# lh3/psmc

Hardware: AMD Instinct MI355X
Metric: genome bins/sec through forward-backward (n=64) (higher is better)
Workload: dtype f64; 1 GPU; configs[2]: whole-genome .psmcfa-like batch, 30000001 bins x 64 states in 90 segments per GPU, -p 4+25*2+4+6, one E-step (EM iteration) per step, parameters of a different EM round every step; mode=fast, bins_per_gpu=30000001, bins_total=30000001, n_states=64, segments=90, longest_segment=2490000, tiles=8127, speculative_overlap_bins=3072, structured_sweeps=True, tile_bins=3712

## Files before the change

include/psmc_hip.h:

```cpp
#ifndef PSMC_HIP_H
#define PSMC_HIP_H
#include <stdint.h>
#ifdef __cplusplus
extern "C" {
#endif

#define PSMC_HIP_MODE_EXACT 0
#define PSMC_HIP_MODE_FAST  1

#define PSMC_HIP_MAX_STATES 1024

#define PSMC_HIP_OK        0
#define PSMC_HIP_EINVAL   -1
#define PSMC_HIP_ENOMEM   -2
#define PSMC_HIP_EDEVICE  -3
#define PSMC_HIP_ENOTSUP  -4
#define PSMC_HIP_ESTATE   -5
#define PSMC_HIP_ECONVERGE -6

typedef struct psmc_hip_ctx psmc_hip_ctx;

int psmc_hip_device_count(void);
int psmc_hip_device_cus(int device);

int psmc_hip_create(psmc_hip_ctx **ctx, int n_states, int device, int mode);
void psmc_hip_destroy(psmc_hip_ctx *ctx);
const char *psmc_hip_strerror(int err);
const char *psmc_hip_last_error(const psmc_hip_ctx *ctx);

int psmc_hip_set_option(psmc_hip_ctx *ctx, const char *key, double value);

int psmc_hip_set_cu_range(psmc_hip_ctx *ctx, int first, int count);

int psmc_hip_load_segments(psmc_hip_ctx *ctx, int n_seg, const uint8_t *const *seq, const int32_t *L);
int psmc_hip_load_segments_device(psmc_hip_ctx *ctx, int n_seg, const void *d_obs, const int64_t *off,
                                  const int32_t *L);
int psmc_hip_select(psmc_hip_ctx *ctx, int n_sel, const int32_t *seg_idx);

int psmc_hip_estep(psmc_hip_ctx *ctx, const double *a, const double *e, const double *a0, double *A, double *E,
                   double *A0, double *LL, double *chk);

int psmc_hip_reserve_tables(psmc_hip_ctx *ctx);

int psmc_hip_reserve_batch_tables(psmc_hip_ctx *ctx, int64_t max_bins);
int psmc_hip_estep_batch(psmc_hip_ctx *ctx, int n_rep, const double *a, const double *e, const double *a0,
                         const int32_t *sel_off, const int32_t *sel_idx, double *A, double *sums, double *E, double *LL);
typedef void (*psmc_hip_batch_done_fn)(void *user, int n_done, const int32_t *replicates);
int psmc_hip_estep_batch_cb(psmc_hip_ctx *ctx, int n_rep, const double *a, const double *e, const double *a0,
                            const int32_t *sel_off, const int32_t *sel_idx, double *A, double *sums, double *E, double *LL,
                            psmc_hip_batch_done_fn done, void *user);
int psmc_hip_batch_info(psmc_hip_ctx *ctx, int out[2]);

int psmc_hip_estep_segments(psmc_hip_ctx *ctx, const double *a, const double *e, const double *a0, double *segA,
                            double *segE, double *segA0, double *segLL, double *chk);

int psmc_hip_estep_device(psmc_hip_ctx *ctx, const double *a, const double *e, const double *a0, void *d_stats,
                          void *stream);
int psmc_hip_fast_diag(psmc_hip_ctx *ctx, double *warm_err_fwd, double *warm_err_bwd, int *n_chunks,
                       int *warmup_used);
int psmc_hip_fast_repairs(psmc_hip_ctx *ctx, int out[6]);
int psmc_hip_fast_plan(psmc_hip_ctx *ctx, double out[8]);

int psmc_hip_estep_factored(psmc_hip_ctx *ctx, const double *a, const double *e, const double *a0, double *sums,
                            double *E, double *LL);

int psmc_hip_fast_info(psmc_hip_ctx *ctx, int out[8]);

int psmc_hip_get_tables(psmc_hip_ctx *ctx, int seg, double *f, double *b, double *s);

int psmc_hip_decode(psmc_hip_ctx *ctx, int seg, int32_t *path, double *maxp);

int psmc_hip_posterior(psmc_hip_ctx *ctx, int seg, double *post, double *recomb);

int psmc_hip_post_counts(psmc_hip_ctx *ctx, int seg, const int32_t *cnt1, int32_t l, int32_t n_cnt, double *cnt);

int psmc_hip_scales(psmc_hip_ctx *ctx, int seg, double *s);


typedef struct psmc_hip_group psmc_hip_group;
int  psmc_hip_group_create(psmc_hip_group **g, int n_states, int n_dev, const int *devices, int mode);
void psmc_hip_group_destroy(psmc_hip_group *g);
const char *psmc_hip_group_last_error(const psmc_hip_group *g);
int  psmc_hip_group_set_option(psmc_hip_group *g, const char *key, double value);
int  psmc_hip_group_load_segments(psmc_hip_group *g, int n_seg, const uint8_t *const *seq, const int32_t *L);
int  psmc_hip_group_estep(psmc_hip_group *g, const double *a, const double *e, const double *a0, double *A, double *E,
                          double *A0, double *LL, double *chk);
int  psmc_hip_group_estep_factored(psmc_hip_group *g, const double *a, const double *e, const double *a0, double *sums,
                                   double *E, double *LL);
int  psmc_hip_group_selfcheck(psmc_hip_group *g, int out[4]);
int  psmc_hip_group_info(psmc_hip_group *g, int *n_shards, int32_t *shard_of_seg, int *last_reduce);
int  psmc_hip_group_route(psmc_hip_group *g, int seg, psmc_hip_ctx **ctx, int *local_seg);
int  psmc_hip_estep_factored_device(psmc_hip_ctx *ctx, const double *a, const double *e, const double *a0, void *d_stats,
                                    void *stream);

#ifdef __cplusplus
}
#endif
#endif
```

psmc_amd/csrc/api.hip:

```cpp
#include "psmc_hip_ctx.h"

static void destroy_kids(psmc_hip_ctx *c);

static int make_streams(psmc_hip_ctx *c)
{
	hipStream_t *st[5] = {&c->stream, &c->stream2, &c->stream3, &c->stream4, &c->stream5};
	for (hipStream_t *s : st) if (*s) { (void)hipStreamSynchronize(*s); (void)hipStreamDestroy(*s); *s = nullptr; }
	if (c->cu_count <= 0) {
		for (hipStream_t *s : st) if (hipStreamCreateWithFlags(s, hipStreamNonBlocking) != hipSuccess) return PSMC_HIP_EDEVICE;
		return 0;
	}
	int cus = 0;
	if (hipDeviceGetAttribute(&cus, hipDeviceAttributeMultiprocessorCount, c->device) != hipSuccess || cus <= 0) return PSMC_HIP_EDEVICE;
	if (c->cu_first < 0 || c->cu_first + c->cu_count > cus) return PSMC_HIP_EINVAL;
	std::vector<uint32_t> mask((size_t)(cus + 31) / 32, 0u);
	for (int i = c->cu_first; i < c->cu_first + c->cu_count; ++i) mask[(size_t)i >> 5] |= 1u << (i & 31);
	for (hipStream_t *s : st) if (hipExtStreamCreateWithCUMask(s, (uint32_t)mask.size(), mask.data()) != hipSuccess) return PSMC_HIP_EDEVICE;
	return 0;
}

extern "C" int psmc_hip_device_cus(int device)
{
	int cus = 0;
	if (hipDeviceGetAttribute(&cus, hipDeviceAttributeMultiprocessorCount, device) != hipSuccess) { (void)hipGetLastError(); return 0; }
// ... 28 lines not shown

extern "C" int psmc_hip_device_count(void)
{
	int n = 0;
	if (hipGetDeviceCount(&n) != hipSuccess) return 0;
	return n;
}

extern "C" const char *psmc_hip_strerror(int err)
{
	switch (err) {
	case PSMC_HIP_OK: return "ok";
	case PSMC_HIP_EINVAL: return "invalid argument";
	case PSMC_HIP_ENOMEM: return "out of memory";
	case PSMC_HIP_EDEVICE: return "HIP runtime error";
	case PSMC_HIP_ENOTSUP: return "not supported in this build";
	case PSMC_HIP_ESTATE: return "call order violated";
	case PSMC_HIP_ECONVERGE: return "fast-mode tile boundaries did not converge";
	default: return "unknown error";
	}
}
extern "C" const char *psmc_hip_last_error(const psmc_hip_ctx *ctx) { return ctx ? ctx->err.c_str() : ""; }

extern "C" int psmc_hip_create(psmc_hip_ctx **out, int n_states, int device, int mode)
{
	if (!out) return PSMC_HIP_EINVAL;
	*out = nullptr;
	if (n_states < 1) return PSMC_HIP_EINVAL;
	if (mode != PSMC_HIP_MODE_EXACT && mode != PSMC_HIP_MODE_FAST) return PSMC_HIP_EINVAL;
	if (n_states > PSMC_HIP_MAX_STATES) return PSMC_HIP_ENOTSUP;
	int nd = psmc_hip_device_count();
	if (nd <= 0 || device < 0 || device >= nd) return PSMC_HIP_EDEVICE;
	if (hipSetDevice(device) != hipSuccess) return PSMC_HIP_EDEVICE;
	psmc_hip_ctx *c = new (std::nothrow) psmc_hip_ctx();
	if (!c) return PSMC_HIP_ENOMEM;
	c->n = n_states; c->ns = n_states > 128 ? (n_states + 63) / 64 * 64 : (n_states > 64 ? 128 : 64); c->device = device; c->mode = mode;
	c->par_len = c->ns > 128 ? 2 * (size_t)c->ns * c->ns + 4 * (size_t)c->ns : psmc_hip_ctx::PAR_LEN;
	if (make_streams(c) != 0) { psmc_hip_destroy(c); return PSMC_HIP_EDEVICE; }
	for (int i = 0; i < 14; ++i)
		if (hipEventCreate(&c->evx[i]) != hipSuccess) { delete c; return PSMC_HIP_EDEVICE; }
	for (int i = 0; i < 10; ++i)
		if (hipEventCreate(&c->ev[i]) != hipSuccess) { delete c; return PSMC_HIP_EDEVICE; }
	if (hipHostMalloc((void **)&c->h_par, c->par_len * sizeof(double), hipHostMallocDefault) != hipSuccess ||
	    hipMalloc((void **)&c->d_par, c->par_len * sizeof(double)) != hipSuccess) {
		psmc_hip_destroy(c);
		return PSMC_HIP_ENOMEM;
	}
	if (const char *env = getenv("PSMC_HIP_OPTIONS")) {
		std::string all(env);
		size_t at = 0;
		while (at < all.size()) {
			size_t end = all.find(',', at);
			if (end == std::string::npos) end = all.size();
			const std::string kv = all.substr(at, end - at);
			const size_t eq = kv.find('=');
			at = end + 1;
			if (kv.empty()) continue;
			char *endp = nullptr;
			const double val = eq == std::string::npos ? 0.0 : strtod(kv.c_str() + eq + 1, &endp);
			const bool parsed = eq != std::string::npos && eq + 1 < kv.size() && endp && *endp == '\0';
			if (parsed && kv.compare(0, eq, "rccl") == 0) continue;
			if (!parsed || psmc_hip_set_option(c, kv.substr(0, eq).c_str(), val) != PSMC_HIP_OK) {
				fprintf(stderr, "[psmc_hip] PSMC_HIP_OPTIONS: bad entry \"%s\" (unknown key, value out of range, or not a number)\n", kv.c_str());
				psmc_hip_destroy(c);
				return PSMC_HIP_EINVAL;
			}
		}
	}
	*out = c;
	return PSMC_HIP_OK;
}

static void destroy_kids(psmc_hip_ctx *c)
{
	if (c->x_twin) { psmc_hip_destroy(c->x_twin); c->x_twin = nullptr; }
	for (psmc_hip_ctx *k : c->kids) psmc_hip_destroy(k);
	c->kids.clear();
	c->share_T = 0;
}

extern "C" void psmc_hip_destroy(psmc_hip_ctx *c)
{
	if (!c) return;
	(void)hipSetDevice(c->device);
	destroy_kids(c);
	if (c->parent) {
		void *mine[] = {c->d_seg_off, c->d_seg_len, c->d_work, c->d_chunks, c->d_entry, c->d_bexit, c->d_Cpart, c->d_Epart, c->d_LLpart,
		                c->d_stage, c->d_stats, c->d_warm, c->d_bentry, c->d_dirty, c->d_cnt, c->d_gate, c->d_queue, c->d_touch, c->d_items, c->d_ftiles, c->d_Kcol,
		                c->d_segA, c->d_segE, c->d_segA0, c->d_chk};
		for (void *p : mine) if (p) (void)hipFree(p);
		if (c->h_cnt) (void)hipHostFree(c->h_cnt);
		if (c->h_ritems) (void)hipHostFree(c->h_ritems);
		if (c->h_mlen) (void)hipHostFree(c->h_mlen);
		if (c->h_chunks) (void)hipHostFree(c->h_chunks);
		if (c->h_mis) (void)hipHostFree(c->h_mis);
		if (c->d_prevx) (void)hipFree(c->d_prevx);
		if (c->d_finv) (void)hipFree(c->d_finv);
		delete c;
		return;
	}
	if (c->stream) (void)hipStreamSynchronize(c->stream);
	free_wide_fast(c);
	if (c->stream2) (void)hipStreamSynchronize(c->stream2);
	if (c->stream3) (void)hipStreamSynchronize(c->stream3);
	if (c->stream4) (void)hipStreamSynchronize(c->stream4);
	if (c->stream5) (void)hipStreamSynchronize(c->stream5);
	if (!c->obs_borrowed && c->d_obs) (void)hipFree(c->d_obs);
	void *ptrs[] = {c->d_seg_off, c->d_seg_len, c->d_work, c->d_par, c->d_f, c->d_b, c->d_s, c->d_segA, c->d_segE,
	                c->d_segA0, c->d_chk, c->d_chunks, c->d_entry, c->d_bexit, c->d_Cpart, c->d_Epart, c->d_LLpart,
	                c->d_stage, c->d_stats, c->d_warm, c->d_bentry, c->d_dirty, c->d_cnt, c->d_gate, c->d_queue, c->d_touch, c->d_sb, c->d_items, c->d_ftiles, c->d_Kcol,
	                c->d_bw_seg, c->d_bw_par, c->d_bw_tab, c->d_bpar, c->d_s_all, c->d_cu_mask, c->d_lkp, c->d_lkoff, c->d_b2};
	for (void *p : ptrs) if (p) (void)hipFree(p);
	if (c->h_par) (void)hipHostFree(c->h_par);
	if (c->h_cnt) (void)hipHostFree(c->h_cnt);
	if (c->h_ritems) (void)hipHostFree(c->h_ritems);
	if (c->h_mlen) (void)hipHostFree(c->h_mlen);
	if (c->h_chunks) (void)hipHostFree(c->h_chunks);
	if (c->h_mis) (void)hipHostFree(c->h_mis);
	if (c->d_prevx) (void)hipFree(c->d_prevx);
	if (c->d_finv) (void)hipFree(c->d_finv);
	for (int i = 0; i < 10; ++i) if (c->ev[i]) (void)hipEventDestroy(c->ev[i]);
	for (int i = 0; i < 14; ++i) if (c->evx[i]) (void)hipEventDestroy(c->evx[i]);
	if (c->stream4) (void)hipStreamDestroy(c->stream4);
	if (c->stream5) (void)hipStreamDestroy(c->stream5);
	if (c->stream2) (void)hipStreamDestroy(c->stream2);
	if (c->stream3) (void)hipStreamDestroy(c->stream3);
	if (c->stream) (void)hipStreamDestroy(c->stream);
	delete c;
}

extern "C" int psmc_hip_set_option(psmc_hip_ctx *c, const char *key, double v)
{
	if (!c || !key) return PSMC_HIP_EINVAL;
	std::string k(key);
	if (k == "batch_first") { if (v < 0 || v > 1e6) return PSMC_HIP_EINVAL; c->batch_first = (int)v; return PSMC_HIP_OK; }
	destroy_kids(c);
	if (k == "chunk") { if (v < 0) return PSMC_HIP_EINVAL; c->chunk = (int)v; c->plan_dirty = true; }
	else if (k == "warmup") { if (v < 0) return PSMC_HIP_EINVAL; c->warmup = (int)v; c->warmup_set = true; c->plan_dirty = true; }
	else if (k == "max_rounds") c->max_rounds = (int)v;
	else if (k == "structured") { c->struct_opt = v != 0 ? 1 : 0; }
	else if (k == "learn") { c->learn = v != 0 ? 1 : 0; }
	else if (k == "merge") { c->merge = v != 0 ? 1 : 0; c->plan_dirty = true; c->chunk_cap = 0; }
	else if (k == "adapt") { c->adapt = v != 0 ? 1 : 0; c->plan_dirty = true; c->chunk_cap = 0; }
	else if (k == "prev_start") { c->prev_start = v != 0 ? 1 : 0; c->prev_ok = false; c->plan_dirty = true; c->chunk_cap = 0; }
	else if (k == "warm_shift") { if (v < 0 || v > 4) return PSMC_HIP_EINVAL; c->warm_shift = (int)v; c->warm_shift_set = true; c->plan_dirty = true; }
	else if (k == "merge1") { if (v < -1 || v > 1) return PSMC_HIP_EINVAL; c->merge1 = (int)v; c->plan_dirty = true; }
	else if (k == "phase1") { if (v < -1 || v > 1) return PSMC_HIP_EINVAL; c->phase1 = (int)v; }
	else if (k == "phase1_waves") { if (v < 1 || v > 4) return PSMC_HIP_EINVAL; c->phase1_waves = (int)v; }
	else if (k == "lanes8") { if (v < -1 || v > 1) return PSMC_HIP_EINVAL; c->lanes8 = (int)v; }
	else if (k == "gap_tiles") { c->gap_tiles = v != 0 ? 1 : 0; c->plan_dirty = true; c->items_dirty = true; }
	else if (k == "coarse") { if (v < -1 || v > 16) return PSMC_HIP_EINVAL; c->coarse = (int)v; c->plan_dirty = true; c->items_dirty = true; }
	else if (k == "kc_sub") { if (v < 1 || v > 16) return PSMC_HIP_EINVAL; c->kc_sub = (int)v; c->kc_sub_set = true; c->plan_dirty = true; c->items_dirty = true; }
	else if (k == "two_phase") { if (v != -1 && v != 0 && v != 2) return PSMC_HIP_EINVAL; c->two_phase = (int)v; c->plan_dirty = true; c->items_dirty = true; }
	else if (k == "kc_min") { if (v < -1) return PSMC_HIP_EINVAL; c->kc_min = (int)v; c->items_dirty = true; }
	else if (k == "ckpt") { c->ckpt = v != 0 ? 1 : 0; }
	else if (k == "fuse") { c->fuse = v != 0 ? 1 : 0; c->plan_dirty = true; }
	else if (k == "fuse128") { if (v != 0 && v != 2) return PSMC_HIP_EINVAL; c->fuse128 = (int)v; c->plan_dirty = true; c->items_dirty = true; }
	else if (k == "group_cap") { if (v < 0) return PSMC_HIP_EINVAL; c->group_cap = (int)v; c->items_dirty = true; }
	else if (k == "share_learn") { c->share_learn = v != 0 ? 1 : 0; }
	else if (k == "exact_refwd") { if (v < -1 || v > 2) return PSMC_HIP_EINVAL; c->exact_refwd = (int)v; c->reserved_refwd = -1; c->reserved_cap = 0; if (c->d_b2) { (void)hipFree(c->d_b2); c->d_b2 = nullptr; c->b2_bins = c->b2_alloc = 0; } }
	else if (k == "batch_sort") { c->batch_sort = v != 0 ? 1 : 0; }
	else if (k == "batch_tailfill") c->batch_tailfill = v != 0;
	else if (k == "batch_major") c->batch_major = v != 0;
	else if (k == "batch_bins") { if (v < 0) return PSMC_HIP_EINVAL; c->batch_bins = (int64_t)v; }
	else if (k == "overlap") c->overlap = v != 0 ? 1 : 0;
	else if (k == "warm_tol") c->warm_tol = v;
	else if (k == "wide_fast") { if (v != 0 && v != 1) return PSMC_HIP_EINVAL; c->wide_fast = (int)v; }
	else if (k == "wide_decode") { if (v != 0 && v != 1) return PSMC_HIP_EINVAL; c->wide_decode = (int)v; }
	else if (k == "rep_impl") c->rep_impl = v < 0 ? -1 : (v != 0 ? 1 : 0);
	else return PSMC_HIP_EINVAL;
	return PSMC_HIP_OK;
}

int set_segments_common(psmc_hip_ctx *c, int n_seg, const int32_t *L)
{
	destroy_kids(c);
	c->reserved_refwd = -1; c->reserved_cap = 0;
	if (c->d_b2) { (void)hipFree(c->d_b2); c->d_b2 = nullptr; c->b2_bins = c->b2_alloc = 0; }
	c->n_seg = n_seg;
	c->L.assign(L, L + n_seg);
	int rc;
	if ((rc = dev_alloc(c, &c->d_seg_off, (size_t)n_seg))) return rc;
	if ((rc = dev_alloc(c, &c->d_seg_len, (size_t)n_seg))) return rc;
	HIPCHK(c, hipMemcpy(c->d_seg_off, c->off.data(), sizeof(int64_t) * n_seg, hipMemcpyHostToDevice));
	HIPCHK(c, hipMemcpy(c->d_seg_len, c->L.data(), sizeof(int32_t) * n_seg, hipMemcpyHostToDevice));
	std::vector<int32_t> all(n_seg);
	for (int i = 0; i < n_seg; ++i) all[i] = i;
	return psmc_hip_select(c, n_seg, all.data());
}

extern "C" int psmc_hip_load_segments(psmc_hip_ctx *c, int n_seg, const uint8_t *const *seq, const int32_t *L)
{
	if (!c || n_seg < 1 || !seq || !L) return fail(c, PSMC_HIP_EINVAL, "load_segments: bad argument");
	HIPCHK(c, hipSetDevice(c->device));
	c->off.resize(n_seg);
	int64_t tot = 0;
	for (int i = 0; i < n_seg; ++i) {
		if (L[i] < 1 || !seq[i]) return fail(c, PSMC_HIP_EINVAL, "load_segments: empty segment");
		c->off[i] = tot;
		tot += ((int64_t)L[i] + 63) & ~(int64_t)63;
	}
	c->total = tot;
	std::vector<uint8_t> host((size_t)tot + 256, 2);
	for (int i = 0; i < n_seg; ++i) {
		for (int32_t j = 0; j < L[i]; ++j)
			if (seq[i][j] > 2) return fail(c, PSMC_HIP_EINVAL, "load_segments: symbol outside {0,1,2}");
		memcpy(host.data() + c->off[i], seq[i], (size_t)L[i]);
	}
	if (!c->obs_borrowed && c->d_obs) { (void)hipFree(c->d_obs); }
	c->d_obs = nullptr; c->obs_borrowed = false;
	int rc;
	if ((rc = dev_alloc(c, &c->d_obs, host.size()))) return rc;
	HIPCHK(c, hipMemcpy(c->d_obs, host.data(), host.size(), hipMemcpyHostToDevice));
	return set_segments_common(c, n_seg, L);
}

extern "C" int psmc_hip_load_segments_device(psmc_hip_ctx *c, int n_seg, const void *d_obs, const int64_t *off,
                                             const int32_t *L)
{
	if (!c || n_seg < 1 || !d_obs || !off || !L) return fail(c, PSMC_HIP_EINVAL, "load_segments_device: bad argument");
	HIPCHK(c, hipSetDevice(c->device));
	int64_t end = 0;
	for (int i = 0; i < n_seg; ++i) {
		if (L[i] < 1 || (off[i] & 63) || off[i] < end) return fail(c, PSMC_HIP_EINVAL, "load_segments_device: bad layout");
		end = off[i] + (((int64_t)L[i] + 63) & ~(int64_t)63);
	}
	if (!c->obs_borrowed && c->d_obs) (void)hipFree(c->d_obs);
	c->d_obs = (uint8_t *)d_obs; c->obs_borrowed = true;
	c->off.assign(off, off + n_seg);
	c->total = end;
	return set_segments_common(c, n_seg, L);
}

extern "C" int psmc_hip_select(psmc_hip_ctx *c, int n_sel, const int32_t *idx)
{
	if (!c || n_sel < 1 || !idx) return fail(c, PSMC_HIP_EINVAL, "select: bad argument");
	if (c->n_seg < 1) return fail(c, PSMC_HIP_ESTATE, "select: no segments loaded");
	std::vector<int32_t> pos(c->n_seg, -1);
	c->sel.assign(idx, idx + n_sel);
	c->work.clear(); c->mult.clear(); c->sel2work.resize(n_sel);
	for (int i = 0; i < n_sel; ++i) {
		if (idx[i] < 0 || idx[i] >= c->n_seg) return fail(c, PSMC_HIP_EINVAL, "select: index out of range");
		if (pos[idx[i]] < 0) { pos[idx[i]] = (int32_t)c->work.size(); c->work.push_back(idx[i]); c->mult.push_back(0); }
		c->sel2work[i] = pos[idx[i]];
		c->mult[pos[idx[i]]]++;
	}
	HIPCHK(c, hipSetDevice(c->device));
	int rc;
	if ((rc = dev_alloc(c, &c->d_work, c->work.size()))) return rc;
	HIPCHK(c, hipMemcpy(c->d_work, c->work.data(), sizeof(int32_t) * c->work.size(), hipMemcpyHostToDevice));
	c->plan_dirty = true;
	++c->sel_serial;
	return PSMC_HIP_OK;
}

bool factor_structure(int n, int S, const double *a , double *sp )
{
	double *P = sp, *R = sp + S, *qa = sp + 2 * S, *cc = sp + 3 * S, *dd = sp + 4 * S;
	memset(sp, 0, 5 * (size_t)S * sizeof(double));
	if (n < 3) return false;
	const double pl = a[(n - 1) * S + 0], pu = a[0 * S + (n - 1)];
	if (!(pl > 1e-280) || !(pu > 1e-280)) return false;
	for (int l = 0; l < n - 1; ++l) qa[l] = a[(n - 1) * S + l] / pl;
	for (int k = 1; k < n; ++k) P[k] = a[k * S + 0];
	for (int l = 1; l < n; ++l) cc[l] = a[0 * S + l] / pu;
	for (int k = 0; k < n - 1; ++k) R[k] = a[k * S + (n - 1)];
	const double tol = 64 * 2.220446049250313e-16;
	for (int k = 0; k < n; ++k) {
		for (int l = 0; l < n; ++l) {
			if (l == k) continue;
			const double v = a[k * S + l], w = l < k ? P[k] * qa[l] : R[k] * cc[l];
			if (!(fabs(v - w) <= tol * fabs(v) + 1e-290)) return false;
		}
		dd[k] = a[k * S + k] - P[k] * qa[k] - R[k] * cc[k];
		if (!(dd[k] >= 0.0)) return false;
	}
	return true;
}

static void fill_kcc(int S, const double *sp, const double *e3 , double *out )
{
	const double *P = sp, *R = sp + S, *qa = sp + 2 * S, *cv = sp + 3 * S, *dd = sp + 4 * S;
	for (int dir = 0; dir < 2; ++dir) {
		double *t = out + (size_t)dir * 11 * S;
		const double *mS = dir == 0 ? P : cv, *wS = dir == 0 ? qa : R, *mP = dir == 0 ? R : qa, *wP = dir == 0 ? cv : P;
		for (int k = 0; k < S; ++k) { t[k] = mS[k]; t[S + k] = mP[k]; }
		for (int sy = 0; sy < 3; ++sy)
			for (int k = 0; k < S; ++k) {
				const double ev = e3[sy * S + k];
				double *u = t + 2 * S + (size_t)sy * 3 * S;
				u[k] = wS[k] * ev; u[S + k] = wP[k] * ev; u[2 * S + k] = dd[k] * ev;
			}
	}
}

bool fill_params(const psmc_hip_ctx *c, const double *a, const double *e, const double *a0, double *dst)
{
	const int n = c->n;
	if (c->ns > 128) {
		const size_t S = (size_t)c->ns;
		double *pa = dst, *pt = pa + S * S, *pe = pt + S * S, *pa0 = pe + 3 * S;
		memset(pa, 0, c->par_len * sizeof(double));
		for (int k = 0; k < n; ++k) {
			for (int l = 0; l < n; ++l) { pa[k * S + l] = a[(size_t)k * n + l]; pt[l * S + k] = a[(size_t)k * n + l]; }
			pe[k] = e[k]; pe[S + k] = e[n + k];
			pa0[k] = a0[k];
// ... 299 lines not shown
```

psmc_amd/csrc/api_batch.hip:

```cpp
#include "psmc_hip_ctx.h"

namespace {
struct RepSel { std::vector<int32_t> work, sel2work; int64_t bins = 0; };
}

static int batch_selections(psmc_hip_ctx *c, int n_rep, const int32_t *sel_off, const int32_t *sel_idx, std::vector<RepSel> &reps)
{
	std::vector<int32_t> pos(c->n_seg);
	reps.assign(n_rep, RepSel());
	for (int r = 0; r < n_rep; ++r) {
		const int n_sel = sel_off[r + 1] - sel_off[r];
		if (n_sel < 1) return fail(c, PSMC_HIP_EINVAL, "estep_batch: empty selection");
		std::fill(pos.begin(), pos.end(), -1);
		RepSel &R = reps[r];
		R.sel2work.resize(n_sel);
		for (int i = 0; i < n_sel; ++i) {
			const int32_t sg = sel_idx[sel_off[r] + i];
			if (sg < 0 || sg >= c->n_seg) return fail(c, PSMC_HIP_EINVAL, "estep_batch: index out of range");
			if (pos[sg] < 0) { pos[sg] = (int32_t)R.work.size(); R.work.push_back(sg); R.bins += ((int64_t)c->L[sg] + 63) & ~(int64_t)63; }
			R.sel2work[i] = pos[sg];
		}
	}
	return 0;
}
// ... 226 lines not shown
		if (c->bpar_cap < (size_t)n_rep) { if ((rc = dev_alloc(c, &c->d_bpar, (size_t)n_rep * PL))) return rc; c->bpar_cap = (size_t)n_rep; }
		if (refwd && !c->d_cu_mask && (rc = dev_alloc(c, &c->d_cu_mask, (size_t)4096))) return rc;
		size_t lk_worst = 0;
		for (int g = 0; g < n_launches; ++g) {
			size_t t = 0;
			for (int i = l_first[g]; i < l_first[g + 1]; ++i) t += wseg[i] >= 0 ? (size_t)(c->L[wseg[i]] / LKP_DIV + LKP_MIN) : 1;
			lk_worst = std::max(lk_worst, t);
		}
		if (c->lkp_cap < lk_worst) { if ((rc = dev_alloc(c, &c->d_lkp, lk_worst))) return rc; c->lkp_cap = lk_worst; }
		if (c->lkoff_cap < worst_entries) { if ((rc = dev_alloc(c, &c->d_lkoff, worst_entries))) return rc; c->lkoff_cap = worst_entries; }
		if (fwd_all && c->s_all_cap < (size_t)all_bins + 128) { if ((rc = dev_alloc(c, &c->d_s_all, (size_t)all_bins + 128))) return rc; c->s_all_cap = (size_t)all_bins + 128; }
	}
	static const bool dbg_t = getenv("PSMC_HIP_DEBUG_TIMES") != nullptr;
	auto now = []() { return dbg_now(); };
	{
		std::vector<double> hp((size_t)n_rep * PL);
		for (int r = 0; r < n_rep; ++r) (void)fill_params(c, a + (size_t)r * n * n, e + (size_t)r * 2 * n, a0 + (size_t)r * n, hp.data() + (size_t)r * PL);
		HIPCHK(c, hipStreamSynchronize(c->stream));
		HIPCHK(c, hipMemcpyAsync(c->d_bw_seg, wseg.data(), sizeof(int32_t) * n_all, hipMemcpyHostToDevice, c->stream));
		HIPCHK(c, hipMemcpyAsync(c->d_bw_par, wpar.data(), sizeof(int32_t) * n_all, hipMemcpyHostToDevice, c->stream));
		HIPCHK(c, hipMemcpyAsync(c->d_bw_tab, wtab.data(), sizeof(int64_t) * n_all, hipMemcpyHostToDevice, c->stream));
		HIPCHK(c, hipMemcpyAsync(c->d_bw_tab + n_all, wtab_s.data(), sizeof(int64_t) * n_all, hipMemcpyHostToDevice, c->stream));
		HIPCHK(c, hipMemcpyAsync(c->d_bpar, hp.data(), sizeof(double) * hp.size(), hipMemcpyHostToDevice, c->stream));
		HIPCHK(c, hipStreamSynchronize(c->stream));
	}
	c->tables_batch = true;
	double fwd_all_s = 0.0;
	if (fwd_all) {
		const double t0 = now();
		EstepLaunch p;
		fill_common(c, p, c->stream, c->d_bpar);
		p.d_work = c->d_bw_seg; p.n_work = n_all; p.d_work_par = c->d_bw_par; p.d_work_tab = c->d_bw_tab + n_all; p.par_stride = (int64_t)PL; p.work_align = align;
		p.exact_refwd = 1; p.exact_only = 1; p.d_s = c->d_s_all;
		if (launch_exact(p) != 0) return fail(c, PSMC_HIP_EDEVICE, "launch_exact (batch, forward pass of all entries)", hipGetLastError());
		if (dbg_t) { (void)hipStreamSynchronize(c->stream); fwd_all_s = now() - t0; }
	}
	if ((double)n_all * (double)(S * S) * 8.0 > 16e9) {
		c->err = "estep_batch: the per-entry statistics of this call (" + std::to_string(n_all) + " entries x " + std::to_string(S) + "^2 doubles) need more than 16 GB of host memory: send fewer replicates per call at this many states";
		return PSMC_HIP_ENOMEM;
	}
	c->h_segA.resize((size_t)n_all * S * S); c->h_segE.resize((size_t)n_all * 3 * S);
	std::vector<double> lk_all((size_t)n_all, 0.0);
	std::vector<int> last_launch(n_rep, 0);
	{
		std::vector<int> launch_of((size_t)n_all, 0);
		for (int g = 0; g < n_launches; ++g) for (int i = l_first[g]; i < l_first[g + 1]; ++i) launch_of[i] = g;
		for (int r = 0; r < n_rep; ++r) for (int w : ent_of[r]) if (w >= 0) last_launch[r] = std::max(last_launch[r], launch_of[w]);
	}
	std::vector<double> sA((size_t)n * n), sE((size_t)2 * n);
	double t_sums = 0.0;
	auto finalize = [&](int r) {
		const RepSel &R = reps[r];
		std::fill(sA.begin(), sA.end(), 0.0); std::fill(sE.begin(), sE.end(), 0.0);
		double ll = 0.0;
		for (size_t i = 0; i < R.sel2work.size(); ++i) {
			const int w = ent_of[r][R.sel2work[i]];
			const double *hA = &c->h_segA[(size_t)w * S * S], *hE = &c->h_segE[(size_t)w * 3 * S];
			ll += lk_all[(size_t)w];
			for (int k = 0; k < n; ++k)
				for (int l = 0; l < n; ++l) sA[(size_t)k * n + l] += hA[k * S + l];
			for (int b = 0; b < 2; ++b)
				for (int l = 0; l < n; ++l) sE[(size_t)b * n + l] += hE[b * S + l];
		}
		if (A) memcpy(A + (size_t)r * n * n, sA.data(), sizeof(double) * n * n);
		if (E) memcpy(E + (size_t)r * 2 * n, sE.data(), sizeof(double) * 2 * n);
		if (LL) LL[r] = ll;
		if (sums) {
			double *q = sums + (size_t)r * 5 * n;
			memset(q, 0, sizeof(double) * 5 * n);
			for (int k = 0; k < n; ++k)
				for (int l = 0; l < n; ++l) {
					const double v = sA[(size_t)k * n + l];
					if (l < k) { q[k] += v; q[3 * n + l] += v; } else if (l > k) { q[n + k] += v; q[4 * n + l] += v; } else q[2 * n + k] = v;
				}
		}
	};
	std::vector<int32_t> finished;
	for (int g = 0; g < n_launches; ++g) {
		const double t_a = now();
		const int e0 = l_first[g], nw = l_first[g + 1] - e0;
		int64_t run = 0; int32_t longest = 0;
		for (int i = e0; i < e0 + nw; ++i) if (wseg[i] >= 0) { run = std::max(run, wtab[i] + padded_len(wseg[i])); longest = std::max(longest, c->L[wseg[i]]); }
		EstepLaunch p;
		fill_common(c, p, c->stream, c->d_bpar);
		p.d_work = c->d_bw_seg + e0; p.n_work = nw; p.d_work_par = c->d_bw_par + e0; p.d_work_tab = c->d_bw_tab + e0; p.par_stride = (int64_t)PL; p.work_align = align;
		p.exact_refwd = refwd ? (c->exact_refwd == 1 ? 1 : 2) : 0;
		p.d_cu_mask = c->d_cu_mask;
		if (fwd_all) { p.exact_only = 2; p.d_work_tab_s = c->d_bw_tab + n_all + e0; p.d_s = c->d_s_all; }
		p.d_segA = c->d_segA; p.d_segE = c->d_segE; p.d_segA0 = c->d_segA0; p.d_chk = c->d_chk;
		const double t_b = now();
		if (launch_exact(p) != 0) return fail(c, PSMC_HIP_EDEVICE, "launch_exact (batch)", hipGetLastError());
		if (dbg_t) (void)hipStreamSynchronize(c->stream);
		const double t_c = now();
		std::vector<int64_t> lkoff((size_t)nw);
		int64_t lk_tot = 0;
		for (int i = 0; i < nw; ++i) { lkoff[i] = lk_tot; lk_tot += wseg[e0 + i] >= 0 ? c->L[wseg[e0 + i]] / LKP_DIV + LKP_MIN : 1; }
		HIPCHK(c, hipMemcpyAsync(c->d_lkoff, lkoff.data(), sizeof(int64_t) * nw, hipMemcpyHostToDevice, c->stream));
		if (launch_lk_products(c->stream, p, fwd_all ? c->d_s_all : c->d_s, c->d_lkoff, c->d_lkp) != 0) return fail(c, PSMC_HIP_EDEVICE, "launch_lk_products", hipGetLastError());
		c->h_lkp.resize((size_t)lk_tot);
		HIPCHK(c, hipMemcpyAsync(c->h_segA.data() + (size_t)e0 * S * S, c->d_segA, sizeof(double) * nw * S * S, hipMemcpyDeviceToHost, c->stream));
		HIPCHK(c, hipMemcpyAsync(c->h_segE.data() + (size_t)e0 * 3 * S, c->d_segE, sizeof(double) * nw * 3 * S, hipMemcpyDeviceToHost, c->stream));
		HIPCHK(c, hipMemcpyAsync(c->h_lkp.data(), c->d_lkp, sizeof(double) * (size_t)lk_tot, hipMemcpyDeviceToHost, c->stream));
		HIPCHK(c, hipStreamSynchronize(c->stream));
		const double t_d = now();
		collect_timing(c);
		int n_over = 0;
		for (int i = 0; i < nw; ++i) {
			if (wseg[e0 + i] < 0) continue;
			const int32_t sg = wseg[e0 + i];
			const double *q = &c->h_lkp[(size_t)lkoff[i]];
			const int cnt = (int)q[0], cap_i = c->L[sg] / LKP_DIV + LKP_MIN;
			if (cnt >= 1 && cnt < cap_i) {
				double sum = 0.0;
				for (int j = 1; j <= cnt; ++j) sum += log(q[j]);
				lk_all[(size_t)e0 + i] = sum;
			} else {
				++n_over;
				c->h_s.resize((size_t)c->L[sg]);
				HIPCHK(c, hipMemcpyAsync(c->h_s.data(), (fwd_all ? c->d_s_all + wtab_s[e0 + i] : c->d_s + wtab[e0 + i]), sizeof(double) * (size_t)c->L[sg], hipMemcpyDeviceToHost, c->stream));
				HIPCHK(c, hipStreamSynchronize(c->stream));
				lk_all[(size_t)e0 + i] = host_lk(c->h_s.data(), c->L[sg]);
			}
		}
		if (dbg_t && n_over) fprintf(stderr, "[psmc_hip] batch launch %d: %d entries logged more products than their buffer holds (host hmm_lk)\n", g, n_over);
		if (dbg_t) fprintf(stderr, "[psmc_hip] batch launch %d: %d entries (longest %d bins), %.1f M table bins | prepare %.3f s, kernels %.3f (fwd %.0f bwd %.0f expect %.0f ms%s), read-back %.3f, hmm_lk %.3f\n",
		                   g, nw, (int)longest, run / 1e6, t_b - t_a, t_c - t_b, c->last_ms[1], c->last_ms[2], c->last_ms[3],
		                   fwd_all ? (g == 0 ? (std::string("; forward pass of all entries ") + std::to_string(fwd_all_s) + " s").c_str() : "; fwd: see launch 0") : "", t_d - t_c, now() - t_d);
		++c->last_batch_groups;
		const double t_f = now();
		finished.clear();
		for (int r = 0; r < n_rep; ++r) if (last_launch[r] == g) { finalize(r); finished.push_back(r); }
		t_sums += now() - t_f;
		if (done && !finished.empty()) done(user, (int)finished.size(), finished.data());
	}
	if (dbg_t) {
		std::string per;
		for (int g = 0; g < n_launches; ++g) per += (g ? " " : "") + std::to_string(std::count(last_launch.begin(), last_launch.end(), g));
		fprintf(stderr, "[psmc_hip] batch: %d replicates, %d entries in %d launches (replicates complete after launch 0..: %s), host sums %.3f s\n", n_rep, n_all, n_launches, per.c_str(), t_sums);
	}
	return PSMC_HIP_OK;
}

static psmc_hip_ctx *batch_child(psmc_hip_ctx *c, int r)
{
	while ((int)c->kids.size() <= r) {
		psmc_hip_ctx *k = new (std::nothrow) psmc_hip_ctx();
		if (!k) return nullptr;
		k->n = c->n; k->ns = c->ns; k->device = c->device; k->mode = c->mode; k->parent = c;
		k->chunk = c->chunk > 0 ? c->chunk : c->share_T;
		k->warmup = c->warmup; k->max_rounds = c->max_rounds; k->rep_impl = c->rep_impl;
		k->n_sub = c->n_sub; k->target_waves = c->target_waves; k->overlap = c->overlap; k->warm_tol = c->warm_tol; k->struct_opt = c->struct_opt;
		k->struct_tiles_set = c->struct_tiles_set; k->struct_tiles = c->struct_tiles;
		k->two_phase = c->two_phase; k->kc_div = c->kc_div; k->kc_min = c->kc_min; k->ckpt = c->ckpt; k->fuse = c->fuse;
		k->learn = c->learn; k->group_cap = c->group_cap; k->warm_shift = c->warm_shift; k->kc_sub = c->kc_sub; k->kcol_prio = c->kcol_prio;
		k->fuse128 = c->fuse128; k->coarse = c->coarse; k->gate = c->gate; k->lanes8 = c->lanes8; k->gap_tiles = c->gap_tiles; k->exact_refwd = c->exact_refwd;
		k->merge = c->merge; k->adapt = c->adapt; k->prev_start = c->prev_start;
		k->merge1 = c->merge1; k->merge_order = c->merge_order; k->runs_late = c->runs_late; k->warm_shift_set = c->warm_shift_set; k->kc_sub_set = c->kc_sub_set;
		k->stream = c->stream; k->stream2 = c->stream2; k->stream3 = c->stream3; k->stream4 = c->stream4; k->stream5 = c->stream5;
		for (int i = 0; i < 14; ++i) k->evx[i] = c->evx[i];
		for (int i = 0; i < 10; ++i) k->ev[i] = c->ev[i];
		k->h_par = c->h_par; k->d_par = c->d_par; k->par_len = c->par_len;
		k->d_obs = c->d_obs; k->obs_borrowed = true; k->off = c->off; k->total = c->total;
		if (set_segments_common(k, c->n_seg, c->L.data()) != 0) { c->err = k->err; psmc_hip_destroy(k); return nullptr; }
		c->kids.push_back(k);
	}
	return c->kids[r];
}

static int batch_exact_once(psmc_hip_ctx *c, int r, const int32_t *idx, int n_sel, const double *a, const double *e, const double *a0,
                            double *A, double *sums, double *E, double *LL, const char *why)
{
	const int n = c->n;
	fprintf(stderr, "[psmc_hip] replicate %d: fast E-step did not converge (%s); repeating this E-step with the exact kernels\n", c->batch_first + r, why);
	int rc = 0;
	if (!c->x_twin) {
		if ((rc = psmc_hip_create(&c->x_twin, n, c->device, PSMC_HIP_MODE_EXACT))) return fail(c, rc, "estep_batch: cannot create the exact twin context");
		if ((rc = psmc_hip_load_segments_device(c->x_twin, c->n_seg, c->d_obs, c->off.data(), c->L.data()))) {
			c->err = "exact twin: " + c->x_twin->err; psmc_hip_destroy(c->x_twin); c->x_twin = nullptr; return rc;
		}
	}
	std::vector<double> Af;
	double *Ao = A;
	if (!Ao) { Af.resize((size_t)n * n); Ao = Af.data(); }
	if ((rc = psmc_hip_select(c->x_twin, n_sel, idx)) || (rc = psmc_hip_estep(c->x_twin, a, e, a0, Ao, E, nullptr, LL, nullptr))) { c->err = "exact twin: " + c->x_twin->err; return rc; }
	if (sums) {
		memset(sums, 0, sizeof(double) * 5 * (size_t)n);
		for (int k = 0; k < n; ++k)
			for (int l = 0; l < n; ++l) {
				const double v = Ao[(size_t)k * n + l];
				if (l < k) { sums[k] += v; sums[3 * n + l] += v; } else if (l > k) { sums[n + k] += v; sums[4 * n + l] += v; } else sums[2 * n + k] = v;
			}
	}
	++c->n_exact_fallbacks;
	return PSMC_HIP_OK;
}

static int batch_fast(psmc_hip_ctx *c, int n_rep, const double *a, const double *e, const double *a0, const int32_t *sel_off,
                      const int32_t *sel_idx, double *A, double *sums, double *E, double *LL, psmc_hip_batch_done_fn done, void *user)
{
	const int n = c->n;
	if (c->share_T == 0 && c->share_learn) {
		int T = c->chunk;
		if (T <= 0) {
			std::vector<RepSel> reps;
			int rc0 = batch_selections(c, n_rep, sel_off, sel_idx, reps);
			if (rc0) return rc0;
			int64_t most = 0; size_t nw = 1;
			for (const RepSel &R : reps) {
				int64_t bins = 0;
				for (int32_t sg : R.work) bins += c->L[sg];
				if (bins > most) { most = bins; nw = R.work.size(); }
			}
			T = auto_tile_len(c, most, nw, true);
		}
		c->share_T = T;
		c->sh_glue_f.assign(c->n_seg, {}); c->sh_glue_b.assign(c->n_seg, {}); c->sh_wf.assign(c->n_seg, {}); c->sh_wb.assign(c->n_seg, {});
		for (int sg = 0; sg < c->n_seg; ++sg) {
			const size_t nt = ((size_t)c->L[sg] + T - 1) / T;
			c->sh_glue_f[sg].assign(nt, 0); c->sh_glue_b[sg].assign(nt, 0); c->sh_wf[sg].assign(nt, c->warmup); c->sh_wb[sg].assign(nt, c->warmup);
		}
	}
	static const bool dbg_t = getenv("PSMC_HIP_DEBUG_TIMES") != nullptr;
	const double t_call = dbg_now();
	double t_est = 0.0;
	for (int r = 0; r < n_rep; ++r) {
		const double t_k = dbg_now();
		psmc_hip_ctx *k = batch_child(c, c->batch_first + r);
		c->dbg_acc[0] += dbg_now() - t_k;
		if (!k) return fail(c, PSMC_HIP_ENOMEM, "estep_batch: cannot create the replicate context");
		const int n_sel = sel_off[r + 1] - sel_off[r];
		if (n_sel < 1) return fail(c, PSMC_HIP_EINVAL, "estep_batch: empty selection");
		const int32_t *idx = sel_idx + sel_off[r];
		int rc = 0;
		{
			const double t_s = dbg_now();
			if ((int)k->sel.size() != n_sel || memcmp(k->sel.data(), idx, sizeof(int32_t) * n_sel) != 0) rc = psmc_hip_select(k, n_sel, idx);
			c->dbg_acc[1] += dbg_now() - t_s;
		}
		const double t_e = dbg_now();
		const double *ar = a + (size_t)r * n * n, *er = e + (size_t)r * 2 * n, *a0r = a0 + (size_t)r * n;
		if (rc == 0) {
			double *Ar = A ? A + (size_t)r * n * n : nullptr, *Sr = sums ? sums + (size_t)r * 5 * n : nullptr, *Er = E ? E + (size_t)r * 2 * n : nullptr, *Lr = LL ? LL + r : nullptr;
			if (A) rc = psmc_hip_estep(k, ar, er, a0r, Ar, Er, nullptr, Lr, nullptr);
			if (rc == 0 && sums) rc = psmc_hip_estep_factored(k, ar, er, a0r, Sr, Er, Lr);
			if (rc == PSMC_HIP_ECONVERGE) rc = batch_exact_once(c, r, idx, n_sel, ar, er, a0r, Ar, Sr, Er, Lr, k->err.c_str());
		}
		t_est += dbg_now() - t_e;
		if (rc) { c->err = "replicate " + std::to_string(r) + ": " + k->err; return rc; }
		if (done) { const int32_t rr = r; done(user, 1, &rr); }
	}
	if (dbg_t) {
		const double *q = c->dbg_acc;
		fprintf(stderr, "[psmc_hip] fast batch on device %d: %d replicates %.3f s | contexts %.3f, select %.3f, E-steps %.3f (plan %.3f, items %.3f, launches %.3f, rest %.3f); "
		                "%.0f repair rounds, %.0f repaired tiles\n", c->device, n_rep, dbg_now() - t_call, q[0], q[1], t_est, q[2], q[3], q[4], t_est - q[2] - q[3] - q[4], q[6], q[7]);
		for (double &v : c->dbg_acc) v = 0.0;
	}
	c->tables_batch = true;
	c->last_batch_groups = n_rep;
	return PSMC_HIP_OK;
}

extern "C" int psmc_hip_estep_batch(psmc_hip_ctx *c, int n_rep, const double *a, const double *e, const double *a0,
                                    const int32_t *sel_off, const int32_t *sel_idx, double *A, double *sums, double *E, double *LL)
{
	return psmc_hip_estep_batch_cb(c, n_rep, a, e, a0, sel_off, sel_idx, A, sums, E, LL, nullptr, nullptr);
}

extern "C" int psmc_hip_estep_batch_cb(psmc_hip_ctx *c, int n_rep, const double *a, const double *e, const double *a0,
                                       const int32_t *sel_off, const int32_t *sel_idx, double *A, double *sums, double *E, double *LL,
                                       psmc_hip_batch_done_fn done, void *user)
{
	if (!c || n_rep < 1 || !a || !e || !a0 || !sel_off || !sel_idx || (!A && !sums)) return fail(c, PSMC_HIP_EINVAL, "estep_batch: bad argument");
	if (c->parent) return fail(c, PSMC_HIP_EINVAL, "estep_batch: not on a replicate context");
	if (c->n_seg < 1) return fail(c, PSMC_HIP_ESTATE, "estep_batch: no segments loaded");
	HIPCHK(c, hipSetDevice(c->device));
	c->wd_kind = WD_NONE;
	if (c->mode == PSMC_HIP_MODE_EXACT || c->ns > 128) return batch_exact(c, n_rep, a, e, a0, sel_off, sel_idx, A, sums, E, LL, done, user);
	return batch_fast(c, n_rep, a, e, a0, sel_off, sel_idx, A, sums, E, LL, done, user);
}

extern "C" int psmc_hip_batch_info(psmc_hip_ctx *c, int out[2])
{
	if (!c || !out) return PSMC_HIP_EINVAL;
	out[0] = c->last_batch_groups; out[1] = (int)c->kids.size();
	return PSMC_HIP_OK;
}
```

psmc_amd/csrc/api_fast.hip:

```cpp
#include "psmc_hip_ctx.h"

int ensure_fast_buffers(psmc_hip_ctx *c)
{
	if (c->d_stage && c->d_stats && c->d_warm && c->d_cnt && c->h_cnt && c->d_gate) return 0;
	int rc;
	const size_t sl = (size_t)c->ns * c->ns + 3 * (size_t)c->ns + 1;
	if ((rc = dev_alloc(c, &c->d_stage, (size_t)RED_ROWS * sl))) return rc;
	if ((rc = dev_alloc(c, &c->d_stats, sl))) return rc;
	if ((rc = dev_alloc(c, &c->d_warm, (size_t)2))) return rc;
	if ((rc = dev_alloc(c, &c->d_cnt, (size_t)4))) return rc;
	if ((rc = dev_alloc(c, &c->d_gate, (size_t)4))) return rc;
	if (!c->h_cnt && (hipHostMalloc((void **)&c->h_cnt, 4 * sizeof(int), hipHostMallocMapped) != hipSuccess ||
	                  hipHostGetDevicePointer((void **)&c->m_cnt, c->h_cnt, 0) != hipSuccess)) {
		c->h_cnt = nullptr;
		return fail(c, PSMC_HIP_ENOMEM, "hipHostMalloc (mapped)");
	}
	return 0;
}

int auto_tile_len(const psmc_hip_ctx *c, int64_t bins, size_t n_work, bool st)
{
	const int64_t ROUND1 = 4096;
	int64_t want = st ? c->struct_tiles : c->target_waves;
	if (st && !c->struct_tiles_set && bins < 2 * ROUND1 * (int64_t)std::max(c->warmup, 1))
// ... 91 lines not shown
		for (int b = 0; b < nc; ++b) {
			if (c->gap[b]) { if (same(b - 1, b)) c->glue_f[b] = 1; if (same(b, b + 1)) c->glue_b[b] = 1; }
			if (b > 0 && c->gap[b - 1] && same(b - 1, b)) c->glue_f[b] = 1;
			if (b + 1 < nc && c->gap[b + 1] && same(b, b + 1)) c->glue_b[b] = 1;
		}
	}
	c->plan_dirty = false; c->chunks_dirty = false; c->prev_ok = false;
	return 0;
}

static int build_items(psmc_hip_ctx *c, bool two_phase_bwd, int coarse)
{
	const int nc = (int)c->chunks.size(), W = c->warmup;
	const int cf = std::max(1, coarse), cb = two_phase_bwd ? 1 : cf;
	std::vector<int> odd(nc, 0), idx(nc, 0);
	for (int b = 1; b < nc; ++b) if (c->chunks[b].off == c->chunks[b - 1].off) { odd[b] = !odd[b - 1]; idx[b] = idx[b - 1] + 1; }
	std::vector<std::pair<long long, std::pair<int, int>>> kf, kb;
	auto key = [](int steps, bool run, bool phase_b) { return (run ? -(1ll << 40) : (phase_b ? (1ll << 40) : 0ll)) - steps; };
	std::vector<char> from_above(nc, 0), in_run(nc, 0), in_run_f(nc, 0), in_run_b(nc, 0);
	std::vector<std::pair<int, int>> gf, gb;
	auto same_seg = [&](int x, int y) { return c->chunks[x].off == c->chunks[y].off; };
	const bool gaps = c->gap_tiles && (int)c->gap.size() == nc;
	std::vector<int64_t> eff(nc + 1, 0);
	for (int b = 0; b < nc; ++b) eff[b + 1] = eff[b] + ((gaps && c->gap[b]) ? 0 : c->chunks[b].hi - c->chunks[b].lo + 1);
	auto span_ok = [&](int b, int e) { return eff[e + 1] - eff[b] <= (int64_t)c->group_cap; };
	for (int b = 0; b < nc;) {
		int e = b + 1;
		while (e < nc && c->glue_f[e] && same_seg(e, b) && span_ok(b, e)) ++e;
		if (e - b > 1) for (int t = b; t < e; ++t) in_run[t] = in_run_f[t] = 1;
		else
			while (e < nc && e - b < cf && same_seg(e, b) && idx[e] % cf != 0 && !c->glue_f[e] && !(e + 1 < nc && c->glue_f[e + 1] && same_seg(e + 1, e))) ++e;
		gf.push_back({b, e - b});
		b = e;
	}
	for (int b = 0; b < nc;) {
		int e = b + 1;
		while (e < nc && c->glue_b[e - 1] && same_seg(e, b) && span_ok(b, e) &&
		       c->chunks[e].lo < c->chunks[e].L)
			++e;
		if (e - b > 1) for (int t = b; t < e; ++t) in_run[t] = in_run_b[t] = 1;
		else
			while (e < nc && e - b < cb && same_seg(e, b) && idx[e] % cb != 0 && !c->glue_b[e - 1] && !(e + 1 < nc && c->glue_b[e] && same_seg(e + 1, e)) &&
			       c->chunks[e].lo < c->chunks[e].L)
				++e;
		gb.push_back({b, e - b});
		b = e;
	}
	int n_run = 0;
	for (int b = 0; b < nc; ++b) n_run += in_run[b];
	const int cap_b = (nc + 7) / 8 * 4;
	c->runs_in_b = two_phase_bwd && c->runs_late && n_run > 0 && n_run <= cap_b / 2;
	int above_budget = c->runs_in_b ? cap_b - n_run : nc;
	for (const auto &gr : gb) {
		const int b = gr.first, e = b + gr.second;
		const Chunk &lo = c->chunks[b], &top = c->chunks[e - 1];
		bool pb = two_phase_bwd && e - b == 1 && odd[b] && b + 1 < nc && c->chunks[b + 1].off == lo.off && c->chunks[b + 1].lo < c->chunks[b + 1].L;
		if (pb && c->runs_in_b && (in_run[b] || in_run[b + 1] || above_budget <= 0)) pb = false;
		if (pb) { from_above[b] = 1; --above_budget; }
		kb.push_back({key(std::min(top.hi + chunk_warm_b(top, W) + 1, top.L) - lo.lo, in_run_b[b] != 0, pb), {b, e - b}});
	}
	std::vector<int> la, lb;
	{
		std::vector<int> freet;
		for (int b = 0; b < nc; ++b) {
			if (from_above[b]) lb.push_back(b | (1 << 30));
			else if (b > 0 && from_above[b - 1]) la.push_back(b);
			else if (c->runs_in_b && in_run[b]) lb.push_back(b);
			else freet.push_back(b);
		}
		const bool single = lb.empty() && nc <= 4096;
		for (int b : freet) { if (single || la.size() <= lb.size()) la.push_back(b); else lb.push_back(b); }
	}
	for (const auto &gr : gf) {
		const int b = gr.first, e = b + gr.second;
		const Chunk &h = c->chunks[b], &l = c->chunks[e - 1];
		kf.push_back({key(l.hi - std::max(1, h.lo - chunk_warm_f(h, W)) + 1, in_run_f[b] != 0, false), {b, e - b}});
	}
	std::sort(kf.begin(), kf.end()); std::sort(kb.begin(), kb.end());
	std::vector<int> h((size_t)4 * nc, 0), mem((size_t)4 * nc, 0);
	c->n_mem_f = c->n_mem_b = 0;
	for (size_t i = 0; i < kf.size(); ++i) {
		h[2 * i] = kf[i].second.first; h[2 * i + 1] = kf[i].second.second;
		if (in_run_f[kf[i].second.first])
			for (int t = 0; t < kf[i].second.second; ++t) { mem[2 * (size_t)c->n_mem_f] = kf[i].second.first + t; mem[2 * (size_t)c->n_mem_f + 1] = 1; ++c->n_mem_f; }
	}
	for (size_t i = 0; i < kb.size(); ++i) {
		h[(size_t)2 * nc + 2 * i] = kb[i].second.first; h[(size_t)2 * nc + 2 * i + 1] = kb[i].second.second;
		if (in_run_b[kb[i].second.first])
			for (int t = 0; t < kb[i].second.second; ++t) {
				mem[(size_t)2 * nc + 2 * (size_t)c->n_mem_b] = kb[i].second.first + t; mem[(size_t)2 * nc + 2 * (size_t)c->n_mem_b + 1] = 1; ++c->n_mem_b;
			}
	}
	c->n_items_f = (int)kf.size(); c->n_items_b = (int)kb.size();
	c->order_f.clear();
	for (const auto &it : kf) if (!in_run_f[it.second.first]) c->order_f.push_back(it.second.first);
	c->n_long_f = c->n_long_b = 0;
	while (c->n_long_f < c->n_items_f && in_run_f[kf[c->n_long_f].second.first]) ++c->n_long_f;
	while (c->n_long_b < c->n_items_b && in_run_b[kb[c->n_long_b].second.first]) ++c->n_long_b;
	c->n_B_b = 0;
	for (int b = 0; b < nc; ++b) c->n_B_b += from_above[b];
	{
		c->n_list_a = (int)la.size(); c->n_list_b = (int)lb.size();
		c->count_group = c->ns == 128 && c->fuse128 == 2 ? 16 : 4;
		while (la.size() % c->count_group) la.push_back(-1);
		while (lb.size() % c->count_group) lb.push_back(-1);
		la.insert(la.end(), lb.begin(), lb.end());
		if (!la.empty()) HIPCHK(c, hipMemcpy(c->d_ftiles, la.data(), sizeof(int) * la.size(), hipMemcpyHostToDevice));
	}
	c->items_two_phase = two_phase_bwd ? 2 : 0; c->items_coarse = coarse;
	HIPCHK(c, hipMemcpy(c->d_items, h.data(), sizeof(int) * h.size(), hipMemcpyHostToDevice));
	{
		std::vector<int> sg;
		for (size_t i = (size_t)c->n_long_b; i < kb.size(); ++i)
			for (int t = kb[i].second.second - 1; t >= 0; --t) { sg.push_back(kb[i].second.first + t); sg.push_back(1); }
		c->n_singles_b = (int)sg.size() / 2;
		if (!sg.empty()) HIPCHK(c, hipMemcpy(c->d_items + (size_t)24 * nc, sg.data(), sizeof(int) * sg.size(), hipMemcpyHostToDevice));
	}
	HIPCHK(c, hipMemcpy(c->d_items + (size_t)8 * nc, mem.data(), sizeof(int) * mem.size(), hipMemcpyHostToDevice));
	{
		std::vector<int> fx;
		for (int b = 0; b < nc; ++b)
			if (!in_run_f[b] && !(b > 0 && in_run_f[b - 1] && same_seg(b - 1, b))) { fx.push_back(b); fx.push_back(1); }
		c->n_fix_f = (int)fx.size() / 2;
		if (!fx.empty()) HIPCHK(c, hipMemcpy(c->d_items + (size_t)30 * nc, fx.data(), sizeof(int) * fx.size(), hipMemcpyHostToDevice));
	}
	{
		const int n4f = c->n_items_f - c->n_long_f, n4b = c->n_items_b - c->n_long_b - c->n_B_b;
		std::vector<std::pair<long long, int>> qk;
		for (int k = 0; 4 * k < n4f; ++k) {
			long long st = 0;
			for (int i = c->n_long_f + 4 * k; i < std::min(c->n_long_f + 4 * k + 4, c->n_items_f); ++i) {
				const Chunk &h = c->chunks[kf[i].second.first], &l = c->chunks[kf[i].second.first + kf[i].second.second - 1];
				st = std::max(st, (long long)(l.hi - std::max(1, h.lo - chunk_warm_f(h, W)) + 1));
			}
			qk.push_back({-st * 504, 2 * k});
		}
		for (int k = 0; 4 * k < n4b; ++k) {
			long long st = 0;
			for (int i = c->n_long_b + 4 * k; i < std::min(c->n_long_b + 4 * k + 4, c->n_long_b + n4b); ++i) {
				const Chunk &lo = c->chunks[kb[i].second.first], &top = c->chunks[kb[i].second.first + kb[i].second.second - 1];
				const int q = std::min(top.hi + chunk_warm_b(top, W) + 1, top.L);
				st = std::max(st, (long long)(q - (coarse > 1 ? std::min(lo.hi, lo.L - 1) : std::min(top.hi, top.L - 1))));
			}
			qk.push_back({-st * 534, 2 * k + 1});
		}
		std::stable_sort(qk.begin(), qk.end(), [](const std::pair<long long, int> &x, const std::pair<long long, int> &y) { return x.first < y.first; });
		std::vector<int> qv(qk.size());
		for (size_t i = 0; i < qk.size(); ++i) qv[i] = qk[i].second;
		if (c->queue_cap < qv.size()) { int rc; if ((rc = dev_alloc(c, &c->d_queue, qv.size()))) return rc; c->queue_cap = qv.size(); }
		c->n_queue = (int)qv.size();
		if (!qv.empty()) HIPCHK(c, hipMemcpy(c->d_queue, qv.data(), sizeof(int) * qv.size(), hipMemcpyHostToDevice));
	}
	std::vector<int> wl((size_t)4 * nc, 0), kc, runs_f, runs_b, kslot, kuniq;
	int gap_slot[2] = {-1, -1};
	auto push_kc = [&](int t, int dir) {
		const int j = (int)kc.size() / 2;
		kc.push_back(t); kc.push_back(dir);
		if (gaps && c->gap[t] && c->chunk_used % 4 == 0) {
			if (gap_slot[dir] < 0) { gap_slot[dir] = (int)kuniq.size(); kuniq.push_back(j); }
			kslot.push_back(gap_slot[dir]);
		} else { kslot.push_back((int)kuniq.size()); kuniq.push_back(j); }
	};
	c->n_wl_f = c->n_wl_b = 0;
	const int kc_min = c->kc_min >= 0 ? c->kc_min : (c->ns == 128 ? (nc > 4096 ? 12 : 8) : (nc > 4096 ? 5 : 4));
	const bool chains = kc_min >= 2;
	const int head_count = c->ns == 64 ? 0 : 1;
	auto add_runs = [&](const std::vector<std::pair<long long, std::pair<int, int>>> &k, int n_long, bool bwd) {
		int &nw = bwd ? c->n_wl_b : c->n_wl_f;
		std::vector<int> &rv = bwd ? runs_b : runs_f;
		int *w = wl.data() + (bwd ? (size_t)2 * nc : 0);
		int budget = std::max(64, nc / c->kc_div);
		for (int i = 0; i < n_long; ++i) {
			int first = k[i].second.first, count = k[i].second.second;
			int cost = 0;
			for (int tt = first; tt < first + count; ++tt) cost += (gaps && c->gap[tt] && c->chunk_used % 4 == 0) ? 0 : 1;
			cost = std::max(cost - 1, 1);
			const bool chain = chains && count >= kc_min && cost <= budget;
			if (chain) budget -= cost;
			if (chain && !bwd && c->chunks[first].lo == 1) {
				w[2 * nw] = first; w[2 * nw + 1] = (head_count == 0 && count - 1 >= 2) ? -1 : 2; ++nw;
				first += 1; count -= 1;
				if (count >= 2) {
					rv.push_back(first); rv.push_back(count); rv.push_back((int)(kc.size() / 2)); rv.push_back(0);
					for (int t = first; t < first + count - 1; ++t) push_kc(t, 0);
				}
			} else if (chain) {
				w[2 * nw] = bwd ? first + count - 1 : first; w[2 * nw + 1] = head_count; ++nw;
				rv.push_back(first); rv.push_back(count); rv.push_back((int)(kc.size() / 2)); rv.push_back(0);
				if (!bwd) for (int t = first; t < first + count - 1; ++t) push_kc(t, 0);
				else for (int t = first + count - 1; t > first; --t) push_kc(t, 1);
			} else { w[2 * nw] = first; w[2 * nw + 1] = (head_count == 0 && !bwd) ? -(count - 1) : count; ++nw; }
		}
	};
	add_runs(kf, c->n_long_f, false);
	add_runs(kb, c->n_long_b, true);
	c->n_chain_f = (int)runs_f.size() / 4; c->n_chain_b = (int)runs_b.size() / 4; c->n_kc = (int)kc.size() / 2; c->n_kuniq = (int)kuniq.size();
	if ((size_t)c->n_kc > (size_t)2 * nc || (size_t)(c->n_chain_f + c->n_chain_b) > (size_t)nc) return fail(c, PSMC_HIP_ESTATE, "build_items: list overflow");
	HIPCHK(c, hipMemcpy(c->d_items + (size_t)12 * nc, wl.data(), sizeof(int) * wl.size(), hipMemcpyHostToDevice));
	if (c->n_kc > 0) {
		std::vector<int> runs(runs_f); runs.insert(runs.end(), runs_b.begin(), runs_b.end());
		HIPCHK(c, hipMemcpy(c->d_items + (size_t)16 * nc, kc.data(), sizeof(int) * kc.size(), hipMemcpyHostToDevice));
		HIPCHK(c, hipMemcpy(c->d_items + (size_t)20 * nc, runs.data(), sizeof(int) * runs.size(), hipMemcpyHostToDevice));
		HIPCHK(c, hipMemcpy(c->d_items + (size_t)26 * nc, kslot.data(), sizeof(int) * kslot.size(), hipMemcpyHostToDevice));
		HIPCHK(c, hipMemcpy(c->d_items + (size_t)28 * nc, kuniq.data(), sizeof(int) * kuniq.size(), hipMemcpyHostToDevice));
		const size_t nsub = kcol2_on(c) ? (size_t)c->kc_sub_used : 1;
		const size_t need = (size_t)c->n_kuniq * nsub * ((size_t)c->ns * c->ns + c->ns);
		if (need > c->kcol_cap) { int rc; if ((rc = dev_alloc(c, &c->d_Kcol, need))) return rc; c->kcol_cap = need; }
	}
	c->items_dirty = false;
	if (getenv("PSMC_HIP_DEBUG"))
		fprintf(stderr, "[psmc_hip] buffers: obs %p (+%lld) chunks %p (%d) items %p entry %p bentry %p bexit %p f %p b %p s %p sb %p Cpart %p Epart %p ftiles %p touch %p par %p Kcol %p\n",
		        (void *)c->d_obs, (long long)c->total + 256, (void *)c->d_chunks, nc, (void *)c->d_items, (void *)c->d_entry, (void *)c->d_bentry, (void *)c->d_bexit,
		        (void *)c->d_f, (void *)c->d_b, (void *)c->d_s, (void *)c->d_sb, (void *)c->d_Cpart, (void *)c->d_Epart, (void *)c->d_ftiles, (void *)c->d_touch, (void *)c->d_par, (void *)c->d_Kcol);
	if (getenv("PSMC_HIP_DEBUG"))
		fprintf(stderr, "[psmc_hip] items: %d tiles of %d bins, fwd %d items (%d runs, %d run tiles, %d walks, %d chains), bwd %d items (%d runs, %d run tiles, %d walks, %d chains, %d from above), %d transfer matrices, fused lists %d + %d\n",
		        nc, c->chunk_used, c->n_items_f, c->n_long_f, c->n_mem_f, c->n_wl_f, c->n_chain_f, c->n_items_b, c->n_long_b, c->n_mem_b, c->n_wl_b, c->n_chain_b, c->n_B_b, c->n_kc, c->n_list_a, c->n_list_b);
	return 0;
}

static void learn_groups(psmc_hip_ctx *c)
{
	const int nc = (int)c->chunks.size(), W = c->warmup;
	const int cap = W << c->warm_shift_used;
	for (int b : c->flagged_f)
		if (b > 0 && b < nc && !c->glue_f[b] && c->chunks[b - 1].off == c->chunks[b].off) {
			Chunk &ch = c->chunks[b];
			if (ch.wf < cap && ch.lo - ch.wf > 1) { ch.wf = std::min(cap, std::max(2 * ch.wf, W)); c->chunks_dirty = true; }
			else c->glue_f[b] = 1;
			c->items_dirty = true;
		}
	for (int b : c->flagged_b)
		if (b >= 0 && b + 1 < nc && !c->glue_b[b] && c->chunks[b + 1].off == c->chunks[b].off) {
			Chunk &ch = c->chunks[b];
			if (ch.wb < cap && (int64_t)ch.hi + ch.wb + 1 < ch.L) { ch.wb = std::min(cap, std::max(2 * ch.wb, W)); c->chunks_dirty = true; }
			else c->glue_b[b] = 1;
			c->items_dirty = true;
		}
	if (c->parent && c->parent->share_T == c->chunk_used && (!c->flagged_f.empty() || !c->flagged_b.empty())) {
		psmc_hip_ctx *P = c->parent;
		auto put = [&](int b) {
			if (b < 0 || b >= nc) return;
			const int sg = c->chunk_seg[b], ix = c->chunk_idx[b];
			if (sg >= (int)P->sh_glue_f.size() || ix >= (int)P->sh_glue_f[sg].size()) return;
			P->sh_glue_f[sg][ix] |= c->glue_f[b]; P->sh_glue_b[sg][ix] |= c->glue_b[b];
			P->sh_wf[sg][ix] = std::max(P->sh_wf[sg][ix], c->chunks[b].wf); P->sh_wb[sg][ix] = std::max(P->sh_wb[sg][ix], c->chunks[b].wb);
		};
		for (int b : c->flagged_f) put(b);
		for (int b : c->flagged_b) put(b);
	}
}

static void adapt_warmups(psmc_hip_ctx *c)
{
	const int nc = (int)c->chunks.size();
	const int cap = c->warmup << c->warm_shift_used, floor_w = std::min(c->warmup, 256);
	const double tol = c->warm_tol;
	bool changed = false;
	for (int b = 0; b < nc; ++b) {
		const double m = c->h_mis[b];
		if (!(m > 0.0)) continue;
		if (c->glue_f[b] || (b + 1 < nc && c->glue_f[b + 1] && c->chunks[b + 1].off == c->chunks[b].off)) continue;
		Chunk &ch = c->chunks[b];
		if (ch.lo - ch.wf <= 1) continue;
		int w = ch.wf;
		if (m > tol) {
			const int ml = c->h_mlen[b];
			w = std::min(std::max(cap, w), w + (ml > 0 ? 16 * ml + 64 : w));
		} else {
			const double slack = log10(tol / std::max(m, 1e-17)), keep = 2.0;
			if (slack > keep) w = std::max(floor_w, w - (((int)std::min((slack - keep) * 160.0, w / 8.0) + 15) & ~15));
		}
		if (w != ch.wf) { ch.wf = w; changed = true; }
	}
	if (changed) {
		c->chunks_dirty = true;
		int64_t total = 0, waste = 0;
		for (size_t i = 0; i + 3 < c->order_f.size(); i += 4) {
			int64_t s4 = 0, mx = 0;
			for (int r = 0; r < 4; ++r) { const Chunk &ch = c->chunks[c->order_f[i + r]]; const int64_t st = (int64_t)ch.hi - std::max(1, ch.lo - ch.wf) + 1; s4 += st; mx = std::max(mx, st); }
			total += 4 * mx; waste += 4 * mx - s4;
		}
		if (total > 0 && waste * 100 > total * 3) c->items_dirty = true;
	}
}

int enqueue_fast(psmc_hip_ctx *c, const double *a, const double *e, const double *a0, double *d_out,
                        hipStream_t st)
{
	HIPCHK(c, hipSetDevice(c->device));
	if (c->n_seg < 1) return fail(c, PSMC_HIP_ESTATE, "estep: no segments loaded");
	int rc;
	c->dec_kind = DEC_NONE;
	const unsigned long long serial0 = dbg_root(c)->tab_serial;
	if ((rc = ensure_tables(c, false))) return rc;
	c->tables_batch = false;
	if ((rc = stage_params(c, a, e, a0, st))) return rc;
	if (!c->want_factored && !(c->use_struct && fused_counts(c)) && (rc = ensure_tables(c, true))) return rc;
	if (c->ns == 128 && !c->use_struct)
		return fail(c, PSMC_HIP_ENOTSUP, "fast mode beyond 64 states needs a transition matrix of the PSMC form (structured sweeps)");
	if (c->want_factored && !c->use_struct)
		return fail(c, PSMC_HIP_ENOTSUP, "factored statistics need a transition matrix of the PSMC form");
	{
		const double t0 = dbg_now();
		if ((c->plan_dirty || c->planned_struct != c->use_struct) && (rc = plan_fast(c))) return rc;
		dbg_root(c)->dbg_acc[2] += dbg_now() - t0;
	}
	EstepLaunch p;
	fill_common(c, p, st);
	p.d_chunks = c->d_chunks; p.n_chunks = (int)c->chunks.size(); p.warmup = c->warmup; p.n_sub = c->n_sub_used;
	const bool two_phase_bwd = c->two_phase_used >= 1 && p.fused == 1;
	p.merge1 = c->merge1_used; p.merge_order = c->merge_order >= 0 ? c->merge_order : (c->chunk_used < c->warmup ? 1 : 0);
	if (c->chunks_dirty) {
		psmc_hip_ctx *R = dbg_root(c);
		if (R->h_chunks_cap < c->chunks.size()) {
			if (R->h_chunks) { (void)hipHostFree(R->h_chunks); R->h_chunks = nullptr; }
			if (hipHostMalloc((void **)&R->h_chunks, sizeof(Chunk) * c->chunks.size(), hipHostMallocDefault) != hipSuccess) return fail(c, PSMC_HIP_ENOMEM, "hipHostMalloc");
			R->h_chunks_cap = c->chunks.size();
		}
		HIPCHK(c, hipStreamSynchronize(st));
		memcpy(R->h_chunks, c->chunks.data(), sizeof(Chunk) * c->chunks.size());
		HIPCHK(c, hipMemcpyAsync(c->d_chunks, R->h_chunks, sizeof(Chunk) * c->chunks.size(), hipMemcpyHostToDevice, st));
		c->chunks_dirty = false;
	}
	const int coarse = (c->use_struct && p.fused != 0) ? c->coarse_used : 1;
	{
		const double t0 = dbg_now();
		if (c->use_struct && (c->items_dirty || c->items_two_phase != (two_phase_bwd ? 2 : 0) || c->items_coarse != coarse) && (rc = build_items(c, two_phase_bwd, coarse))) return rc;
		dbg_root(c)->dbg_acc[3] += dbg_now() - t0;
	}
	p.lanes8 = (c->lanes8 >= 0 ? c->lanes8 != 0 && p.fused != 0 : p.fused == 2 && p.n_chunks > 4096) && c->ns == 64 ? 1 : 0;
	{
		const size_t nc_ = c->chunks.size(), S_ = (size_t)c->ns;
		const size_t need = p.fused == 2 ? nc_ * 7 * S_ + 64 : (p.fused == 1 ? (nc_ / 4 + 8) * S_ * S_ : nc_ * (size_t)c->n_sub_used * S_ * S_);
		if (c->cpart_cap < need) { if ((rc = dev_alloc(c, &c->d_Cpart, need))) return rc; c->cpart_cap = need; }
	}
	{
		c->merge_used = c->merge != 0 && c->h_mlen && c->use_struct && p.fused == 1 && c->ns == 64 && c->chunk_used % 16 == 0;
		p.merge = c->merge_used ? 1 : 0;
		p.d_fmerge = c->d_touch + 2 * (size_t)p.n_chunks; p.d_finv = c->d_finv; p.m_mlen = c->m_mlen; p.h_mlen = c->h_mlen; p.m_mis = c->m_mis;
		p.d_fix_f = c->d_items + 30 * (size_t)p.n_chunks; p.n_fix_f = c->n_fix_f;
		if (c->h_mlen) memset(c->h_mlen, 0, sizeof(int) * p.n_chunks);
		if (c->h_mis) for (int b = 0; b < p.n_chunks; ++b) c->h_mis[b] = -1.0;
		const bool prev = c->prev_start && c->d_prevx && c->prev_ok && c->use_struct && c->prev_serial == serial0 && c->prev_f == c->d_f && c->prev_ckpt == p.ckpt;
		p.d_prevx = prev ? c->d_prevx : nullptr;
		c->prev_ok = false;
	}
	p.d_gate = (c->gate >= 0 ? c->gate != 0 : coarse > 1) ? c->d_gate : nullptr;
	if (c->phase1 != 0 && c->use_struct && p.fused == 1 && c->ns == 64 && !p.lanes8 && !p.merge1 && c->overlap && c->n_queue > 0) {
		int cus = c->cu_count;
		if (cus <= 0 && (hipDeviceGetAttribute(&cus, hipDeviceAttributeMultiprocessorCount, c->device) != hipSuccess || cus <= 0)) return fail(c, PSMC_HIP_EDEVICE, "hipDeviceGetAttribute");
		p.d_queue = c->d_queue; p.n_queue = c->n_queue; p.d_qhead = c->d_gate + 2;
		p.q_grid = std::min(c->n_queue, 4 * cus * c->phase1_waves);
	}
	p.coarse = coarse; p.d_singles_b = c->d_items + 24 * (size_t)p.n_chunks; p.n_singles_b = c->n_singles_b;
	p.n_B_b = c->n_B_b; p.runs_in_b = c->runs_in_b ? 1 : 0; p.n_list_a = c->n_list_a; p.n_list_b = c->n_list_b; p.d_ftiles = c->d_ftiles; p.count_group = c->count_group;
	c->timing_two_launches = p.fused == 1 && p.n_list_b > 0;
	p.d_items_f = c->d_items; p.d_items_b = c->d_items + 2 * p.n_chunks;
	p.d_ritems_f = c->d_items + 4 * p.n_chunks; p.d_ritems_b = c->d_items + 6 * p.n_chunks;
	p.n_items_f = c->n_items_f; p.n_items_b = c->n_items_b; p.tile_len = c->chunk_used; p.h_ritems = c->h_ritems; p.m_ritems = c->m_ritems; p.m_cnt = c->m_cnt;
	c->flagged_f.clear(); c->flagged_b.clear();
	p.flagged_f = &c->flagged_f; p.flagged_b = &c->flagged_b;
	p.d_entry = c->d_entry; p.d_bentry = c->d_bentry; p.d_bexit = c->d_bexit; p.d_Cpart = c->d_Cpart; p.d_Epart = c->d_Epart;
	p.d_dirty = c->d_dirty; p.d_cnt = c->d_cnt; p.h_cnt = c->h_cnt; p.tol = c->warm_tol; p.max_rounds = c->max_rounds;
	p.d_touch_f = c->d_touch; p.d_touch_b = c->d_touch + p.n_chunks; p.d_dirty_b = c->d_dirty + p.n_chunks;
	p.stream2 = c->stream2; p.stream3 = c->stream3; p.stream4 = c->stream4; p.overlap = c->overlap;
	p.n_long_f = c->n_long_f; p.n_long_b = c->n_long_b; p.n_mem_f = c->n_mem_f; p.n_mem_b = c->n_mem_b;
	p.d_members_f = c->d_items + 8 * p.n_chunks; p.d_members_b = c->d_items + 10 * p.n_chunks;
	p.d_wl_f = c->d_items + 12 * (size_t)p.n_chunks; p.d_wl_b = c->d_items + 14 * (size_t)p.n_chunks; p.n_wl_f = c->n_wl_f; p.n_wl_b = c->n_wl_b;
	p.d_kc = c->d_items + 16 * (size_t)p.n_chunks; p.d_kruns = c->d_items + 20 * (size_t)p.n_chunks;
	p.n_kc = c->n_kc; p.n_chain_f = c->n_chain_f; p.n_chain_b = c->n_chain_b;
	p.d_kslot = c->d_items + 26 * (size_t)p.n_chunks; p.d_kuniq = c->d_items + 28 * (size_t)p.n_chunks; p.n_kuniq = c->n_kuniq;
	p.kcol_prio = c->kcol_prio;
	p.d_Kcol = c->d_Kcol; p.kc_sub = kcol2_on(c) ? c->kc_sub_used : 1;
	p.d_Kexp = c->d_Kcol ? c->d_Kcol + (size_t)c->n_kuniq * p.kc_sub * c->ns * c->ns : nullptr; p.stream5 = c->stream5;
	for (int i = 0; i < 14; ++i) p.evx[i] = c->evx[i];
	p.d_LLpart = c->d_LLpart; p.d_stage = c->d_stage; p.d_stats = d_out; p.d_warm = c->d_warm;
	p.tiny_total = (double)c->sel.size() * HMM_TINY_H;
	if (p.d_prevx) launch_gather_prev(p, st, c->n_long_f, c->n_items_f - c->n_long_f, c->d_prevx);
	{
		const double t0 = dbg_now();
		if (launch_fast(p, &c->report) != 0) return fail(c, PSMC_HIP_EDEVICE, "launch_fast", hipGetLastError());
		psmc_hip_ctx *R = dbg_root(c);
		R->dbg_acc[4] += dbg_now() - t0;
		R->dbg_acc[6] += c->report.fwd_rounds + c->report.bwd_rounds; R->dbg_acc[7] += c->report.fwd_tiles + c->report.bwd_tiles;
	}
	if (getenv("PSMC_HIP_DEBUG_FLAGGED")) {
		auto dump = [&](const char *dir, const std::vector<int> &fl, const std::vector<uint8_t> &glue, bool bwd) {
			std::vector<int> u(fl); std::sort(u.begin(), u.end()); u.erase(std::unique(u.begin(), u.end()), u.end());
			fprintf(stderr, "[psmc_hip] flagged %s: %zu tile repairs, %zu distinct tiles, rounds %d:", dir, fl.size(), u.size(), bwd ? c->report.bwd_rounds : c->report.fwd_rounds);
			for (size_t i = 0; i < u.size() && i < 400; ++i) {
				const int b = u[i]; const Chunk &ch = c->chunks[b];
				int seg = 0; while (seg + 1 < c->n_seg && c->off[seg + 1] <= ch.off) ++seg;
				fprintf(stderr, " [t%d seg%d %d..%d w%d g%d x%d m%.1e ml%d]", b, seg, ch.lo, ch.hi, bwd ? ch.wb : ch.wf, (int)glue[b], (int)std::count(fl.begin(), fl.end(), b),
				        c->h_mis ? c->h_mis[(bwd ? c->chunks.size() : 0) + b] : 0.0, (!bwd && c->h_mlen) ? c->h_mlen[b] : 0);
			}
			fprintf(stderr, "\n");
		};
		dump("fwd", c->flagged_f, c->glue_f, false); dump("bwd", c->flagged_b, c->glue_b, true);
	}
	if (!c->report.converged) return fail(c, PSMC_HIP_ECONVERGE, "fast mode: tile boundaries did not converge within max_rounds");
	if (c->merge_used && c->h_mlen)
		for (size_t b = 0; b < c->chunks.size(); ++b) {
			c->report.merged += c->h_mlen[b] > 0;
			if (c->h_mlen[b] < 0 || (c->h_mlen[b] > 0 && !c->adapt)) c->flagged_f.push_back((int)b);
		}
	if (c->use_struct && c->adapt && c->merge_used && c->h_mis) adapt_warmups(c);
	if (c->use_struct && c->learn) learn_groups(c);
	if (c->use_struct) { c->prev_ok = true; c->prev_serial = dbg_root(c)->tab_serial; c->prev_f = c->d_f; c->prev_ckpt = p.ckpt; }
	c->dec_kind = c->merge_used ? DEC_MERGED : (p.fused != 0 ? DEC_NO_BT : DEC_FAST);
	c->dec_serial = dbg_root(c)->tab_serial;
	return 0;
}

int read_warm(psmc_hip_ctx *c, hipStream_t st)
{
	unsigned long long w[2];
	HIPCHK(c, hipMemcpyAsync(w, c->d_warm, sizeof(w), hipMemcpyDeviceToHost, st));
	HIPCHK(c, hipStreamSynchronize(st));
	memcpy(&c->warm_err[0], &w[0], 8); memcpy(&c->warm_err[1], &w[1], 8);
	return 0;
}

extern "C" int psmc_hip_estep_device(psmc_hip_ctx *c, const double *a, const double *e, const double *a0,
                                     void *d_stats, void *stream)
{
	if (!c || !a || !e || !a0 || !d_stats) return fail(c, PSMC_HIP_EINVAL, "estep_device: bad argument");
	if (c->mode != PSMC_HIP_MODE_FAST) return fail(c, PSMC_HIP_ENOTSUP, "estep_device: fast mode only");
	c->timing_valid = false;
	return enqueue_fast(c, a, e, a0, (double *)d_stats, (hipStream_t)stream);
}

extern "C" int psmc_hip_fast_diag(psmc_hip_ctx *c, double *wf, double *wb, int *n_chunks, int *warmup_used)
{
	if (!c) return PSMC_HIP_EINVAL;
	if (c->mode != PSMC_HIP_MODE_FAST || !c->d_warm) return fail(c, PSMC_HIP_ESTATE, "fast_diag: no fast E-step yet");
	HIPCHK(c, hipSetDevice(c->device));
	unsigned long long w[2];
	HIPCHK(c, hipMemcpy(w, c->d_warm, sizeof(w), hipMemcpyDeviceToHost));
	memcpy(&c->warm_err[0], &w[0], 8); memcpy(&c->warm_err[1], &w[1], 8);
	if (wf) *wf = c->warm_err[0];
	if (wb) *wb = c->warm_err[1];
	if (n_chunks) *n_chunks = (int)(c->wf_ran ? c->wf_chunks.size() : c->chunks.size());
	if (warmup_used) *warmup_used = c->wf_ran ? c->wf_W : c->warmup;
	return PSMC_HIP_OK;
}

extern "C" int psmc_hip_fast_repairs(psmc_hip_ctx *c, int out[6])
{
	if (!c || !out) return PSMC_HIP_EINVAL;
	out[0] = c->report.fwd_rounds; out[1] = c->report.bwd_rounds;
	out[2] = c->report.fwd_tiles; out[3] = c->report.bwd_tiles;
	out[4] = c->report.merged; out[5] = c->report.recounted;
	return PSMC_HIP_OK;
}

void unpack_factored(const double *h, int n, double *sums, double *E, double *LL)
{
	if (sums) memcpy(sums, h, sizeof(double) * 5 * n);
	if (E) memcpy(E, h + (size_t)5 * n, sizeof(double) * 2 * n);
	if (LL) *LL = h[(size_t)7 * n];
}

extern "C" int psmc_hip_estep_factored(psmc_hip_ctx *c, const double *a, const double *e, const double *a0, double *sums,
                                       double *E, double *LL)
{
	if (!c || !a || !e || !a0) return fail(c, PSMC_HIP_EINVAL, "estep_factored: bad argument");
	if (c->mode != PSMC_HIP_MODE_FAST) return fail(c, PSMC_HIP_ENOTSUP, "estep_factored: fast mode only");
	HIPCHK(c, hipSetDevice(c->device));
	if (c->ns > 128 && c->wide_fast) return estep_factored_wide(c, a, e, a0, sums, E, LL);
	int rc;
	if ((rc = ensure_fast_buffers(c))) return rc;
	c->want_factored = true;
	rc = enqueue_fast(c, a, e, a0, c->d_stats, c->stream);
	c->want_factored = false;
	if (rc) return rc;
	if ((rc = read_warm(c, c->stream))) return rc;
	collect_timing(c);
	const int n = c->n;
	std::vector<double> h((size_t)7 * n + 1);
	HIPCHK(c, hipMemcpy(h.data(), c->d_stats, sizeof(double) * h.size(), hipMemcpyDeviceToHost));
	unpack_factored(h.data(), n, sums, E, LL);
	return PSMC_HIP_OK;
}

extern "C" int psmc_hip_estep_factored_device(psmc_hip_ctx *c, const double *a, const double *e, const double *a0, void *d_stats, void *stream)
{
	if (!c || !a || !e || !a0 || !d_stats) return fail(c, PSMC_HIP_EINVAL, "estep_factored_device: bad argument");
	if (c->mode != PSMC_HIP_MODE_FAST) return fail(c, PSMC_HIP_ENOTSUP, "estep_factored_device: fast mode only");
	HIPCHK(c, hipSetDevice(c->device));
	c->timing_valid = false;
	if (c->ns > 128 && c->wide_fast) return estep_wide_fast(c, a, e, a0, (double *)d_stats, (hipStream_t)stream);
	c->want_factored = true;
	const int rc = enqueue_fast(c, a, e, a0, (double *)d_stats, (hipStream_t)stream);
	c->want_factored = false;
	return rc;
}

extern "C" int psmc_hip_fast_info(psmc_hip_ctx *c, int out[8])
{
	if (!c || !out) return PSMC_HIP_EINVAL;
	if (c->wf_ran) {
		const int nc = (int)c->wf_chunks.size();
		out[0] = 1; out[1] = c->wf_T; out[2] = nc; out[3] = nc; out[4] = 3; out[5] = 0; out[6] = 1; out[7] = 0;
		return PSMC_HIP_OK;
	}
	out[0] = c->use_struct ? 1 : 0; out[1] = c->chunk_used; out[2] = c->use_struct ? c->n_items_f : (int)c->chunks.size();
	out[3] = c->use_struct ? c->n_items_b : (int)c->chunks.size();
	out[4] = c->last_fused; out[5] = c->last_ckpt; out[6] = c->timing_two_launches ? 2 : 1; out[7] = c->merge1_used;
	return PSMC_HIP_OK;
}

extern "C" int psmc_hip_fast_plan(psmc_hip_ctx *c, double out[8])
{
	if (!c || !out) return PSMC_HIP_EINVAL;
	if (c->plan_dirty || c->chunks.empty()) return fail(c, PSMC_HIP_ESTATE, "fast_plan: no current plan (run a fast E-step first)");
	const int nc = (int)c->chunks.size();
	double sf = 0, sb = 0, mf = 0, mb = 0; int nf = 0, nb = 0, gf = 0, gb = 0;
	for (int b = 0; b < nc; ++b) {
		const Chunk &ch = c->chunks[b];
		if (c->glue_f[b]) ++gf; else if (!(ch.flags & CHUNK_ANCHOR_F)) { sf += ch.wf; mf = std::max(mf, (double)ch.wf); ++nf; }
		if (c->glue_b[b]) ++gb; else if (!(ch.flags & (CHUNK_ANCHOR_B | CHUNK_LAST))) { sb += ch.wb; mb = std::max(mb, (double)ch.wb); ++nb; }
	}
	out[0] = nc; out[1] = c->chunk_used; out[2] = nf ? sf / nf : 0.0; out[3] = nb ? sb / nb : 0.0; out[4] = mf; out[5] = mb; out[6] = gf; out[7] = gb;
	return PSMC_HIP_OK;
}

int estep_fast(psmc_hip_ctx *c, const double *a, const double *e, const double *a0, double *A, double *E,
                      double *A0, double *LL, double *chk)
{
	const int n = c->n;
	int rc = enqueue_fast(c, a, e, a0, c->d_stats, c->stream);
	if (rc) return rc;
	if ((rc = read_warm(c, c->stream))) return rc;
	collect_timing(c);
	std::vector<double> h((size_t)n * n + 2 * n + 1);
	HIPCHK(c, hipMemcpy(h.data(), c->d_stats, sizeof(double) * h.size(), hipMemcpyDeviceToHost));
	if (A) memcpy(A, h.data(), sizeof(double) * n * n);
	if (E) memcpy(E, h.data() + (size_t)n * n, sizeof(double) * 2 * n);
	if (LL) *LL = h[(size_t)n * n + 2 * n];
	if (A0) memset(A0, 0, sizeof(double) * n);
	if (chk) for (size_t i = 0; i < c->sel.size(); ++i) chk[i] = 1.0;
	return PSMC_HIP_OK;
}

extern "C" int psmcdbg_check_bentry(psmc_hip_ctx *c)
{
	if (!c || c->ns != 64 || !c->d_bentry || !c->d_ftiles) return -1;
	(void)hipSetDevice(c->device);
	(void)hipDeviceSynchronize();
	const int nc = (int)c->chunks.size();
	const int ga = (c->n_list_a + 3) / 4, gb = (c->n_list_b + 3) / 4, ng = ga + gb;
	std::vector<int> tl(4 * (size_t)ng), tf(nc), tb(nc);
	const std::vector<Chunk> &ch = c->chunks;
	(void)hipMemcpy(tl.data(), c->d_ftiles, sizeof(int) * tl.size(), hipMemcpyDeviceToHost);
	(void)hipMemcpy(tf.data(), c->d_touch, sizeof(int) * tf.size(), hipMemcpyDeviceToHost);
	(void)hipMemcpy(tb.data(), c->d_touch + nc, sizeof(int) * tb.size(), hipMemcpyDeviceToHost);
	const double *d_e = c->d_par + 4 * 4096;
	{
			std::vector<double> ha(64 * 64), he(3 * 64), hb((size_t)nc * 64), hx((size_t)nc * 64);
			(void)hipMemcpy(ha.data(), c->d_par, sizeof(double) * ha.size(), hipMemcpyDeviceToHost);
			(void)hipMemcpy(he.data(), d_e, sizeof(double) * he.size(), hipMemcpyDeviceToHost);
			(void)hipMemcpy(hb.data(), c->d_bentry, sizeof(double) * hb.size(), hipMemcpyDeviceToHost);
			(void)hipMemcpy(hx.data(), c->d_bexit, sizeof(double) * hx.size(), hipMemcpyDeviceToHost);
			for (int k = 0; k < 64; ++k) he[128 + k] = 1.0;
			std::vector<int> from_above(nc, 0), in_list(nc, 0);
			for (size_t i = 0; i < tl.size(); ++i) if (tl[i] >= 0) { from_above[tl[i] & ~(1 << 30)] = (tl[i] >> 30) & 1; in_list[tl[i] & ~(1 << 30)] = i < 4 * (size_t)ga ? 1 : 2; }
			for (int b0 = 0; b0 < nc;) {
				int b1 = b0; while (b1 + 1 < nc && ch[b1 + 1].off == ch[b0].off) ++b1;
				const int L = ch[b0].L;
				std::vector<uint8_t> o(L);
				(void)hipMemcpy(o.data(), c->d_obs + ch[b0].off, (size_t)L, hipMemcpyDeviceToHost);
				std::vector<double> bt(64), y(64);
				for (int k = 0; k < 64; ++k) bt[k] = he[(o[L - 1] & 3) * 64 + k];
				int b = b1;
				for (int pp = L - 1; pp >= 1; --pp) {
					while (b >= b0 && std::min(ch[b].hi, L - 1) < ch[b].lo) --b;
					if (b >= b0 && pp == std::min(ch[b].hi, L - 1)) {
						double sx = 0, sy = 0, num = 0, den = 0;
						for (int k = 0; k < 64; ++k) { sx += hb[(size_t)b * 64 + k]; sy += bt[k]; }
						for (int k = 0; k < 64; ++k) { num = std::max(num, std::fabs(hb[(size_t)b * 64 + k] / sx - bt[k] / sy)); den = std::max(den, bt[k] / sy); }
						if (!(num / den < 1e-9))
							fprintf(stderr, "[psmc_hip] RECHECK bentry of tile %d (lo %d hi %d L %d list %d from_above %d tf %d tb %d; above: tf %d tb %d list %d) off by %.2e, sum %.3e; rounds %d/%d\n",
							        b, ch[b].lo, ch[b].hi, L, in_list[b], from_above[b], tf[b], tb[b], b + 1 <= b1 ? tf[b + 1] : -1, b + 1 <= b1 ? tb[b + 1] : -1, b + 1 <= b1 ? in_list[b + 1] : -1, num / den, sx,
							        c->report.fwd_rounds, c->report.bwd_rounds);
						--b;
					}
					double tot = 0;
					for (int k = 0; k < 64; ++k) { double acc = 0; for (int l = 0; l < 64; ++l) acc += ha[k * 64 + l] * bt[l]; y[k] = acc; }
					for (int k = 0; k < 64; ++k) { bt[k] = he[(o[pp - 1] & 3) * 64 + k] * y[k]; tot += bt[k]; }
					for (int k = 0; k < 64; ++k) bt[k] /= tot;
				}
				b0 = b1 + 1;
			}
		}
	return 0;
}
```

psmc_amd/csrc/estep_struct.hip:

```cpp
#include <hip/hip_runtime.h>
#include "wave_prims.h"
#include "struct_prims.h"
#include "psmc_hip_internal.h"

namespace psmc {

#ifdef PSMC_TRACE_SWEEP
__device__ unsigned long long g_trace_f[4 * 16384], g_trace_b[4 * 16384], g_trace_w[4 * 16384];
__device__ __forceinline__ void trace_put(unsigned long long *t, int block, int slot, unsigned long long v) {
	if ((threadIdx.x & 63) == 0 && block < 16384) t[4 * block + slot] = v;
}
__device__ __forceinline__ unsigned long long trace_hw() {
	const unsigned hw = __builtin_amdgcn_s_getreg((31 << 11) | (0 << 6) | 4), xcc = __builtin_amdgcn_s_getreg((31 << 11) | (0 << 6) | 20);
	return (unsigned long long)hw | ((unsigned long long)(xcc & 0xf) << 32);
}
#define PSMC_TRACE(t, block, slot, v) trace_put(t, block, slot, v)
#else
#define PSMC_TRACE(t, block, slot, v) ((void)0)
#endif

template <int J> __device__ __forceinline__ int sym_of(unsigned w) { return (int)((w >> (8 * J)) & 3u); }
__device__ __forceinline__ unsigned sym_word(const uint4 sv, int g) { return g == 0 ? sv.x : (g == 1 ? sv.y : (g == 2 ? sv.z : sv.w)); }
__device__ __forceinline__ int64_t readlane_i64(int64_t v, int lane) {
	const unsigned lo = (unsigned)__builtin_amdgcn_readlane((int)(unsigned)v, lane);
// ... 414 lines not shown
			int mode = (base + 1 > cur.lo && base + 16 < cur.top) ? 1 : ((base + 1 > cur.top && base + 16 <= p_first) ? 2 : 0);
			if (walk && mode == 1) mode = 2;
			if (__all(mode == 1)) bwd_block<1, NPL, LPT>(sc, hm, lds_e, k0, m, sv, base, p_first, p_low, T, cur, x, bto, sbo, bentry, bexit);
			else if (__all(mode == 2)) bwd_block<2, NPL, LPT>(sc, hm, lds_e, k0, m, sv, base, p_first, p_low, T, cur, x, bto, sbo, bentry, bexit);
			else bwd_block<0, NPL, LPT>(sc, hm, lds_e, k0, m, sv, base, p_first, p_low, T, cur, x, bto, sbo, bentry, bexit);
		}
	}
#ifdef PSMC_TRACE_SWEEP
	if (trb) { PSMC_TRACE(g_trace_b, block, 2, wall_clock64()); PSMC_TRACE(g_trace_b, block, 1, __builtin_readcyclecounter() - trb_c0); }
#endif
}

template <bool REPAIR, int NPL, int LPT = 16>
__global__ __launch_bounds__(64) void k_bwd_struct(const double *__restrict__ sp, const double *__restrict__ e,
                                                     const uint8_t *__restrict__ obs, const Chunk *__restrict__ chunks,
                                                     const SweepItem *__restrict__ items, int n_items, int W, int T,
                                                     int flags, double *__restrict__ bt, double *__restrict__ sb,
                                                     double *__restrict__ bentry, double *__restrict__ bexit,
                                                     int *__restrict__ touch_b)
{
	bwd_struct_body<REPAIR, NPL, LPT>(blockIdx.x, sp, e, obs, chunks, items, n_items, W, T, flags, bt, sb, bentry, bexit, touch_b);
}

template <bool CK>
__global__ __launch_bounds__(64) void k_phase1_queue(const double *__restrict__ sp, const double *__restrict__ e,
                                                       const double *__restrict__ a0, const uint8_t *__restrict__ obs,
                                                       const Chunk *__restrict__ chunks, const SweepItem *__restrict__ items_f, int n_f,
                                                       const SweepItem *__restrict__ items_b, int n_b, int W, int T, int flags_f,
                                                       int flags_b, double *__restrict__ f, double *__restrict__ invd,
                                                       double *__restrict__ entry, double *__restrict__ bt, double *__restrict__ sb,
                                                       double *__restrict__ bentry, double *__restrict__ bexit, int *__restrict__ touch_f,
                                                       int *__restrict__ touch_b, const int *__restrict__ q, int n_q,
                                                       int *__restrict__ head, int *__restrict__ started, const FwdCtl ctl)
{
	announce_start(started);
	for (;;) {
		int i = 0;
		if (threadIdx.x == 0) i = atomicAdd(head, 1);
		i = __builtin_amdgcn_readfirstlane(i);
		if (i >= n_q) break;
		const int w = q[i];
		__builtin_amdgcn_s_setprio(0);
		if ((w & 1) == 0)
			fwd_struct_body<false, 4, CK>(w >> 1, sp, e, a0, obs, chunks, items_f, n_f, W, T, flags_f, f, invd, entry, touch_f, ctl);
		else
			bwd_struct_body<false, 4>(w >> 1, sp, e, obs, chunks, items_b, n_b, W, T, flags_b, bt, sb, bentry, bexit, touch_b);
	}
}

template <int NPL>
__global__ __launch_bounds__(64) void k_walk_struct(const double *__restrict__ sp, const double *__restrict__ e,
                                                      const double *__restrict__ a0, const uint8_t *__restrict__ obs,
                                                      const Chunk *__restrict__ chunks, const SweepItem *__restrict__ items_f,
                                                      int n_f, const SweepItem *__restrict__ items_b, int n_b, int W, int T,
                                                      double *__restrict__ entry, double *__restrict__ bentry,
                                                      double *__restrict__ bexit, int *__restrict__ started)
{
	announce_start(started);
	const int nbf = (n_f + 3) / 4;
	if ((int)blockIdx.x < nbf)
		fwd_struct_body<false, NPL>(blockIdx.x, sp, e, a0, obs, chunks, items_f, n_f, W, T, SWEEP_WALK, nullptr, nullptr, entry, nullptr);
	else
		bwd_struct_body<false, NPL>(blockIdx.x - nbf, sp, e, obs, chunks, items_b, n_b, W, T, SWEEP_WALK, nullptr, nullptr, bentry, bexit,
		                       nullptr);
}

__device__ __forceinline__ double walk_ev(int sym, double e0, double e1) { return sym == 0 ? e0 : (sym == 1 ? e1 : 1.0); }

__global__ __launch_bounds__(64) void k_walk1_struct(const double *__restrict__ sp, const double *__restrict__ e,
                                                       const double *__restrict__ a0, const uint8_t *__restrict__ obs,
                                                       const Chunk *__restrict__ chunks, const SweepItem *__restrict__ items_f,
                                                       int n_f, const SweepItem *__restrict__ items_b, int n_b, int W, int T,
                                                       double *__restrict__ entry, double *__restrict__ bentry,
                                                       double *__restrict__ bexit, int *__restrict__ started)
{
	const int lane = threadIdx.x, block = (int)blockIdx.x;
	announce_start(started);
#ifdef PSMC_TRACE_SWEEP
	PSMC_TRACE(g_trace_w, block, 0, wall_clock64()); PSMC_TRACE(g_trace_w, block, 3, trace_hw());
	struct TraceEnd { int b; __device__ ~TraceEnd() { if (threadIdx.x == 0 && b < 16384) g_trace_w[4 * b + 2] = wall_clock64(); } } trace_end{block};
#endif
	__builtin_amdgcn_s_setprio(3);
	const WaveScanMasks wm = wave_scan_masks(lane);
	const double e0 = e[lane], e1 = e[64 + lane];
	if (block < n_f) {
		const SweepItem it = items_f[block];
		const Chunk c = chunks[it.first];
		const bool warm_only = it.count <= 0;
		const int thru = warm_only ? -it.count : it.count;
		const int p_last = thru == 0 ? c.lo - 1 : chunks[it.first + thru - 1].hi;
		const uint8_t *o = obs + c.off;
		StructPar1 s1; s1.mS = sp[lane]; s1.wS = sp[128 + lane]; s1.mP = sp[64 + lane]; s1.wP = sp[192 + lane]; s1.dd = sp[256 + lane];
		double x = a0[lane];
		int p_first;
		const int ws = max(1, c.lo - chunk_warm_f(c, W));
		if (ws == 1) { x *= walk_ev((int)o[0] & 3, e0, e1); p_first = 2; } else p_first = ws;
		int tile = c.lo >= p_first ? it.first : it.first + 1, next_lo = c.lo >= p_first ? c.lo : c.lo + T;
		const int g_first = (p_first - 1) >> 2, g_last = (p_last - 1) >> 2;
		unsigned w = *reinterpret_cast<const unsigned *>(o + 4 * g_first);
		for (int g = g_first; g <= g_last; ++g) {
			const unsigned wn = *reinterpret_cast<const unsigned *>(o + 4 * min(g + 1, g_last));
#pragma unroll
			for (int j = 0; j < 4; ++j) {
				const int p = 4 * g + j + 1;
				if (p < p_first || p > p_last) continue;
				if (p == next_lo) { entry[(int64_t)tile * 64 + lane] = x; ++tile; next_lo += T; }
				double ev = walk_ev((int)((w >> (8 * j)) & 3u), e0, e1);
				if (j == 3) ev *= rcp_newton(first_lane_f64(wave_sum_nat(x)));
				x = struct_step1(s1, x, wm) * ev;
			}
			w = wn;
		}
		if (warm_only) entry[(int64_t)(it.first + thru) * 64 + lane] = x;
	} else {
		const SweepItem it = items_b[block - n_f];
		const bool warm_only = it.count == 0;
		int tile = it.first + max(it.count, 1) - 1;
		const Chunk c = chunks[tile];
		int lo = c.lo, top = min(c.hi, c.L - 1);
		const int L = c.L, p_low = warm_only ? top + 1 : chunks[it.first + 1].lo;
		if (top < lo) return;
		const uint8_t *o = obs + c.off;
		StructPar1 s1; s1.mS = sp[192 + lane]; s1.wS = sp[64 + lane]; s1.mP = sp[128 + lane]; s1.wP = sp[lane]; s1.dd = sp[256 + lane];
		const int q = min(c.hi + chunk_warm_b(c, W) + 1, L);
		double x = walk_ev((int)o[q - 1] & 3, e0, e1);
		const int p_first = q - 1;
		const int g_first = (p_first - 1) >> 2, g_last = (p_low - 1) >> 2;
		unsigned w = *reinterpret_cast<const unsigned *>(o + 4 * g_first);
		for (int g = g_first; g >= g_last; --g) {
			const unsigned wn = *reinterpret_cast<const unsigned *>(o + 4 * max(g - 1, g_last));
#pragma unroll
			for (int j = 3; j >= 0; --j) {
				const int p = 4 * g + j + 1;
				if (p > p_first || p < p_low) continue;
				double ev = walk_ev((int)((w >> (8 * j)) & 3u), e0, e1);
				if (j == 3) ev *= rcp_newton(first_lane_f64(wave_sum_nat(x)));
				if (p == top) bentry[(int64_t)tile * 64 + lane] = x;
				x = struct_step1(s1, x, wm) * ev;
				if (p == lo) { bexit[(int64_t)tile * 64 + lane] = x; --tile; top = lo - 1; lo -= T; }
			}
			w = wn;
		}
		if (warm_only || it.count > 1) bentry[(int64_t)tile * 64 + lane] = x;
	}
}

struct KcTile { int tile, dir; };
__host__ __device__ inline void kc_range(const Chunk &c, int dir, int &lo, int &top)
{
	const bool fwd = dir == 0;
	top = fwd ? c.hi : min(c.hi, c.L - 1);
	lo = fwd ? c.lo : min(((c.lo + 3) & ~3) + 1, top + 1);
}

template <int NPL>
__global__ __launch_bounds__(64) void k_kcol_struct(const double *__restrict__ sp, const double *__restrict__ e,
                                                      const uint8_t *__restrict__ obs, const Chunk *__restrict__ chunks,
                                                      const KcTile *__restrict__ kc, const int *__restrict__ uniq, double *__restrict__ Kcol,
                                                      double *__restrict__ Kexp)
{
	constexpr int S = 16 * NPL, BPT = S / 4;
	__shared__ double lds_e[4 * S];
	const int lane = threadIdx.x, m = lane & 15, k0 = NPL * m;
	fill_lds_e<NPL, 16>(lds_e, e, lane);
	__syncthreads();
	const int j = blockIdx.x / BPT, col = 4 * (blockIdx.x % BPT) + (lane >> 4);
	__builtin_amdgcn_s_setprio(2);
	const KcTile kt = kc[uniq[j]];
	const Chunk c = chunks[kt.tile];
	const bool fwd = kt.dir == 0;
	const int top = fwd ? c.hi : min(c.hi, c.L - 1);
	const int lo = fwd ? c.lo : min(((c.lo + 3) & ~3) + 1, top + 1);
	const uint8_t *o = obs + c.off;
	StructParN<NPL> sc;
	load_struct_par<NPL>(sp, k0, fwd, sc);
	double x[NPL];
#pragma unroll
	for (int i = 0; i < NPL; ++i) x[i] = (k0 + i == col) ? 1.0 : 0.0;
	int E = 0;
	const int n = top - lo + 1;
	for (int q = 0; q < n; ++q) {
		const int p = fwd ? lo + q : top - q;
		const int sym = (int)o[p - 1] & 3;
		double ev[NPL];
		ev_load<NPL>(lds_e + sym * S, k0, ev);
		if ((p & 3) == 0) {
			const double s = row_sum16(lane_sum<NPL>(x));
			const int ex = s > 0.0 ? __builtin_amdgcn_frexp_exp(s) : 0;
#pragma unroll
			for (int i = 0; i < NPL; ++i) x[i] = __builtin_amdgcn_ldexp(x[i], -ex);
			E += ex;
		}
		struct_step<NPL>(sc, x);
#pragma unroll
		for (int i = 0; i < NPL; ++i) x[i] *= ev[i];
	}
	storeN<NPL>(Kcol + ((int64_t)j * S + col) * S + k0, x);
	if (m == 0) Kexp[(int64_t)j * S + col] = (double)E;
}

template <int NQ>
__global__ __launch_bounds__(64 * NQ) void k_kcol2_struct(const double *__restrict__ kcc, const uint8_t *__restrict__ obs,
                                                            const Chunk *__restrict__ chunks, const KcTile *__restrict__ kc, const int *__restrict__ uniq,
                                                            double *__restrict__ Kcol, double *__restrict__ Kexp, int sub, int prio)
{
	constexpr int S = 32 * NQ, NCG = S / 64, KD = 11 * S;
	__shared__ double xch[2][NQ][2][64];
	__shared__ double tab[KD];
	const int lane = threadIdx.x & 63;
	const int w = __builtin_amdgcn_readfirstlane((int)(threadIdx.x >> 6));
	const int j = (int)blockIdx.x / NCG, cg = (int)blockIdx.x % NCG, jt = j / sub, js = j % sub;
	const int col = 64 * cg + lane;
	if (prio >= 2) __builtin_amdgcn_s_setprio(2); else if (prio == 1) __builtin_amdgcn_s_setprio(1);
	const KcTile kt = kc[uniq[jt]];
	const Chunk c = chunks[kt.tile];
	const bool fwd = kt.dir == 0;
	for (int i = threadIdx.x; i < KD; i += 64 * NQ) tab[i] = kcc[(fwd ? 0 : KD) + i];
	__syncthreads();
	int top, lo;
	kc_range(c, kt.dir, lo, top);
	const uint8_t *o = obs + c.off;
	const double *cc = tab + 32 * w;
	double x[32];
#pragma unroll
	for (int k = 0; k < 32; ++k) x[k] = (32 * w + k == col) ? 1.0 : 0.0;
	int E = 0;
	const int n = max(top - lo + 1, 0);
	const int q0 = (int)((int64_t)n * js / sub), q1 = (int)((int64_t)n * (js + 1) / sub);
	for (int q = q0; q < q1; ++q) {
		const int p = fwd ? lo + q : top - q;
		const int sym = min((int)o[p - 1] & 3, 2);
		const double *ce = cc + 2 * S + sym * 3 * S;
		double y[32], sS = 0.0, sP = 0.0;
#pragma unroll
		for (int k = 31; k >= 0; --k) { sS = __builtin_fma(x[k], cc[k], sS); y[k] = ce[k] * sS; }
#pragma unroll
		for (int k = 0; k < 32; ++k) {
			sP = __builtin_fma(x[k], cc[S + k], sP);
			y[k] = __builtin_fma(ce[2 * S + k], x[k], __builtin_fma(ce[S + k], sP, y[k]));
		}
		xch[q & 1][w][0][lane] = sS; xch[q & 1][w][1][lane] = sP;
		__syncthreads();
		if constexpr (NQ == 2) {
			const double S0 = xch[q & 1][0][0][lane], S1 = xch[q & 1][1][0][lane], P0 = xch[q & 1][0][1][lane], P1 = xch[q & 1][1][1][lane];
			const double T = w == 0 ? S1 : P0;
			const double *cz = ce + (w == 0 ? 0 : S);
			if ((p & 3) == 0) {
				const double mag = (S0 + S1) + (P0 + P1);
				const int ex = mag > 0.0 ? __builtin_amdgcn_frexp_exp(mag) : 0;
				const double sc = __builtin_amdgcn_ldexp(1.0, -ex);
#pragma unroll
				for (int k = 0; k < 32; ++k) x[k] = __builtin_fma(cz[k], T, y[k]) * sc;
				E += ex;
			} else {
#pragma unroll
				for (int k = 0; k < 32; ++k) x[k] = __builtin_fma(cz[k], T, y[k]);
			}
		} else {
			double Ts = 0.0, Tp = 0.0, mag = 0.0;
#pragma unroll
			for (int v = 0; v < NQ; ++v) {
				const double Sv = xch[q & 1][v][0][lane], Pv = xch[q & 1][v][1][lane];
				Ts += v > w ? Sv : 0.0; Tp += v < w ? Pv : 0.0; mag += Sv + Pv;
			}
			double sc = 1.0;
			if ((p & 3) == 0) {
				const int ex = mag > 0.0 ? __builtin_amdgcn_frexp_exp(mag) : 0;
				sc = __builtin_amdgcn_ldexp(1.0, -ex);
				E += ex;
			}
#pragma unroll
			for (int k = 0; k < 32; ++k) x[k] = __builtin_fma(ce[k], Ts, __builtin_fma(ce[S + k], Tp, y[k])) * sc;
		}
	}
	double *out = Kcol + ((int64_t)j * S + col) * S + 32 * w;
#pragma unroll
	for (int k = 0; k < 32; ++k) out[k] = x[k];
	if (w == 0) Kexp[(int64_t)j * S + col] = (double)E;
}

__device__ __forceinline__ double wave_max_f64(double v) {
#pragma unroll
	for (int m = 32; m >= 1; m >>= 1) v = fmax(v, __shfl_xor(v, m, 64));
	return v;
}
struct KcRun { int first, count, kc0, pad; };

template <int PER>
__device__ __forceinline__ void struct_step1n(const StructPar1 (&c)[PER], double (&x)[PER], const WaveScanMasks &m)
{
	if constexpr (PER == 1) { x[0] = struct_step1(c[0], x[0], m); }
	else {
		const double s1 = wave_suffix_incl(x[1] * c[1].mS, m), s0 = wave_suffix_incl(x[0] * c[0].mS, m);
		const double p0 = wave_prefix_incl_bc(x[0] * c[0].mP), p1 = wave_prefix_incl_bc(x[1] * c[1].mP);
		const double tot1 = readlane_f64(s1, 0), tot0 = readlane_f64(p0, 63);
		const double y0 = __builtin_fma(c[0].wS, s0 + tot1, __builtin_fma(c[0].wP, p0, c[0].dd * x[0]));
		const double y1 = __builtin_fma(c[1].wS, s1, __builtin_fma(c[1].wP, p1 + tot0, c[1].dd * x[1]));
		x[0] = y0; x[1] = y1;
	}
}

template <int PER>
__global__ __launch_bounds__(64 * (PER == 1 ? 2 : 8)) void k_kchain_struct(const KcRun *__restrict__ runs, int n_f, const int *__restrict__ kslot,
                                                        const double *__restrict__ Kcol,
                                                        const double *__restrict__ Kexp, const double *__restrict__ sp,
                                                        const double *__restrict__ e, const uint8_t *__restrict__ obs,
                                                        const Chunk *__restrict__ chunks, double *__restrict__ entry,
                                                        double *__restrict__ bentry, int sub)
{
	constexpr int S = 64 * PER, RW = 32 / PER, NW = S / RW;
	__shared__ double part[2][NW][S];
	const int lane = threadIdx.x & 63;
	const int w = __builtin_amdgcn_readfirstlane((int)(threadIdx.x >> 6));
	__builtin_amdgcn_s_setprio(3);
	const bool fwd = (int)blockIdx.x < n_f;
	const KcRun r = runs[blockIdx.x];
	double *vec = fwd ? entry : bentry;
	int t = fwd ? r.first : r.first + r.count - 1;
	double x[PER];
	const WaveScanMasks wm = wave_scan_masks(lane);
	StructPar1 s1[PER];
	double e0[PER], e1[PER];
#pragma unroll
	for (int q = 0; q < PER; ++q) {
		const int k = lane + 64 * q;
		x[q] = vec[(int64_t)t * S + k];
		s1[q].mS = sp[3 * S + k]; s1[q].wS = sp[S + k]; s1[q].mP = sp[2 * S + k]; s1[q].wP = sp[k]; s1[q].dd = sp[4 * S + k];
		e0[q] = e[k]; e1[q] = e[S + k];
	}
	const int n_mats = (r.count - 1) * sub;
	const int row0 = RW * w, src_h = row0 >> 6, src_l = row0 & 63;
	double ma[RW][PER], mb[RW][PER], ea[PER], eb[PER];
	auto load = [&](int j, double (&m)[RW][PER], double (&ex)[PER]) {
		const int64_t kb = ((int64_t)kslot[r.kc0 + j / sub] * sub + j % sub) * S;
#pragma unroll
		for (int i = 0; i < RW; ++i)
#pragma unroll
			for (int h = 0; h < PER; ++h) m[i][h] = Kcol[(kb + row0 + i) * S + lane + 64 * h];
#pragma unroll
		for (int h = 0; h < PER; ++h) ex[h] = Kexp[kb + lane + 64 * h];
	};
	auto product = [&](int j, const double (&m)[RW][PER], const double (&ex)[PER]) {
		double xs[PER], y[PER], em = -1e300;
#pragma unroll
		for (int h = 0; h < PER; ++h) em = fmax(em, x[h] > 0.0 ? ex[h] : -1e300);
		const double emax = wave_max_f64(em);
#pragma unroll
		for (int h = 0; h < PER; ++h) { xs[h] = x[h] > 0.0 ? __builtin_amdgcn_ldexp(x[h], (int)(ex[h] - emax)) : 0.0; y[h] = 0.0; }
		double src = xs[0];
		if constexpr (PER == 2) src = src_h ? xs[1] : xs[0];
#pragma unroll
		for (int i = 0; i < RW; ++i) {
			const double v = readlane_f64(src, src_l + i);
#pragma unroll
			for (int h = 0; h < PER; ++h) y[h] = __builtin_fma(v, m[i][h], y[h]);
		}
		double (*pp)[S] = part[j & 1];
#pragma unroll
		for (int h = 0; h < PER; ++h) pp[w][lane + 64 * h] = y[h];
		__syncthreads();
#pragma unroll
		for (int h = 0; h < PER; ++h) {
			double tsum = pp[0][lane + 64 * h];
#pragma unroll
			for (int v = 1; v < NW; ++v) tsum += pp[v][lane + 64 * h];
			y[h] = tsum;
		}
		double tot = y[0];
		if constexpr (PER == 2) tot += y[1];
		const double inv = rcp_newton(first_lane_f64(wave_sum_nat(tot)));
#pragma unroll
		for (int h = 0; h < PER; ++h) x[h] = y[h] * inv;
	};
	auto tile_done = [&]() {
		double y[PER];
#pragma unroll
		for (int h = 0; h < PER; ++h) y[h] = x[h];
		if (!fwd) {
			const Chunk c = chunks[t];
			const int top = min(c.hi, c.L - 1), ps = min((c.lo + 3) & ~3, top);
			const uint8_t *o = obs + c.off;
			for (int pq = ps; pq >= c.lo; --pq) {
				const int sym = (int)o[pq - 1] & 3;
				double ev[PER];
#pragma unroll
				for (int h = 0; h < PER; ++h) ev[h] = walk_ev(sym, e0[h], e1[h]);
				if ((pq & 3) == 0) {
					double tot = y[0];
					if constexpr (PER == 2) tot += y[1];
					const double inv = rcp_newton(first_lane_f64(wave_sum_nat(tot)));
#pragma unroll
					for (int h = 0; h < PER; ++h) ev[h] *= inv;
				}
				struct_step1n<PER>(s1, y, wm);
#pragma unroll
				for (int h = 0; h < PER; ++h) y[h] *= ev[h];
			}
		}
		t += fwd ? 1 : -1;
#pragma unroll
		for (int h = 0; h < PER; ++h) { if (w == 0) vec[(int64_t)t * S + lane + 64 * h] = y[h]; x[h] = y[h]; }
	};
	if (n_mats > 0) load(0, ma, ea);
	for (int j = 0; j < n_mats; j += 2) {
		if (j + 1 < n_mats) load(j + 1, mb, eb);
		product(j, ma, ea);
		if (j % sub == sub - 1) tile_done();
		if (j + 1 >= n_mats) break;
		if (j + 2 < n_mats) load(j + 2, ma, ea);
		product(j + 1, mb, eb);
		if ((j + 1) % sub == sub - 1) tile_done();
	}
}

template <int NPL, bool CK, int LPT = 16>
__global__ __launch_bounds__(64) void k_sweep_struct(const double *__restrict__ sp, const double *__restrict__ e,
                                                       const double *__restrict__ a0, const uint8_t *__restrict__ obs,
                                                       const Chunk *__restrict__ chunks, const SweepItem *__restrict__ items_f,
                                                       int n_f, const SweepItem *__restrict__ items_b, int n_b, int W, int T,
                                                       int flags_f, int flags_b, double *__restrict__ f, double *__restrict__ invd,
                                                       double *__restrict__ entry, double *__restrict__ bt,
                                                       double *__restrict__ sb, double *__restrict__ bentry,
                                                       double *__restrict__ bexit, int *__restrict__ started, const double *__restrict__ prevx)
{
	announce_start(started);
	constexpr int R = 64 / LPT;
	const int nbf = (n_f + R - 1) / R, nbb = (n_b + R - 1) / R, both = 2 * min(nbf, nbb), b = blockIdx.x;
	bool fwd; int blk;
	if (!(flags_b & SWEEP_ALTERNATE)) { fwd = b < nbf; blk = fwd ? b : b - nbf; }
	else if (b < both) { fwd = (b & 1) == 0; blk = b >> 1; }
	else { fwd = nbf > nbb; blk = b - both + min(nbf, nbb); }
	if (fwd) fwd_struct_body<false, NPL, CK, LPT>(blk, sp, e, a0, obs, chunks, items_f, n_f, W, T, flags_f, f, invd, entry, nullptr, FwdCtl{prevx, 0.0, nullptr, nullptr, nullptr, nullptr});
	else bwd_struct_body<false, NPL, LPT>(blk, sp, e, obs, chunks, items_b, n_b, W, T, flags_b, bt, sb, bentry, bexit, nullptr);
}

__global__ __launch_bounds__(64) void k_compact(const int *__restrict__ dirty, int n, SweepItem *__restrict__ out,
                                                  SweepItem *__restrict__ host_out, int *__restrict__ host_cnt)
{
	const int lane = threadIdx.x;
	int base = 0;
	for (int i0 = 0; i0 < n; i0 += 64) {
		const int i = i0 + lane;
		const bool d = i < n && dirty[i] != 0;
		const unsigned long long mask = __ballot(d);
		if (d) {
			SweepItem s; s.first = i; s.count = 1;
			const int at = base + __popcll(mask & ((1ull << lane) - 1ull));
			out[at] = s;
			if (host_out) host_out[at] = s;
		}
		base += __popcll(mask);
	}
	if (lane == 0) *host_cnt = base;
	__threadfence_system();
}

void launch_fwd_struct(const EstepLaunch &p, hipStream_t st, int which, int first, int n_items)
{
	if (n_items <= 0) return;
	const bool l8 = p.lanes8 && p.ns == 64 && which == 0;
	const dim3 g(l8 ? (n_items + 7) / 8 : (n_items + 3) / 4), b(64);
	const SweepItem *items = (const SweepItem *)(which == 1 ? p.d_ritems_f : (which == 3 || which == 7 ? p.d_members_f : (which == 6 ? p.d_fix_f : p.d_items_f))) + first;
	const bool fixp = which == 6 || which == 7;
	const int flags = (which == 3 ? (SWEEP_FROM_ENTRY | SWEEP_NO_TOUCH) : 0)
	                  | (p.ckpt ? SWEEP_CKPT : 0) | (which == 0 && p.coarse > 1 ? SWEEP_COARSE : 0) | (fixp ? SWEEP_MERGE : 0);
	const FwdCtl ctl = {which == 0 ? p.d_prevx : nullptr, p.tol, fixp ? p.m_mis : nullptr, fixp ? p.m_mlen : nullptr, p.d_fmerge, p.d_finv};
#define PSMC_LF(REP, NPL, CK) hipLaunchKernelGGL((k_fwd_struct<REP, NPL, CK>), g, b, 0, st, p.d_sp, p.d_e, p.d_a0, p.d_obs, p.d_chunks, \
		items, n_items, p.warmup, p.tile_len, flags, p.d_f, p.d_s, p.d_entry, p.d_touch_f, which == 0 && p.d_gate ? p.d_gate + 1 : nullptr, ctl)
	const bool rep = which != 0;
	if (l8) {
#define PSMC_LF8(CK) hipLaunchKernelGGL((k_fwd_struct<false, 8, CK, 8>), g, b, 0, st, p.d_sp, p.d_e, p.d_a0, p.d_obs, p.d_chunks, \
		items, n_items, p.warmup, p.tile_len, flags, p.d_f, p.d_s, p.d_entry, p.d_touch_f, p.d_gate ? p.d_gate + 1 : nullptr, ctl)
		if (p.ckpt) PSMC_LF8(true); else PSMC_LF8(false);
#undef PSMC_LF8
	} else if (p.ns == 128) { if (rep) PSMC_LF(true, 8, false); else PSMC_LF(false, 8, false); }
	else if (p.ckpt) { if (rep) PSMC_LF(true, 4, true); else PSMC_LF(false, 4, true); }
	else { if (rep) PSMC_LF(true, 4, false); else PSMC_LF(false, 4, false); }
	PSMC_DBG("launch_fwd_struct", which, first, n_items);
#undef PSMC_LF
}
void launch_bwd_struct(const EstepLaunch &p, hipStream_t st, int which, int first, int n_items)
{
	if (n_items <= 0) return;
	const bool l8 = p.lanes8 && p.ns == 64 && which == 4;
	const dim3 g(l8 ? (n_items + 7) / 8 : (n_items + 3) / 4), b(64);
	const SweepItem *items = (const SweepItem *)(which == 1 || which == 5 ? p.d_ritems_b : (which == 3 ? p.d_members_b : p.d_items_b)) + first;
	const int flags = which == 5 ? SWEEP_WALK : (which == 3 ? (SWEEP_FROM_ENTRY | SWEEP_NO_TOUCH) : (which == 4 ? (p.coarse > 1 ? (SWEEP_WALK | SWEEP_COARSE) : SWEEP_TOP_ONLY) : 0));
#define PSMC_LB(REP, NPL) hipLaunchKernelGGL((k_bwd_struct<REP, NPL>), g, b, 0, st, p.d_sp, p.d_e, p.d_obs, p.d_chunks, items, \
		n_items, p.warmup, p.tile_len, flags, p.d_b, p.d_sb, p.d_bentry, p.d_bexit, p.d_touch_b)
	const bool rep = !(which == 0 || which == 4);
	if (l8)
		hipLaunchKernelGGL((k_bwd_struct<false, 8, 8>), g, b, 0, st, p.d_sp, p.d_e, p.d_obs, p.d_chunks, items, n_items, p.warmup, p.tile_len, flags,
		                   p.d_b, p.d_sb, p.d_bentry, p.d_bexit, p.d_touch_b);
	else if (p.ns == 128) { if (rep) PSMC_LB(true, 8); else PSMC_LB(false, 8); }
	else { if (rep) PSMC_LB(true, 4); else PSMC_LB(false, 4); }
	PSMC_DBG("launch_bwd_struct", which, first, n_items);
#undef PSMC_LB
}
void launch_phase1_queue(const EstepLaunch &p, hipStream_t st, int ff, int nf, int fb, int nb)
{
	if (p.n_queue <= 0 || p.q_grid <= 0) return;
	const int flags_f = (p.ckpt ? SWEEP_CKPT : 0) | (p.coarse > 1 ? SWEEP_COARSE : 0);
	const int flags_b = p.coarse > 1 ? (SWEEP_WALK | SWEEP_COARSE) : SWEEP_TOP_ONLY;
	const FwdCtl ctl = {p.d_prevx, p.tol, nullptr, nullptr, p.d_fmerge, p.d_finv};
#define PSMC_LQ(CK) hipLaunchKernelGGL(k_phase1_queue<CK>, dim3(p.q_grid), dim3(64), 0, st, p.d_sp, p.d_e, p.d_a0, p.d_obs, p.d_chunks, \
		(const SweepItem *)p.d_items_f + ff, nf, (const SweepItem *)p.d_items_b + fb, nb, p.warmup, p.tile_len, flags_f, flags_b, p.d_f, p.d_s, \
		p.d_entry, p.d_b, p.d_sb, p.d_bentry, p.d_bexit, p.d_touch_f, p.d_touch_b, p.d_queue, p.n_queue, p.d_qhead, p.d_gate ? p.d_gate + 1 : nullptr, ctl)
	if (p.ckpt) PSMC_LQ(true); else PSMC_LQ(false);
#undef PSMC_LQ
	PSMC_DBG("launch_phase1_queue", nf, nb, p.q_grid);
}
void launch_compact(const EstepLaunch &p, hipStream_t st, bool bwd)
{
	hipLaunchKernelGGL(k_compact, dim3(1), dim3(64), 0, st, bwd ? p.d_dirty_b : p.d_dirty, p.n_chunks,
	                   (SweepItem *)(bwd ? p.d_ritems_b : p.d_ritems_f),
	                   (SweepItem *)(p.m_ritems ? p.m_ritems + (size_t)(bwd ? 1 : 0) * 2 * p.n_chunks : nullptr), p.m_cnt + (bwd ? 1 : 0));
	PSMC_DBG("verify + launch_compact", bwd, p.n_chunks, 0);
}
void launch_sweeps(const EstepLaunch &p, hipStream_t st, int ff, int nf, int fb, int nb, bool top_only)
{
	const bool l8 = p.lanes8 && p.ns == 64 && top_only;
	const int nblk = l8 ? (nf + 7) / 8 + (nb + 7) / 8 : (nf + 3) / 4 + (nb + 3) / 4;
	if (nblk <= 0) return;
	const int co = top_only && p.coarse > 1 ? SWEEP_COARSE : 0;
	const int flags_f = (p.ckpt ? SWEEP_CKPT : 0) | co,
	          flags_b = (top_only ? (co ? SWEEP_WALK | co : SWEEP_TOP_ONLY) : 0) | (top_only && p.merge_order ? SWEEP_MERGED : SWEEP_ALTERNATE);
#define PSMC_LS(NPL, CK) hipLaunchKernelGGL((k_sweep_struct<NPL, CK>), dim3(nblk), dim3(64), 0, st, p.d_sp, p.d_e, p.d_a0, p.d_obs, p.d_chunks, \
		(const SweepItem *)p.d_items_f + ff, nf, (const SweepItem *)p.d_items_b + fb, nb, p.warmup, p.tile_len, flags_f, flags_b, \
		p.d_f, p.d_s, p.d_entry, p.d_b, p.d_sb, p.d_bentry, p.d_bexit, p.d_gate ? p.d_gate + 1 : nullptr, p.d_prevx)
#define PSMC_LS8(CK) hipLaunchKernelGGL((k_sweep_struct<8, CK, 8>), dim3(nblk), dim3(64), 0, st, p.d_sp, p.d_e, p.d_a0, p.d_obs, p.d_chunks, \
		(const SweepItem *)p.d_items_f + ff, nf, (const SweepItem *)p.d_items_b + fb, nb, p.warmup, p.tile_len, flags_f, flags_b, \
		p.d_f, p.d_s, p.d_entry, p.d_b, p.d_sb, p.d_bentry, p.d_bexit, p.d_gate ? p.d_gate + 1 : nullptr, p.d_prevx)
	if (l8) { if (p.ckpt) PSMC_LS8(true); else PSMC_LS8(false); }
	else if (p.ns == 128) PSMC_LS(8, false); else if (p.ckpt) PSMC_LS(4, true); else PSMC_LS(4, false);
#undef PSMC_LS8
	PSMC_DBG("launch_sweeps", nf, nb, top_only);
#undef PSMC_LS
}
__global__ __launch_bounds__(64) void k_gather_prev(const Chunk *__restrict__ chunks, const SweepItem *__restrict__ items, int S, const double *__restrict__ f,
                                                      const double *__restrict__ a0, double *__restrict__ prevx, int ck)
{
	const SweepItem it = items[blockIdx.x];
	const Chunk c = chunks[it.first];
	const int ws = max(1, c.lo - c.wf);
	const bool have = ws > 1 && !(ck && ((ws - 1) & 7));
	for (int k = threadIdx.x; k < S; k += 64) {
		double v = a0[k];
		if (have) { const double t = f[(c.off + ws - 2) * S + k]; v = (t > 0.0 && t < 1e300) ? t : v; }
		prevx[(int64_t)it.first * S + k] = v;
	}
}
void launch_gather_prev(const EstepLaunch &p, hipStream_t st, int first, int n_items, double *prevx)
{
	if (n_items <= 0) return;
	hipLaunchKernelGGL(k_gather_prev, dim3(n_items), dim3(64), 0, st, p.d_chunks, (const SweepItem *)p.d_items_f + first, p.ns, p.d_f, p.d_a0, prevx, p.ckpt);
}

__global__ __launch_bounds__(64) void k_tile_allmiss(const uint8_t *__restrict__ obs, const Chunk *__restrict__ chunks, int *__restrict__ flags)
{
	const Chunk c = chunks[blockIdx.x];
	const uint8_t *o = obs + c.off;
	int bad = 0;
	for (int p = c.lo + (int)threadIdx.x; p <= c.hi; p += 64) bad |= ((int)o[p - 1] & 3) != 2;
	const int any_bad = __any(bad);
	if (threadIdx.x == 0) flags[blockIdx.x] = any_bad ? 0 : 1;
}
int launch_tile_allmiss(hipStream_t st, const uint8_t *d_obs, const Chunk *d_chunks, int n_chunks, int *d_flags)
{
	if (n_chunks <= 0) return 0;
	hipLaunchKernelGGL(k_tile_allmiss, dim3(n_chunks), dim3(64), 0, st, d_obs, d_chunks, d_flags);
	return (int)hipGetLastError();
}

void launch_kchain(const EstepLaunch &p, hipStream_t st_cols, hipStream_t st_chain, hipEvent_t ev_cols)
{
	if (p.n_kc <= 0) return;
	if (p.ns == 128)
		hipLaunchKernelGGL(k_kcol_struct<8>, dim3(p.n_kuniq * 32), dim3(64), 0, st_cols, p.d_sp, p.d_e, p.d_obs, p.d_chunks,
		                   (const KcTile *)p.d_kc, p.d_kuniq, p.d_Kcol, p.d_Kexp);
	else
		hipLaunchKernelGGL(k_kcol2_struct<2>, dim3(p.n_kuniq * p.kc_sub), dim3(128), 0, st_cols, p.d_kcc, p.d_obs, p.d_chunks, (const KcTile *)p.d_kc, p.d_kuniq,
		                   p.d_Kcol, p.d_Kexp, p.kc_sub, p.kcol_prio);
	if (st_cols != st_chain) { (void)hipEventRecord(ev_cols, st_cols); (void)hipStreamWaitEvent(st_chain, ev_cols, 0); }
	if (p.ns == 128)
		hipLaunchKernelGGL(k_kchain_struct<2>, dim3(p.n_chain_f + p.n_chain_b), dim3(512), 0, st_chain, (const KcRun *)p.d_kruns, p.n_chain_f, p.d_kslot,
		                   p.d_Kcol, p.d_Kexp, p.d_sp, p.d_e, p.d_obs, p.d_chunks, p.d_entry, p.d_bentry, p.kc_sub);
	else
		hipLaunchKernelGGL(k_kchain_struct<1>, dim3(p.n_chain_f + p.n_chain_b), dim3(128), 0, st_chain, (const KcRun *)p.d_kruns, p.n_chain_f, p.d_kslot,
		                   p.d_Kcol, p.d_Kexp, p.d_sp, p.d_e, p.d_obs, p.d_chunks, p.d_entry, p.d_bentry, p.kc_sub);
	PSMC_DBG("launch_kchain", p.n_kc, p.n_chain_f, p.n_chain_b);
}
int walk_blocks(const EstepLaunch &p) { return p.ns == 64 ? p.n_wl_f + p.n_wl_b : (p.n_wl_f + 3) / 4 + (p.n_wl_b + 3) / 4; }
void launch_walks(const EstepLaunch &p, hipStream_t st)
{
	if (p.n_wl_f + p.n_wl_b <= 0) return;
	if (p.ns == 64) {
		hipLaunchKernelGGL(k_walk1_struct, dim3(p.n_wl_f + p.n_wl_b), dim3(64), 0, st, p.d_sp, p.d_e, p.d_a0, p.d_obs, p.d_chunks,
		                   (const SweepItem *)p.d_wl_f, p.n_wl_f, (const SweepItem *)p.d_wl_b, p.n_wl_b, p.warmup,
		                   p.tile_len, p.d_entry, p.d_bentry, p.d_bexit, p.d_gate);
		PSMC_DBG("launch_walks", p.n_wl_f, p.n_wl_b, 0);
		return;
	}
	hipLaunchKernelGGL(k_walk_struct<8>, dim3((p.n_wl_f + 3) / 4 + (p.n_wl_b + 3) / 4), dim3(64), 0, st, p.d_sp, p.d_e, p.d_a0, p.d_obs, p.d_chunks,
	                   (const SweepItem *)p.d_wl_f, p.n_wl_f, (const SweepItem *)p.d_wl_b, p.n_wl_b, p.warmup, p.tile_len,
	                   p.d_entry, p.d_bentry, p.d_bexit, p.d_gate);
	PSMC_DBG("launch_walks (four per wave)", p.n_wl_f, p.n_wl_b, 0);
}

}

#ifdef PSMC_TRACE_SWEEP
extern "C" int psmc_hip_debug_trace(int which, unsigned long long *out, int n)
{
	if (n > 16384) n = 16384;
	return (int)(which == 0 ? hipMemcpyFromSymbol(out, HIP_SYMBOL(psmc::g_trace_f), sizeof(unsigned long long) * 4 * n)
	             : which == 1 ? hipMemcpyFromSymbol(out, HIP_SYMBOL(psmc::g_trace_b), sizeof(unsigned long long) * 4 * n)
	                          : hipMemcpyFromSymbol(out, HIP_SYMBOL(psmc::g_trace_w), sizeof(unsigned long long) * 4 * n));
}
#endif
```

psmc_amd/csrc/psmc_hip_ctx.h:

```cpp
#pragma once
#include <hip/hip_runtime.h>
#include <math.h>
#include <stdio.h>
#include <stdlib.h>
#include <string.h>
#include <algorithm>
#include <atomic>
#include <chrono>
#include <string>
#include <thread>
#include <vector>
#include "psmc_hip.h"
#include "psmc_hip_internal.h"

using namespace psmc;

#define HMM_TINY_H 1e-25

constexpr int DEC_NONE = 0;
constexpr int DEC_FAST = 1;
constexpr int DEC_EXACT = 2;
constexpr int DEC_NO_BT = 3;
constexpr int DEC_MERGED = 4;
constexpr int DEC_WIDE = 5;
constexpr int WD_NONE = 0;
constexpr int WD_OK = 1;
constexpr int WD_FAILED = 2;

struct psmc_hip_ctx {
	int n = 0, ns = 64, device = 0, mode = PSMC_HIP_MODE_EXACT;
	std::string err;
	int chunk = 0, warmup = 3072, max_rounds = 4096, rep_impl = -1, n_sub = 6, target_waves = 1536, overlap = 1;
	double warm_tol = 1e-12;
	int struct_opt = 1;
	bool struct_tiles_set = false;
	int struct_tiles = 8192;
	bool use_struct = false, planned_struct = false;
	int last_fused = 0, last_ckpt = 0;
	int dec_kind = 0; unsigned long long dec_serial = 0;
	bool want_factored = false;
	int kc_sub = 4;
	int kcol_prio = 2;
	int two_phase = -1;
	int two_phase_used = 2;
	int merge1 = -1;
	int merge1_used = 0;
	int merge_order = -1;
	int lanes8 = -1;
	int gate = -1;
	int *d_gate = nullptr;
	int phase1 = -1;
	int phase1_waves = 2;
	int *d_queue = nullptr;
	size_t queue_cap = 0; int n_queue = 0;
	int coarse = -1;
	int coarse_used = 1, items_coarse = -1;
	bool warm_shift_set = false, kc_sub_set = false;
	int warm_shift_used = 1, kc_sub_used = 4;
	int kc_div = 16;
	int kc_min = -1;
	int n_wl_f = 0, n_wl_b = 0, n_kc = 0, n_chain_f = 0, n_chain_b = 0, n_singles_b = 0;
	double *d_Kcol = nullptr; size_t kcol_cap = 0;
	hipStream_t stream5 = nullptr;
	int ckpt = 1;
	int fuse = 1;
	int fuse128 = 2;
	int count_group = 4;
	int merge = 0;
	int adapt = 0;
	int prev_start = 0;
	int *h_mlen = nullptr, *m_mlen = nullptr;
	double *h_mis = nullptr, *m_mis = nullptr;
	double *d_prevx = nullptr, *d_finv = nullptr;
	std::vector<int> order_f;
	int n_fix_f = 0;
	bool merge_used = false;
	Chunk *h_chunks = nullptr; size_t h_chunks_cap = 0;
	bool prev_ok = false;
	unsigned long long prev_serial = 0, tab_serial = 0;
	const double *prev_f = nullptr; int prev_ckpt = 0;
	int learn = 1;
	int warm_shift = 1;
	bool chunks_dirty = false;
	int group_cap = 131072;
	int *d_items = nullptr;
	int *h_ritems = nullptr;
	int *m_ritems = nullptr, *m_cnt = nullptr;
	std::vector<uint8_t> glue_f, glue_b;
	std::vector<uint8_t> gap;
	int gap_tiles = 1;
	int n_kuniq = 0;
	std::vector<int> flagged_f, flagged_b;
	bool items_dirty = true;
	int n_items_f = 0, n_items_b = 0;
	int n_sub_used = 6;
	int n_seg = 0;
	std::vector<int32_t> L;
	std::vector<int64_t> off;
	int64_t total = 0;
	bool obs_borrowed = false;
	uint8_t *d_obs = nullptr;
	int64_t *d_seg_off = nullptr;
	int32_t *d_seg_len = nullptr;
	std::vector<int32_t> sel;
	std::vector<int32_t> work;
	std::vector<int32_t> sel2work;
	std::vector<int32_t> mult;
	int32_t *d_work = nullptr;
	bool plan_dirty = true;
	double *h_par = nullptr, *d_par = nullptr;
	size_t par_len = 0;
	static constexpr size_t PAR_LEN = 2 * 16384 + 3 * 128 + 128 + 3 * 128 + 5 * 128 + 2 * 11 * 128;
	static constexpr size_t RE128_OFF = 2 * 16384 + 3 * 128 + 128, SP128_OFF = RE128_OFF + 3 * 128, KCC128_OFF = SP128_OFF + 5 * 128;
	static constexpr size_t SP_OFF = 4 * 4096 + 192 + 64 + 192;
	static constexpr size_t KCC_OFF = SP_OFF + 5 * 64;
	double *d_f = nullptr, *d_b = nullptr, *d_s = nullptr, *d_sb = nullptr;
	int64_t tab_bins = 0; bool have_b = false;
	double *d_segA = nullptr, *d_segE = nullptr, *d_segA0 = nullptr, *d_chk = nullptr;
	int seg_cap = 0;
	std::vector<double> h_segA, h_segE, h_segA0, h_chk, h_s;
	std::vector<Chunk> chunks;
	Chunk *d_chunks = nullptr;
	int chunk_cap = 0, chunk_used = 0;
	double *d_entry = nullptr, *d_bentry = nullptr, *d_bexit = nullptr, *d_Cpart = nullptr, *d_Epart = nullptr,
	       *d_LLpart = nullptr;
	size_t cpart_cap = 0;
	int *d_dirty = nullptr, *d_cnt = nullptr, *h_cnt = nullptr, *d_touch = nullptr;
	hipStream_t stream2 = nullptr, stream3 = nullptr, stream4 = nullptr;
	hipEvent_t evx[14] = {nullptr, nullptr, nullptr, nullptr, nullptr, nullptr, nullptr, nullptr, nullptr, nullptr, nullptr, nullptr, nullptr, nullptr};
	bool timing_two_launches = false;
	int n_long_f = 0, n_long_b = 0, n_mem_f = 0, n_mem_b = 0;
	int n_B_b = 0, n_list_a = 0, n_list_b = 0;
	int items_two_phase = -1;
	int runs_late = 1;
	bool runs_in_b = false;
	int *d_ftiles = nullptr;
	FastReport report = {0, 0, 0, 0, 1, 0, 0};
	double *d_stage = nullptr, *d_stats = nullptr;
	unsigned long long *d_warm = nullptr;
	double warm_err[2] = {0, 0};
	hipStream_t stream = nullptr;
	hipEvent_t ev[10] = {nullptr, nullptr, nullptr, nullptr, nullptr, nullptr, nullptr, nullptr, nullptr, nullptr};
	double last_ms[7] = {0, 0, 0, 0, 0, 0, 0};
	bool timing_valid = false;
	int64_t batch_bins = 0;
	int exact_refwd = -1;
	int32_t *d_bw_seg = nullptr, *d_bw_par = nullptr; int64_t *d_bw_tab = nullptr; size_t bw_cap = 0;
	double *d_bpar = nullptr; size_t bpar_cap = 0;
	int *d_cu_mask = nullptr;
	double *d_lkp = nullptr; size_t lkp_cap = 0; std::vector<double> h_lkp;
	int64_t *d_lkoff = nullptr; size_t lkoff_cap = 0;
	double *d_s_all = nullptr; size_t s_all_cap = 0;
	int batch_sort = 1;
	int batch_tailfill = 1;
	int batch_major = 1;
	int batch_first = 0;
	double *d_b2 = nullptr; int64_t b2_bins = 0, b2_alloc = 0;
	int64_t reserved_cap = 0;
	int reserved_refwd = -1;
	int cu_first = 0, cu_count = 0;
	int last_batch_groups = 0;
	bool tables_batch = false;
	psmc_hip_ctx *x_twin = nullptr;
	int n_exact_fallbacks = 0;
	psmc_hip_ctx *parent = nullptr;
	std::vector<psmc_hip_ctx *> kids;
	int share_learn = 1;
	int share_T = 0;
	std::vector<std::vector<uint8_t>> sh_glue_f, sh_glue_b;
	std::vector<std::vector<int32_t>> sh_wf, sh_wb;
	std::vector<int32_t> chunk_seg, chunk_idx;
	double dbg_acc[8] = {0, 0, 0, 0, 0, 0, 0, 0};
	int wide_fast = 0;
	bool wf_ran = false;
	std::vector<Chunk> wf_chunks;
	Chunk *d_wf_chunks = nullptr;
	int wf_cap = 0, wf_T = 0, wf_W = 0;
	bool warmup_set = false;
	double *d_wf_X = nullptr, *d_wf_inv = nullptr; int64_t wf_bins = 0;
	double *d_wf_par = nullptr, *h_wf_par = nullptr;
	double *d_wf_entry = nullptr, *d_wf_bentry = nullptr, *d_wf_bexit = nullptr, *d_wf_part = nullptr, *d_wf_ll = nullptr;
	int *d_wf_dirty = nullptr, *d_wf_list = nullptr;
	int wide_decode = 0;
	int wd_kind = 0; unsigned long long wd_serial = 0, wd_sel = 0, sel_serial = 0;
};
inline double dbg_now() { return std::chrono::duration<double>(std::chrono::steady_clock::now().time_since_epoch()).count(); }
inline psmc_hip_ctx *dbg_root(psmc_hip_ctx *c) { return c->parent ? c->parent : c; }

inline int fail(psmc_hip_ctx *c, int code, const char *what, hipError_t e = hipSuccess)
{
	if (c) {
		c->err = what;
		if (e != hipSuccess) { c->err += ": "; c->err += hipGetErrorString(e); }
	}
	return code;
}
#define HIPCHK(c, call)                                                     \
	do {                                                                    \
		hipError_t e__ = (call);                                            \
		if (e__ != hipSuccess) return fail((c), PSMC_HIP_EDEVICE, #call, e__); \
	} while (0)

template <class T> inline int dev_alloc(psmc_hip_ctx *c, T **p, size_t n)
{
	if (*p) { (void)hipFree(*p); *p = nullptr; }
	if (n == 0) n = 1;
	hipError_t e = hipMalloc((void **)p, n * sizeof(T));
	if (e != hipSuccess) { *p = nullptr; return fail(c, PSMC_HIP_ENOMEM, "hipMalloc", e); }
	static const char *poison = getenv("PSMC_HIP_POISON");
	static int poison_count = 0;
	if (poison) {
		(void)hipMemset(*p, strcmp(poison, "vary") == 0 ? 0x3B + (poison_count++ % 8) : 0xFF, n * sizeof(T));
		(void)hipDeviceSynchronize();
	}
	return 0;
}

int  set_segments_common(psmc_hip_ctx *c, int n_seg, const int32_t *L);
bool fill_params(const psmc_hip_ctx *c, const double *a, const double *e, const double *a0, double *dst);
int  stage_params(psmc_hip_ctx *c, const double *a, const double *e, const double *a0, hipStream_t st);
int  ensure_tables(psmc_hip_ctx *c, bool need_b, int64_t want_bins = 0, bool need_f = true);
bool fused_counts(const psmc_hip_ctx *c);
bool kcol2_on(const psmc_hip_ctx *c);
void fill_common(psmc_hip_ctx *c, EstepLaunch &p, hipStream_t st, const double *par_base = nullptr);
void collect_timing(psmc_hip_ctx *c);
double host_lk(const double *s, int L);
int  ensure_seg_outputs(psmc_hip_ctx *c, int nw);
int  estep_exact(psmc_hip_ctx *c, const double *a, const double *e, const double *a0, double *A, double *E, double *A0, double *LL, double *chk);
int  ensure_fast_buffers(psmc_hip_ctx *c);
int  auto_tile_len(const psmc_hip_ctx *c, int64_t bins, size_t n_work, bool structured);
int  enqueue_fast(psmc_hip_ctx *c, const double *a, const double *e, const double *a0, double *d_out, hipStream_t st);
int  read_warm(psmc_hip_ctx *c, hipStream_t st);
void unpack_factored(const double *h, int n, double *sums, double *E, double *LL);
bool factor_structure(int n, int S, const double *a, double *sp);
void free_wide_fast(psmc_hip_ctx *c);
int  estep_wide_fast(psmc_hip_ctx *c, const double *a, const double *e, const double *a0, double *d_out, hipStream_t st);
int  estep_factored_wide(psmc_hip_ctx *c, const double *a, const double *e, const double *a0, double *sums, double *E, double *LL);
int  estep_fast(psmc_hip_ctx *c, const double *a, const double *e, const double *a0, double *A, double *E, double *A0, double *LL, double *chk);
```

psmc_amd/csrc/psmc_hip_internal.h:

```cpp
#pragma once
#include <cstdio>
#include <cstdlib>
#include <hip/hip_runtime.h>
#include <stdint.h>
#include <vector>

namespace psmc {

constexpr int NS = 64;
constexpr int NORM_EVERY = 4;
constexpr int STATS_LEN = NS * NS + 3 * NS + 1;

struct Chunk {
	int64_t off;
	int32_t L;
	int32_t lo;
	int32_t hi;
	int32_t mult;
	int32_t flags;
	int32_t wf, wb;
};
__host__ __device__ inline int chunk_warm_f(const Chunk &c, int) { return c.wf; }
__host__ __device__ inline int chunk_warm_b(const Chunk &c, int) { return c.wb; }
constexpr int CHUNK_ANCHOR_F = 1;
constexpr int CHUNK_ANCHOR_B = 2;
constexpr int CHUNK_LAST = 4;

struct ExWork {
	const int32_t *seg;
	const int32_t *par;
	const int64_t *tab;
	const int64_t *tab_s;
	int n;
	int64_t par_stride;
};

struct FastReport { int fwd_rounds, bwd_rounds, fwd_tiles, bwd_tiles, converged, merged, recounted; };

struct EstepLaunch {
	hipStream_t stream, stream2, stream3;
	hipEvent_t evx[14];
	int overlap;
	int rep_impl, n_states;
	const int64_t *d_work_tab_s;
	int *d_cu_mask = nullptr;
	int exact_only;
	int exact_refwd;
	int ns;
	const double *d_a;
	const double *d_aeT;
	const double *d_e;
	const double *d_a0;
	const double *d_re;
	const double *d_sp;
	int structured;
	const double *d_kcc;
	int kc_sub;
	int kcol_prio;
	int fused;
	int ckpt;
	int merge_order;
	int merge1;
	const int *d_items_f, *d_items_b;
	int n_items_f, n_items_b, tile_len;
	int n_long_f, n_long_b;
	const int *d_members_f, *d_members_b;
	int n_mem_f, n_mem_b;
	int lanes8;
	int *d_gate;
	const int *d_queue; int n_queue;
	int q_grid; int *d_qhead;
	int coarse;
	const int *d_singles_b; int n_singles_b;
	int n_B_b;
	const int *d_ftiles; int n_list_a, n_list_b;
	int count_group;
	int runs_in_b;
	hipStream_t stream4, stream5;
	const int *d_wl_f, *d_wl_b; int n_wl_f, n_wl_b;
	const int *d_kc, *d_kruns; int n_kc, n_chain_f, n_chain_b;
	const int *d_kslot, *d_kuniq; int n_kuniq;
	double *d_Kcol, *d_Kexp;
	int *d_ritems_f, *d_ritems_b;
	int *h_ritems;
	int *m_ritems, *m_cnt;
	std::vector<int> *flagged_f, *flagged_b;
	const uint8_t *d_obs;
	const int64_t *d_seg_off;
	const int32_t *d_seg_len;
	const int32_t *d_work;
	int n_work;
	const int32_t *d_work_par; const int64_t *d_work_tab; int64_t par_stride; int work_align;
	double *d_f, *d_b, *d_s;
	double *d_segA, *d_segE, *d_segA0, *d_chk;
	const Chunk *d_chunks;
	int n_chunks, warmup, n_sub;
	double *d_entry, *d_bentry, *d_bexit;
	int *d_dirty, *d_dirty_b, *d_cnt, *h_cnt;
	int *d_touch_f, *d_touch_b;
	int merge;
	const int *d_fix_f; int n_fix_f;
	int *d_fmerge;
	double *d_finv;
	int *m_mlen, *h_mlen;
	double *m_mis;
	const double *d_prevx;
	double *d_sb;
	double tol; int max_rounds;
	double *d_Cpart;
	double *d_Epart;
	double *d_LLpart;
	double *d_stage;
	double *d_stats;
	unsigned long long *d_warm;
	double tiny_total;
	hipEvent_t ev[10];
};

inline bool dbg_sync_on() { static const bool on = getenv("PSMC_HIP_DEBUG_SYNC") != nullptr; return on; }
#define PSMC_DBG(NAME, A, B, C) do { if (psmc::dbg_sync_on()) { hipError_t e_ = hipDeviceSynchronize(); \
	fprintf(stderr, "[psmc_hip] %s(%d, %d, %d): %s\n", NAME, (int)(A), (int)(B), (int)(C), hipGetErrorString(e_)); fflush(stderr); } } while (0)

constexpr int RED_ROWS = 64;

int launch_exact(const EstepLaunch &p);
constexpr int LKP_DIV = 16, LKP_MIN = 64;
int launch_lk_products(hipStream_t st, const EstepLaunch &p, const double *d_s, const int64_t *d_lk_off, double *d_out);
int launch_exact_wide(const EstepLaunch &p);
int launch_post_decode_wide(hipStream_t st, const double *f, const double *b, const double *s, int64_t off, int L, int n, int S, int32_t *path, double *maxp);
int launch_post_full_wide(hipStream_t st, const double *a, const double *e, const uint8_t *obs, const double *f, const double *b, const double *s,
                          int64_t off, int L, int n, int S, double *post, double *recomb);
int launch_post_counts_wide(hipStream_t st, const double *f, const double *b, const double *s, int64_t off, int min_l, const int32_t *cnt1,
                            int n_cnt, int n, int S, double *cnt);
int launch_fast(const EstepLaunch &p, FastReport *rep);
void launch_fwd_struct(const EstepLaunch &p, hipStream_t st, int which, int first, int n_items);
void launch_bwd_struct(const EstepLaunch &p, hipStream_t st, int which, int first, int n_items);
void launch_compact(const EstepLaunch &p, hipStream_t st, bool bwd);
void launch_gather_prev(const EstepLaunch &p, hipStream_t st, int first, int n_items, double *prevx);
int launch_tile_allmiss(hipStream_t st, const uint8_t *d_obs, const Chunk *d_chunks, int n_chunks, int *d_flags);
void launch_walks(const EstepLaunch &p, hipStream_t st);
void launch_gate(hipStream_t st, const int *ctr, int want);
int walk_blocks(const EstepLaunch &p);
void launch_kchain(const EstepLaunch &p, hipStream_t st_cols, hipStream_t st_chain, hipEvent_t ev_cols);
void launch_sweeps(const EstepLaunch &p, hipStream_t st, int ff, int nf, int fb, int nb, bool top_only);
void launch_phase1_queue(const EstepLaunch &p, hipStream_t st, int ff, int nf, int fb, int nb);
void launch_bwd_count(const EstepLaunch &p, hipStream_t st, int list, bool redo, bool all_from_bentry = false);
void launch_bwd_acc(const EstepLaunch &p, hipStream_t st, int which, int first, int n);
void launch_reduce_factored(const EstepLaunch &p, hipStream_t st);
int launch_post_decode(hipStream_t st, const double *f, const double *b, const double *s, int64_t off, int L, int n,
                       int ns, int32_t *path, double *maxp);
int launch_post_full(hipStream_t st, const double *a, const double *e, const uint8_t *obs, const double *f, const double *b,
                     const double *s, int64_t off, int L, int n, int ns, double *post, double *recomb);
int launch_post_counts(hipStream_t st, const double *f, const double *b, const double *s, int64_t off, int min_l,
                       const int32_t *cnt1, int n_cnt, int n, int ns, double *cnt);
int launch_post_fast(hipStream_t st, const double *f, const double *b, const double *sb, const double *re, const double *a,
                     const uint8_t *obs, int64_t off, int L, int n, int ns, double *post, double *recomb, int32_t *path, double *maxp);
int launch_scales_fast(hipStream_t st, const double *f, const double *invd, const double *entry, const double *a0, const double *e,
                       const uint8_t *obs, int64_t off, int L, int T, int first, int ns, double *s);
int post_counts_fast_blocks(int min_l);
int launch_post_counts_fast(hipStream_t st, const double *f, const double *b, const double *re, const uint8_t *obs, int64_t off,
                            int L, int min_l, const int32_t *cnt1, int n_cnt, int n, int ns, double *part, double *cnt);
int run_selftest(hipStream_t stream, unsigned *d_flags);
int run_microbench(hipStream_t stream, double *d_out);
int run_pipe_probe(hipStream_t stream, double *d_out, int n_waves, unsigned mask, int rounds);
int run_pipe_probe2(hipStream_t stream, double *d_out, const int *kinds8, int rounds, const void *gsrc);
int run_place_probe(hipStream_t stream, double *d_out, int n_waves, int wpb, int steps);
int run_stream_probe(hipStream_t stream, const double *src, double *dst, size_t n);
int run_hbm_probe(hipStream_t stream, int which, double *a, double *b, size_t bytes);
int run_load_probe(hipStream_t stream, double *d_out, int n_waves, int steps);
int run_load_probe_st(hipStream_t stream, double *d_out, int n_waves, int steps, double *tbl, int store_steps, int mode);

}
```

psmc_amd/hip.py:

```python
import ctypes as C
import os
import numpy as np

MODE_EXACT = 0
MODE_FAST = 1

_HERE = os.path.dirname(os.path.abspath(__file__))
_LIB = None
_DIAG = None

_dp = C.POINTER(C.c_double)
_u8p = C.POINTER(C.c_uint8)
_i32p = C.POINTER(C.c_int32)
_i64p = C.POINTER(C.c_int64)

EXPORTS = [
    "psmc_hip_device_count", "psmc_hip_device_cus", "psmc_hip_set_cu_range", "psmc_hip_reserve_tables", "psmc_hip_create", "psmc_hip_destroy", "psmc_hip_strerror",
    "psmc_hip_last_error", "psmc_hip_set_option", "psmc_hip_load_segments",
    "psmc_hip_load_segments_device", "psmc_hip_select", "psmc_hip_estep",
    "psmc_hip_estep_segments", "psmc_hip_estep_batch", "psmc_hip_estep_batch_cb", "psmc_hip_reserve_batch_tables", "psmc_hip_batch_info", "psmc_hip_estep_device", "psmc_hip_fast_diag", "psmc_hip_fast_repairs", "psmc_hip_fast_info", "psmc_hip_estep_factored",
    "psmc_hip_get_tables", "psmc_hip_decode", "psmc_hip_posterior", "psmc_hip_post_counts", "psmc_hip_scales",
    "psmc_hip_group_selfcheck", "psmc_hip_fast_plan",
    "psmc_hip_group_create", "psmc_hip_group_destroy", "psmc_hip_group_last_error", "psmc_hip_group_set_option",
    "psmc_hip_group_load_segments", "psmc_hip_group_estep", "psmc_hip_group_estep_factored", "psmc_hip_group_info",
    "psmc_hip_group_route", "psmc_hip_estep_factored_device",
]

DIAG_EXPORTS = [
    "psmc_hip_selftest", "psmc_hip_last_timing", "psmc_hip_microbench", "psmc_hip_stream_probe", "psmc_hip_hbm_probe",
    "psmc_hip_load_probe", "psmc_hip_load_probe_st", "psmc_hip_pipe_probe", "psmc_hip_pipe_probe2", "psmc_hip_place_probe",
    "psmc_hip_cumask_probe",
]


class HipError(RuntimeError):
    pass


def lib_path():
    return os.environ.get("PSMC_HIP_LIB") or os.path.join(_HERE, "libpsmc_hip.so")


def _share_torch_hip_runtime():
    import sys
    if "torch" in sys.modules or os.environ.get("PSMC_HIP_SYSTEM_RUNTIME"):
        return
    try:
        import importlib.util
        spec = importlib.util.find_spec("torch")
        if spec is None or not spec.origin:
            return
        p = os.path.join(os.path.dirname(spec.origin), "lib", "libamdhip64.so")
        if os.path.exists(p):
            C.CDLL(p, mode=C.RTLD_GLOBAL)
    except Exception:
        pass


def load_library():
    global _LIB
    if _LIB is not None:
        return _LIB
    p = lib_path()
    if not os.path.exists(p):
        raise HipError("%s not built: run `make -C psmc_amd/csrc` (or __graft_entry__.build())" % p)
    _share_torch_hip_runtime()
    lib = C.CDLL(p)
    lib.psmc_hip_strerror.restype = C.c_char_p
    lib.psmc_hip_last_error.restype = C.c_char_p
    lib.psmc_hip_last_error.argtypes = [C.c_void_p]
    lib.psmc_hip_create.argtypes = [C.POINTER(C.c_void_p), C.c_int, C.c_int, C.c_int]
    lib.psmc_hip_destroy.argtypes = [C.c_void_p]
    lib.psmc_hip_destroy.restype = None
    lib.psmc_hip_set_option.argtypes = [C.c_void_p, C.c_char_p, C.c_double]
    lib.psmc_hip_load_segments.argtypes = [C.c_void_p, C.c_int, C.POINTER(_u8p), _i32p]
    lib.psmc_hip_load_segments_device.argtypes = [C.c_void_p, C.c_int, C.c_void_p, _i64p, _i32p]
    lib.psmc_hip_select.argtypes = [C.c_void_p, C.c_int, _i32p]
    lib.psmc_hip_set_cu_range.argtypes = [C.c_void_p, C.c_int, C.c_int]
    lib.psmc_hip_reserve_tables.argtypes = [C.c_void_p]
    lib.psmc_hip_device_cus.argtypes = [C.c_int]
    lib.psmc_hip_estep.argtypes = [C.c_void_p, _dp, _dp, _dp, _dp, _dp, _dp, _dp, _dp]
    lib.psmc_hip_estep_segments.argtypes = [C.c_void_p, _dp, _dp, _dp, _dp, _dp, _dp, _dp, _dp]
    lib.psmc_hip_estep_device.argtypes = [C.c_void_p, _dp, _dp, _dp, C.c_void_p, C.c_void_p]
    lib.psmc_hip_fast_diag.argtypes = [C.c_void_p, _dp, _dp, C.POINTER(C.c_int), C.POINTER(C.c_int)]
    lib.psmc_hip_fast_repairs.argtypes = [C.c_void_p, C.POINTER(C.c_int)]
    lib.psmc_hip_fast_info.argtypes = [C.c_void_p, C.POINTER(C.c_int)]
    lib.psmc_hip_get_tables.argtypes = [C.c_void_p, C.c_int, _dp, _dp, _dp]
    lib.psmc_hip_decode.argtypes = [C.c_void_p, C.c_int, _i32p, _dp]
    _LIB = lib
    return lib


def load_diag():
    global _DIAG
    if _DIAG is not None:
        return _DIAG
    load_library()
    p = os.path.join(os.path.dirname(lib_path()), "libpsmc_hip_diag.so")
    if not os.path.exists(p):
        raise HipError("%s not built: run `make -C psmc_amd/csrc`" % p)
    d = C.CDLL(p)
    d.psmc_hip_selftest.argtypes = [C.c_int]
    d.psmc_hip_last_timing.argtypes = [C.c_void_p, _dp]
    _DIAG = d
    return d


def _p(x):
    return x.ctypes.data_as(_dp) if x is not None else None


class HipEStep:

    def __init__(self, n_states, device=0, mode=MODE_FAST, **options):
        self.lib = load_library()
        if self.lib.psmc_hip_device_count() <= 0:
            raise HipError("no HIP device visible: libpsmc_hip needs an AMD GPU (no CPU fallback)")
        self.n = int(n_states)
        self.mode = mode
        h = C.c_void_p()
        rc = self.lib.psmc_hip_create(C.byref(h), self.n, int(device), int(mode))
        if rc != 0:
            raise HipError("psmc_hip_create: %s" % self.lib.psmc_hip_strerror(rc).decode())
        self.h = h
        self.n_seg = 0
        self.n_sel = 0
        self._keep = None
        for k, v in options.items():
            self.set_option(k, v)

    def _chk(self, rc, what):
        if rc != 0:
            raise HipError("%s: %s (%s)" % (what, self.lib.psmc_hip_strerror(rc).decode(),
                                            self.lib.psmc_hip_last_error(self.h).decode()))

    def close(self):
        if getattr(self, "h", None):
            self.lib.psmc_hip_destroy(self.h)
            self.h = None

    def __del__(self):
        try:
            self.close()
        except Exception:
            pass

    def set_option(self, key, value):
        self._chk(self.lib.psmc_hip_set_option(self.h, key.encode(), float(value)), "set_option(%s)" % key)

    def set_cu_range(self, first, count):
        self._chk(self.lib.psmc_hip_set_cu_range(self.h, int(first), int(count)), "set_cu_range")

    def reserve_tables(self):
        self._chk(self.lib.psmc_hip_reserve_tables(self.h), "reserve_tables")

    def reserve_batch_tables(self, max_bins):
        self.lib.psmc_hip_reserve_batch_tables.argtypes = [C.c_void_p, C.c_int64]
        self._chk(self.lib.psmc_hip_reserve_batch_tables(self.h, int(max_bins)), "reserve_batch_tables")

    def load_segments(self, segs):
        segs = [np.ascontiguousarray(s, dtype=np.uint8) for s in segs]
        n = len(segs)
        ptrs = (_u8p * n)(*[s.ctypes.data_as(_u8p) for s in segs])
        lens = np.array([len(s) for s in segs], dtype=np.int32)
        self._chk(self.lib.psmc_hip_load_segments(self.h, n, ptrs, lens.ctypes.data_as(_i32p)), "load_segments")
        self.n_seg = self.n_sel = n
        self.lens = lens

    def load_segments_device(self, d_obs_ptr, offsets, lens, keepalive=None):
        off = np.ascontiguousarray(offsets, dtype=np.int64)
        lens = np.ascontiguousarray(lens, dtype=np.int32)
        self._keep = keepalive
        self._chk(self.lib.psmc_hip_load_segments_device(self.h, len(lens), C.c_void_p(int(d_obs_ptr)),
                                                         off.ctypes.data_as(_i64p), lens.ctypes.data_as(_i32p)),
                  "load_segments_device")
        self.n_seg = self.n_sel = len(lens)
        self.lens = lens

    def select(self, idx):
        idx = np.ascontiguousarray(idx, dtype=np.int32)
        self._chk(self.lib.psmc_hip_select(self.h, len(idx), idx.ctypes.data_as(_i32p)), "select")
        self.n_sel = len(idx)

    def _params(self, a, e, a0):
        a = np.ascontiguousarray(a, dtype=np.float64)
        e = np.ascontiguousarray(np.asarray(e, dtype=np.float64)[:2])
        a0 = np.ascontiguousarray(a0, dtype=np.float64)
        assert a.shape == (self.n, self.n) and e.shape == (2, self.n) and a0.shape == (self.n,)
        return a, e, a0

    def estep(self, a, e, a0):
        a, e, a0 = self._params(a, e, a0)
        n = self.n
        A = np.zeros((n, n)); E = np.zeros((2, n)); A0 = np.zeros(n); LL = C.c_double(0)
        chk = np.zeros(self.n_sel)
        self._chk(self.lib.psmc_hip_estep(self.h, _p(a), _p(e), _p(a0), _p(A), _p(E), _p(A0), C.byref(LL), _p(chk)),
                  "estep")
        return dict(A=A, E=E, A0=A0, LL=LL.value, chk=chk)

    def estep_segments(self, a, e, a0):
        a, e, a0 = self._params(a, e, a0)
        n, ns = self.n, self.n_sel
        sA = np.zeros((ns, n, n)); sE = np.zeros((ns, 3, n)); sA0 = np.zeros((ns, n)); sLL = np.zeros(ns)
        chk = np.zeros(ns)
        self._chk(self.lib.psmc_hip_estep_segments(self.h, _p(a), _p(e), _p(a0), _p(sA), _p(sE), _p(sA0), _p(sLL),
                                                   _p(chk)), "estep_segments")
        return dict(seg_A=sA, seg_E=sE, seg_A0=sA0, seg_LL=sLL, chk=chk)

    def estep_batch(self, params, selections, want="A", on_done=None):
        R, n = len(params), self.n
        assert len(selections) == R
        a = np.ascontiguousarray(np.stack([np.asarray(p[0], dtype=np.float64) for p in params]))
        e = np.ascontiguousarray(np.stack([np.asarray(p[1], dtype=np.float64)[:2] for p in params]))
        a0 = np.ascontiguousarray(np.stack([np.asarray(p[2], dtype=np.float64) for p in params]))
        assert a.shape == (R, n, n) and e.shape == (R, 2, n) and a0.shape == (R, n)
        off = np.concatenate([[0], np.cumsum([len(x) for x in selections])]).astype(np.int32)
        idx = np.concatenate([np.asarray(x, dtype=np.int32) for x in selections]).astype(np.int32)
        A = np.zeros((R, n, n)) if want in ("A", "both") else None
        sums = np.zeros((R, 5, n)) if want in ("sums", "both") else None
        E = np.zeros((R, 2, n)); LL = np.zeros(R)
        out = dict(E=E, LL=LL)
        if A is not None:
            out["A"] = A
        if sums is not None:
            out["sums"] = sums
        if on_done is None:
            self.lib.psmc_hip_estep_batch.argtypes = [C.c_void_p, C.c_int, _dp, _dp, _dp, _i32p, _i32p, _dp, _dp, _dp, _dp]
            self._chk(self.lib.psmc_hip_estep_batch(self.h, R, _p(a), _p(e), _p(a0), off.ctypes.data_as(_i32p), idx.ctypes.data_as(_i32p),
                                                    _p(A), _p(sums), _p(E), _p(LL)), "estep_batch")
            return out
        fn_t = C.CFUNCTYPE(None, C.c_void_p, C.c_int, _i32p)
        cb = fn_t(lambda user, n_done, reps: on_done([int(reps[i]) for i in range(n_done)], out))
        self.lib.psmc_hip_estep_batch_cb.argtypes = [C.c_void_p, C.c_int, _dp, _dp, _dp, _i32p, _i32p, _dp, _dp, _dp, _dp, fn_t, C.c_void_p]
        self._chk(self.lib.psmc_hip_estep_batch_cb(self.h, R, _p(a), _p(e), _p(a0), off.ctypes.data_as(_i32p), idx.ctypes.data_as(_i32p),
                                                   _p(A), _p(sums), _p(E), _p(LL), cb, None), "estep_batch_cb")
        return out

    def batch_info(self):
        o = (C.c_int * 2)()
        self._chk(self.lib.psmc_hip_batch_info(self.h, o), "batch_info")
        return dict(groups=o[0], replicate_contexts=o[1])

    def estep_device(self, a, e, a0, d_stats_ptr, stream_ptr=0):
        a, e, a0 = self._params(a, e, a0)
        self._chk(self.lib.psmc_hip_estep_device(self.h, _p(a), _p(e), _p(a0), C.c_void_p(int(d_stats_ptr)),
                                                 C.c_void_p(int(stream_ptr))), "estep_device")

    def estep_factored(self, a, e, a0):
        a = np.ascontiguousarray(a, dtype=np.float64)
        e = np.ascontiguousarray(np.asarray(e, dtype=np.float64)[:2])
        a0 = np.ascontiguousarray(a0, dtype=np.float64)
        n = self.n
        sums = np.zeros((5, n)); E = np.zeros((2, n)); LL = C.c_double(0)
        self.lib.psmc_hip_estep_factored.argtypes = [C.c_void_p, _dp, _dp, _dp, _dp, _dp, C.POINTER(C.c_double)]
        self._chk(self.lib.psmc_hip_estep_factored(self.h, _p(a), _p(e), _p(a0), _p(sums), _p(E), C.byref(LL)), "estep_factored")
        return dict(sums=sums, E=E, LL=LL.value)

    def estep_factored_device(self, a, e, a0, d_stats_ptr, stream_ptr=0):
        a, e, a0 = self._params(a, e, a0)
        self.lib.psmc_hip_estep_factored_device.argtypes = [C.c_void_p, _dp, _dp, _dp, C.c_void_p, C.c_void_p]
        self._chk(self.lib.psmc_hip_estep_factored_device(self.h, _p(a), _p(e), _p(a0), C.c_void_p(int(d_stats_ptr)),
                                                          C.c_void_p(int(stream_ptr))), "estep_factored_device")

    def fast_diag(self):
        wf = C.c_double(0); wb = C.c_double(0); nc = C.c_int(0); wu = C.c_int(0)
        self._chk(self.lib.psmc_hip_fast_diag(self.h, C.byref(wf), C.byref(wb), C.byref(nc), C.byref(wu)), "fast_diag")
        rp = (C.c_int * 6)()
        self._chk(self.lib.psmc_hip_fast_repairs(self.h, rp), "fast_repairs")
        fi = (C.c_int * 8)()
        self._chk(self.lib.psmc_hip_fast_info(self.h, fi), "fast_info")
        return dict(warm_err_fwd=wf.value, warm_err_bwd=wb.value, n_chunks=nc.value, warmup=wu.value,
                    fwd_rounds=rp[0], bwd_rounds=rp[1], fwd_tiles=rp[2], bwd_tiles=rp[3], merged=rp[4], recounted=rp[5],
                    structured=bool(fi[0]), tile_len=fi[1], items_fwd=fi[2], items_bwd=fi[3], back_half=fi[4], ckpt=bool(fi[5]),
                    fused_launches=fi[6], merged_phase1=fi[7])

    def fast_plan(self):
        o = np.zeros(8)
        self.lib.psmc_hip_fast_plan.argtypes = [C.c_void_p, _dp]
        self._chk(self.lib.psmc_hip_fast_plan(self.h, _p(o)), "fast_plan")
        return dict(tiles=int(o[0]), tile_len=int(o[1]), warm_fwd_mean=o[2], warm_bwd_mean=o[3], warm_fwd_max=int(o[4]), warm_bwd_max=int(o[5]),
                    glued_fwd=int(o[6]), glued_bwd=int(o[7]))

    def tables(self, seg, want_b=True):
        L = int(self.lens[seg])
        f = np.zeros((L, self.n)); s = np.zeros(L)
        b = np.zeros((L, self.n)) if want_b else None
        self._chk(self.lib.psmc_hip_get_tables(self.h, int(seg), _p(f), _p(b), _p(s)), "get_tables")
        return f, b, s

    def decode(self, seg):
        L = int(self.lens[seg])
        path = np.zeros(L, dtype=np.int32); mp = np.zeros(L)
        self._chk(self.lib.psmc_hip_decode(self.h, int(seg), path.ctypes.data_as(_i32p), _p(mp)), "decode")
        return path, mp

    def posterior(self, seg, want_post=True, want_recomb=True):
        L = int(self.lens[seg])
        post = np.zeros((L, self.n)) if want_post else None
        rec = np.zeros(L) if want_recomb else None
        self.lib.psmc_hip_posterior.argtypes = [C.c_void_p, C.c_int, _dp, _dp]
        self._chk(self.lib.psmc_hip_posterior(self.h, int(seg), _p(post), _p(rec)), "posterior")
        return post, rec

    def post_counts(self, seg, cnt1, cnt):
        cnt1 = np.ascontiguousarray(cnt1, dtype=np.int32)
        assert cnt.dtype == np.float64 and cnt.flags.c_contiguous and cnt.shape == (self.n, cnt1.shape[1])
        self.lib.psmc_hip_post_counts.argtypes = [C.c_void_p, C.c_int, _i32p, C.c_int32, C.c_int32, _dp]
        self._chk(self.lib.psmc_hip_post_counts(self.h, int(seg), cnt1.ctypes.data_as(_i32p), cnt1.shape[0], cnt1.shape[1], _p(cnt)), "post_counts")
        return cnt

    def scales(self, seg):
        L = int(self.lens[seg])
        s = np.zeros(L)
        self.lib.psmc_hip_scales.argtypes = [C.c_void_p, C.c_int, _dp]
        self._chk(self.lib.psmc_hip_scales(self.h, int(seg), _p(s)), "scales")
        return s

    def timing(self):
        ms = np.zeros(7)
        self._chk(load_diag().psmc_hip_last_timing(self.h, _p(ms)), "last_timing")
        if self.mode == MODE_FAST:
            return dict(total=ms[0], chains=ms[1], tail=ms[2], expect=ms[3], reduce=ms[4], fwd_sweep=ms[5],
                        bwd_sweep=ms[6], forward=ms[1], backward=ms[2])
        return dict(total=ms[0], forward=ms[1], backward=ms[2], expect=ms[3], reduce=ms[4], fwd_sweep=0.0, bwd_sweep=0.0)


def selftest(device=0):
    lib = load_diag()
    return lib.psmc_hip_selftest(int(device))


MICROBENCH_NAMES = ["fmac_dpp dependent", "v_fma_f64 dependent", "v_add_f64 dependent", "fmac_dpp 4 chains (per op)",
                    "fmac_dpp 8 chains (per op)", "rep_rows_swap dependent", "rep_rows_bperm dependent",
                    "dpp_mov+add dependent", "v_rcp_f64 dependent", "mov_b64_dpp+mul dependent",
                    "v_mul_f64 8 indep (per op)", "f64 division dependent", "mfma_f64_16x16x4 dependent",
                    "mfma_f64_16x16x4 4 accumulators (per op)", "structured step dependent (per step)",
                    "structured step + emission + norm/4 (per step)", "cycle counter MHz (vs 100 MHz wall clock)",
                    "one-state-per-lane structured step + emission + norm/4 (per step)",
                    "4 mfma_f64 + 32 independent v_fma_f64 (per group; 4 mfma alone: 4x the 4-accumulator figure)",
                    "4 mfma_f64 + 32 v_mov_b32_dpp (per group)"]


def microbench(device=0):
    lib = load_diag()
    out = np.zeros(len(MICROBENCH_NAMES))
    lib.psmc_hip_microbench.argtypes = [C.c_int, _dp, C.c_int]
    rc = lib.psmc_hip_microbench(int(device), _p(out), len(MICROBENCH_NAMES))
    if rc != 0:
        raise HipError("microbench: %s" % load_library().psmc_hip_strerror(rc).decode())
    return dict(zip(MICROBENCH_NAMES, out.tolist()))


def hbm_probe(nbytes=8 << 30, device=0):
    lib = load_diag()
    lib.psmc_hip_hbm_probe.argtypes = [C.c_int, C.c_longlong, _dp]
    out = np.zeros(4)
    rc = lib.psmc_hip_hbm_probe(int(device), int(nbytes), _p(out))
    if rc != 0:
        raise HipError("hbm_probe: %s" % load_library().psmc_hip_strerror(rc).decode())
    return dict(zip(["fill", "read", "copy", "sweep_store"], out.tolist()))


def load_probe(n_waves, steps=20000, device=0):
    lib = load_diag()
    lib.psmc_hip_load_probe.argtypes = [C.c_int, C.c_int, C.c_int, _dp]
    out = np.zeros(4)
    rc = lib.psmc_hip_load_probe(int(device), int(n_waves), int(steps), _p(out))
    if rc != 0:
        raise HipError("load_probe: %s" % load_library().psmc_hip_strerror(rc).decode())
    return dict(zip(["ms", "cycles_per_step", "max_cycles_per_step", "mhz"], out.tolist()))


def stream_probe(n_doubles=1 << 27, device=0):
    lib = load_diag()
    lib.psmc_hip_stream_probe.argtypes = [C.c_int, C.c_longlong, _dp]
    ms = C.c_double(0)
    rc = lib.psmc_hip_stream_probe(int(device), int(n_doubles), C.byref(ms))
    if rc != 0:
        raise HipError("stream_probe: %s" % load_library().psmc_hip_strerror(rc).decode())
    return ms.value, 16.0 * n_doubles / (ms.value * 1e-3) / 1e9


PIPE_PROBE_CONFIGS = ["4 matrix waves (1/SIMD)", "4 vector waves (1/SIMD)", "8 matrix waves (2/SIMD)", "8 vector waves (2/SIMD)",
                      "waves 0-3 matrix + 4-7 vector (one of each per SIMD)", "even waves matrix, odd vector (SIMDs not mixed)"]


def pipe_probe(device=0):
    lib = load_diag()
    lib.psmc_hip_pipe_probe.argtypes = [C.c_int, _dp, C.c_int]
    out = np.zeros(8 * len(PIPE_PROBE_CONFIGS))
    rc = lib.psmc_hip_pipe_probe(int(device), _p(out), len(out))
    if rc != 0:
        raise HipError("pipe_probe: %s" % load_library().psmc_hip_strerror(rc).decode())
    return {name: [round(v, 1) for v in out[8 * i:8 * i + 8] if v > 0] for i, name in enumerate(PIPE_PROBE_CONFIGS)}


PIPE_KINDS = {"idle": 0, "mfma_f64": 1, "fma_f64": 2, "mov_dpp": 3, "scan_levels": 4, "ds_read_b128": 5, "sload_readlane": 6,
              "add_u32": 7, "fma_f32": 8, "add_f64": 9}


def pipe_probe2(kinds, rounds=64, device=0):
    lib = load_diag()
    k = (C.c_int * 8)(*([PIPE_KINDS[x] if isinstance(x, str) else int(x) for x in kinds] + [0] * (8 - len(kinds))))
    out = np.zeros(8)
    lib.psmc_hip_pipe_probe2.argtypes = [C.c_int, C.POINTER(C.c_int), C.c_int, _dp]
    rc = lib.psmc_hip_pipe_probe2(int(device), k, int(rounds), _p(out))
    if rc != 0:
        raise HipError("pipe_probe2: %s" % load_library().psmc_hip_strerror(rc).decode())
    return [float(v) for v in out[:len(kinds)]]


def place_probe(n_waves, waves_per_block=1, n_kernels=1, steps=3328, device=0):
    lib = load_diag()
    npad = (n_waves + waves_per_block - 1) // waves_per_block * waves_per_block
    out = np.zeros(3 * npad * n_kernels); ms = C.c_double(0)
    lib.psmc_hip_place_probe.argtypes = [C.c_int, C.c_int, C.c_int, C.c_int, C.c_int, _dp, C.POINTER(C.c_double)]
    rc = lib.psmc_hip_place_probe(int(device), int(n_waves), int(waves_per_block), int(n_kernels), int(steps), _p(out), C.byref(ms))
    if rc != 0:
        raise HipError("place_probe: %s" % load_library().psmc_hip_strerror(rc).decode())
    o = out.reshape(-1, 3)
    o = o[o[:, 0] > 0]
    hw = o[:, 1].astype(np.int64); xcc = o[:, 2].astype(np.int64) & 0xf
    simd = (hw >> 4) & 3; cu = (hw >> 8) & 0xf; sh = (hw >> 12) & 1; se = (hw >> 13) & 7
    key = (((xcc * 8 + se) * 2 + sh) * 16 + cu) * 4 + simd
    _, cnt = np.unique(key, return_counts=True)
    cus = len(np.unique(key // 4))
    return dict(ms=ms.value, cycles_mean=float(o[:, 0].mean()), cycles_max=float(o[:, 0].max()), waves=len(o), simds_used=len(cnt), cus_used=cus,
                max_waves_per_simd=int(cnt.max()), hist={int(k): int((cnt == k).sum()) for k in np.unique(cnt)})


def cumask_probe(n_cus_a, n_waves_a, n_waves_b, steps=3328, device=0):
    lib = load_diag()
    out = np.zeros(3 * (n_waves_a + n_waves_b)); ms = C.c_double(0)
    lib.psmc_hip_cumask_probe.argtypes = [C.c_int, C.c_int, C.c_int, C.c_int, C.c_int, _dp, C.POINTER(C.c_double)]
# ... 99 lines not shown
```

Before: 2.541 billion bins/s.

## Share forward K-column product matrices with backward chains via transposed copy

When a tile needs transfer-product matrices for both the forward and the backward chain, only the forward product is built. It is also written out transposed, and the backward chain reads that transposed copy, rescaling after the multiply and stepping the boundary bins separately. This roughly halves the K-column construction work for such tiles. The cost is a doubled Kcol allocation, strided transposed stores, and extra boundary handling in the chain kernel. It is on by default via kc_share=1, but only applies to the ns=64 path where PER==1.

```diff
diff --git a/include/psmc_hip.h b/include/psmc_hip.h
--- a/include/psmc_hip.h
+++ b/include/psmc_hip.h
@@ -60,6 +60,7 @@
                        int *warmup_used);
 int psmc_hip_fast_repairs(psmc_hip_ctx *ctx, int out[6]);
 int psmc_hip_fast_plan(psmc_hip_ctx *ctx, double out[8]);
+int psmc_hip_fast_plan_kc(psmc_hip_ctx *ctx, int out[4]);
 
 int psmc_hip_estep_factored(psmc_hip_ctx *ctx, const double *a, const double *e, const double *a0, double *sums,
                             double *E, double *LL);
diff --git a/psmc_amd/csrc/api.hip b/psmc_amd/csrc/api.hip
--- a/psmc_amd/csrc/api.hip
+++ b/psmc_amd/csrc/api.hip
@@ -204,6 +204,7 @@
 	else if (k == "coarse") { if (v < -1 || v > 16) return PSMC_HIP_EINVAL; c->coarse = (int)v; c->plan_dirty = true; c->items_dirty = true; }
 	else if (k == "kc_sub") { if (v < 1 || v > 16) return PSMC_HIP_EINVAL; c->kc_sub = (int)v; c->kc_sub_set = true; c->plan_dirty = true; c->items_dirty = true; }
 	else if (k == "two_phase") { if (v != -1 && v != 0 && v != 2) return PSMC_HIP_EINVAL; c->two_phase = (int)v; c->plan_dirty = true; c->items_dirty = true; }
+	else if (k == "kc_share") { if (v != 0 && v != 1) return PSMC_HIP_EINVAL; c->kc_share = (int)v; c->items_dirty = true; }
 	else if (k == "kc_min") { if (v < -1) return PSMC_HIP_EINVAL; c->kc_min = (int)v; c->items_dirty = true; }
 	else if (k == "ckpt") { c->ckpt = v != 0 ? 1 : 0; }
 	else if (k == "fuse") { c->fuse = v != 0 ? 1 : 0; c->plan_dirty = true; }
diff --git a/psmc_amd/csrc/api_batch.hip b/psmc_amd/csrc/api_batch.hip
--- a/psmc_amd/csrc/api_batch.hip
+++ b/psmc_amd/csrc/api_batch.hip
@@ -402,7 +402,7 @@
 		k->n_sub = c->n_sub; k->target_waves = c->target_waves; k->overlap = c->overlap; k->warm_tol = c->warm_tol; k->struct_opt = c->struct_opt;
 		k->struct_tiles_set = c->struct_tiles_set; k->struct_tiles = c->struct_tiles;
 		k->two_phase = c->two_phase; k->kc_div = c->kc_div; k->kc_min = c->kc_min; k->ckpt = c->ckpt; k->fuse = c->fuse;
-		k->learn = c->learn; k->group_cap = c->group_cap; k->warm_shift = c->warm_shift; k->kc_sub = c->kc_sub; k->kcol_prio = c->kcol_prio;
+		k->learn = c->learn; k->group_cap = c->group_cap; k->warm_shift = c->warm_shift; k->kc_sub = c->kc_sub; k->kc_share = c->kc_share; k->kcol_prio = c->kcol_prio;
 		k->fuse128 = c->fuse128; k->coarse = c->coarse; k->gate = c->gate; k->lanes8 = c->lanes8; k->gap_tiles = c->gap_tiles; k->exact_refwd = c->exact_refwd;
 		k->merge = c->merge; k->adapt = c->adapt; k->prev_start = c->prev_start;
 		k->merge1 = c->merge1; k->merge_order = c->merge_order; k->runs_late = c->runs_late; k->warm_shift_set = c->warm_shift_set; k->kc_sub_set = c->kc_sub_set;
diff --git a/psmc_amd/csrc/api_fast.hip b/psmc_amd/csrc/api_fast.hip
--- a/psmc_amd/csrc/api_fast.hip
+++ b/psmc_amd/csrc/api_fast.hip
@@ -267,15 +267,7 @@
 		if (!qv.empty()) HIPCHK(c, hipMemcpy(c->d_queue, qv.data(), sizeof(int) * qv.size(), hipMemcpyHostToDevice));
 	}
 	std::vector<int> wl((size_t)4 * nc, 0), kc, runs_f, runs_b, kslot, kuniq;
-	int gap_slot[2] = {-1, -1};
-	auto push_kc = [&](int t, int dir) {
-		const int j = (int)kc.size() / 2;
-		kc.push_back(t); kc.push_back(dir);
-		if (gaps && c->gap[t] && c->chunk_used % 4 == 0) {
-			if (gap_slot[dir] < 0) { gap_slot[dir] = (int)kuniq.size(); kuniq.push_back(j); }
-			kslot.push_back(gap_slot[dir]);
-		} else { kslot.push_back((int)kuniq.size()); kuniq.push_back(j); }
-	};
+	auto push_kc = [&](int t, int dir) { kc.push_back(t); kc.push_back(dir); };
 	c->n_wl_f = c->n_wl_b = 0;
 	const int kc_min = c->kc_min >= 0 ? c->kc_min : (c->ns == 128 ? (nc > 4096 ? 12 : 8) : (nc > 4096 ? 5 : 4));
 	const bool chains = kc_min >= 2;
@@ -309,6 +301,30 @@
 	};
 	add_runs(kf, c->n_long_f, false);
 	add_runs(kb, c->n_long_b, true);
+	{
+		const int n_kc = (int)kc.size() / 2;
+		const bool gap_share = gaps && c->chunk_used % 4 == 0, share = c->kc_share && kcol2_on(c);
+		std::vector<char> has_f(nc, 0), has_b(nc, 0);
+		for (int j = 0; j < n_kc; ++j) (kc[2 * j + 1] ? has_b : has_f)[kc[2 * j]] = 1;
+		int gap_slot[3] = {-1, -1, -1};
+		std::vector<int> both_slot(share ? nc : 0, -1);
+		c->n_kshared = c->n_kc_shared = 0;
+		for (int j = 0; j < n_kc; ++j) {
+			const int t = kc[2 * j], dir = kc[2 * j + 1];
+			const Chunk &ch = c->chunks[t];
+			const bool sh = share && has_f[t] && has_b[t] && ch.lo > 1 && ch.hi < ch.L && ch.hi - ch.lo + 1 >= 8;
+			const int fl = sh ? KC_SHARED : 0;
+			int *known = (gap_share && c->gap[t]) ? &gap_slot[sh ? 2 : dir] : (sh ? &both_slot[t] : nullptr);
+			int s = known ? *known : -1;
+			if (s < 0) {
+				s = (int)kuniq.size(); kuniq.push_back(j | fl);
+				if (known) *known = s;
+				c->n_kshared += sh;
+			}
+			kslot.push_back(s | fl);
+			c->n_kc_shared += sh;
+		}
+	}
 	c->n_chain_f = (int)runs_f.size() / 4; c->n_chain_b = (int)runs_b.size() / 4; c->n_kc = (int)kc.size() / 2; c->n_kuniq = (int)kuniq.size();
 	if ((size_t)c->n_kc > (size_t)2 * nc || (size_t)(c->n_chain_f + c->n_chain_b) > (size_t)nc) return fail(c, PSMC_HIP_ESTATE, "build_items: list overflow");
 	HIPCHK(c, hipMemcpy(c->d_items + (size_t)12 * nc, wl.data(), sizeof(int) * wl.size(), hipMemcpyHostToDevice));
@@ -319,7 +335,7 @@
 		HIPCHK(c, hipMemcpy(c->d_items + (size_t)26 * nc, kslot.data(), sizeof(int) * kslot.size(), hipMemcpyHostToDevice));
 		HIPCHK(c, hipMemcpy(c->d_items + (size_t)28 * nc, kuniq.data(), sizeof(int) * kuniq.size(), hipMemcpyHostToDevice));
 		const size_t nsub = kcol2_on(c) ? (size_t)c->kc_sub_used : 1;
-		const size_t need = (size_t)c->n_kuniq * nsub * ((size_t)c->ns * c->ns + c->ns);
+		const size_t need = (size_t)c->n_kuniq * nsub * ((size_t)c->ns * c->ns * (c->n_kshared > 0 ? 2 : 1) + c->ns);
 		if (need > c->kcol_cap) { int rc; if ((rc = dev_alloc(c, &c->d_Kcol, need))) return rc; c->kcol_cap = need; }
 	}
 	c->items_dirty = false;
@@ -488,6 +504,7 @@
 	p.kcol_prio = c->kcol_prio;
 	p.d_Kcol = c->d_Kcol; p.kc_sub = kcol2_on(c) ? c->kc_sub_used : 1;
 	p.d_Kexp = c->d_Kcol ? c->d_Kcol + (size_t)c->n_kuniq * p.kc_sub * c->ns * c->ns : nullptr; p.stream5 = c->stream5;
+	p.d_KcolT = c->d_Kcol && c->n_kshared > 0 ? p.d_Kexp + (size_t)c->n_kuniq * p.kc_sub * c->ns : nullptr;
 	for (int i = 0; i < 14; ++i) p.evx[i] = c->evx[i];
 	p.d_LLpart = c->d_LLpart; p.d_stage = c->d_stage; p.d_stats = d_out; p.d_warm = c->d_warm;
 	p.tiny_total = (double)c->sel.size() * HMM_TINY_H;
@@ -625,6 +642,14 @@
 	return PSMC_HIP_OK;
 }
 
+extern "C" int psmc_hip_fast_plan_kc(psmc_hip_ctx *c, int out[4])
+{
+	if (!c || !out) return PSMC_HIP_EINVAL;
+	const bool on = !c->wf_ran && c->use_struct && !c->chunks.empty();
+	out[0] = on ? c->n_kc : 0; out[1] = on ? c->n_kuniq : 0; out[2] = on ? c->n_kshared : 0; out[3] = on ? c->n_kc_shared : 0;
+	return PSMC_HIP_OK;
+}
+
 extern "C" int psmc_hip_fast_plan(psmc_hip_ctx *c, double out[8])
 {
 	if (!c || !out) return PSMC_HIP_EINVAL;
@@ -656,6 +681,17 @@
 	if (A0) memset(A0, 0, sizeof(double) * n);
 	if (chk) for (size_t i = 0; i < c->sel.size(); ++i) chk[i] = 1.0;
 	return PSMC_HIP_OK;
+}
+
+extern "C" int psmcdbg_get_boundary(psmc_hip_ctx *c, double *entry, double *bentry)
+{
+	if (!c || !entry || !bentry || !c->d_entry || !c->d_bentry || c->chunks.empty()) return -1;
+	(void)hipSetDevice(c->device);
+	(void)hipDeviceSynchronize();
+	const size_t n = c->chunks.size() * (size_t)c->ns;
+	if (hipMemcpy(entry, c->d_entry, sizeof(double) * n, hipMemcpyDeviceToHost) != hipSuccess) return -1;
+	if (hipMemcpy(bentry, c->d_bentry, sizeof(double) * n, hipMemcpyDeviceToHost) != hipSuccess) return -1;
+	return 0;
 }
 
 extern "C" int psmcdbg_check_bentry(psmc_hip_ctx *c)
diff --git a/psmc_amd/csrc/estep_struct.hip b/psmc_amd/csrc/estep_struct.hip
--- a/psmc_amd/csrc/estep_struct.hip
+++ b/psmc_amd/csrc/estep_struct.hip
@@ -590,6 +590,11 @@
 	top = fwd ? c.hi : min(c.hi, c.L - 1);
 	lo = fwd ? c.lo : min(((c.lo + 3) & ~3) + 1, top + 1);
 }
+__host__ __device__ inline void kc_range_shared(const Chunk &c, int &lo, int &top)
+{
+	kc_range(c, 1, lo, top);
+	lo += 1; top = c.hi;
+}
 
 template <int NPL>
 __global__ __launch_bounds__(64) void k_kcol_struct(const double *__restrict__ sp, const double *__restrict__ e,
@@ -640,7 +645,7 @@
 template <int NQ>
 __global__ __launch_bounds__(64 * NQ) void k_kcol2_struct(const double *__restrict__ kcc, const uint8_t *__restrict__ obs,
                                                             const Chunk *__restrict__ chunks, const KcTile *__restrict__ kc, const int *__restrict__ uniq,
-                                                            double *__restrict__ Kcol, double *__restrict__ Kexp, int sub, int prio)
+                                                            double *__restrict__ Kcol, double *__restrict__ Kexp, double *__restrict__ KcolT, int sub, int prio)
 {
 	constexpr int S = 32 * NQ, NCG = S / 64, KD = 11 * S;
 	__shared__ double xch[2][NQ][2][64];
@@ -650,13 +655,15 @@
 	const int j = (int)blockIdx.x / NCG, cg = (int)blockIdx.x % NCG, jt = j / sub, js = j % sub;
 	const int col = 64 * cg + lane;
 	if (prio >= 2) __builtin_amdgcn_s_setprio(2); else if (prio == 1) __builtin_amdgcn_s_setprio(1);
-	const KcTile kt = kc[uniq[jt]];
+	const int uq = uniq[jt];
+	const bool shared = (uq & KC_SHARED) != 0;
+	const KcTile kt = kc[uq & ~KC_SHARED];
 	const Chunk c = chunks[kt.tile];
-	const bool fwd = kt.dir == 0;
+	const bool fwd = shared || kt.dir == 0;
 	for (int i = threadIdx.x; i < KD; i += 64 * NQ) tab[i] = kcc[(fwd ? 0 : KD) + i];
 	__syncthreads();
 	int top, lo;
-	kc_range(c, kt.dir, lo, top);
+	if (shared) kc_range_shared(c, lo, top); else kc_range(c, kt.dir, lo, top);
 	const uint8_t *o = obs + c.off;
 	const double *cc = tab + 32 * w;
 	double x[32];
@@ -714,6 +721,11 @@
 	double *out = Kcol + ((int64_t)j * S + col) * S + 32 * w;
 #pragma unroll
 	for (int k = 0; k < 32; ++k) out[k] = x[k];
+	if (shared) {
+		double *outT = KcolT + ((int64_t)j * S + 32 * w) * S + col;
+#pragma unroll
+		for (int k = 0; k < 32; ++k) outT[(int64_t)k * S] = x[k];
+	}
 	if (w == 0) Kexp[(int64_t)j * S + col] = (double)E;
 }
 
@@ -740,13 +752,14 @@
 
 template <int PER>
 __global__ __launch_bounds__(64 * (PER == 1 ? 2 : 8)) void k_kchain_struct(const KcRun *__restrict__ runs, int n_f, const int *__restrict__ kslot,
-                                                        const double *__restrict__ Kcol,
+                                                        const double *__restrict__ Kcol, const double *__restrict__ KcolT,
                                                         const double *__restrict__ Kexp, const double *__restrict__ sp,
                                                         const double *__restrict__ e, const uint8_t *__restrict__ obs,
                                                         const Chunk *__restrict__ chunks, double *__restrict__ entry,
                                                         double *__restrict__ bentry, int sub)
 {
 	constexpr int S = 64 * PER, RW = 32 / PER, NW = S / RW;
+	constexpr bool SH = PER == 1;
 	__shared__ double part[2][NW][S];
 	const int lane = threadIdx.x & 63;
 	const int w = __builtin_amdgcn_readfirstlane((int)(threadIdx.x >> 6));
@@ -758,33 +771,45 @@
 	double x[PER];
 	const WaveScanMasks wm = wave_scan_masks(lane);
 	StructPar1 s1[PER];
+	const bool fr = SH && fwd;
 	double e0[PER], e1[PER];
 #pragma unroll
 	for (int q = 0; q < PER; ++q) {
 		const int k = lane + 64 * q;
 		x[q] = vec[(int64_t)t * S + k];
-		s1[q].mS = sp[3 * S + k]; s1[q].wS = sp[S + k]; s1[q].mP = sp[2 * S + k]; s1[q].wP = sp[k]; s1[q].dd = sp[4 * S + k];
+		s1[q].mS = sp[(fr ? 0 : 3) * S + k]; s1[q].wS = sp[(fr ? 2 : 1) * S + k]; s1[q].mP = sp[(fr ? 1 : 2) * S + k]; s1[q].wP = sp[(fr ? 3 : 0) * S + k];
+		s1[q].dd = sp[4 * S + k];
 		e0[q] = e[k]; e1[q] = e[S + k];
 	}
+	auto is_shared = [&](int j) { return SH && (kslot[r.kc0 + j / sub] & KC_SHARED) != 0; };
 	const int n_mats = (r.count - 1) * sub;
 	const int row0 = RW * w, src_h = row0 >> 6, src_l = row0 & 63;
 	double ma[RW][PER], mb[RW][PER], ea[PER], eb[PER];
 	auto load = [&](int j, double (&m)[RW][PER], double (&ex)[PER]) {
-		const int64_t kb = ((int64_t)kslot[r.kc0 + j / sub] * sub + j % sub) * S;
+		const bool tr = !fwd && is_shared(j);
+		const int64_t kb = ((int64_t)(kslot[r.kc0 + j / sub] & ~KC_SHARED) * sub + (tr ? sub - 1 - j % sub : j % sub)) * S;
+		const double *K = tr ? KcolT : Kcol;
 #pragma unroll
 		for (int i = 0; i < RW; ++i)
 #pragma unroll
-			for (int h = 0; h < PER; ++h) m[i][h] = Kcol[(kb + row0 + i) * S + lane + 64 * h];
+			for (int h = 0; h < PER; ++h) m[i][h] = K[(kb + row0 + i) * S + lane + 64 * h];
 #pragma unroll
 		for (int h = 0; h < PER; ++h) ex[h] = Kexp[kb + lane + 64 * h];
 	};
-	auto product = [&](int j, const double (&m)[RW][PER], const double (&ex)[PER]) {
+	auto product = [&](int j, bool tr, const double (&m)[RW][PER], const double (&ex)[PER]) {
 		double xs[PER], y[PER], em = -1e300;
-#pragma unroll
-		for (int h = 0; h < PER; ++h) em = fmax(em, x[h] > 0.0 ? ex[h] : -1e300);
-		const double emax = wave_max_f64(em);
-#pragma unroll
-		for (int h = 0; h < PER; ++h) { xs[h] = x[h] > 0.0 ? __builtin_amdgcn_ldexp(x[h], (int)(ex[h] - emax)) : 0.0; y[h] = 0.0; }
+		if (!tr) {
+#pragma unroll
+			for (int h = 0; h < PER; ++h) em = fmax(em, x[h] > 0.0 ? ex[h] : -1e300);
+			const double emax = wave_max_f64(em);
+#pragma unroll
+			for (int h = 0; h < PER; ++h) xs[h] = x[h] > 0.0 ? __builtin_amdgcn_ldexp(x[h], (int)(ex[h] - emax)) : 0.0;
+		} else {
+#pragma unroll
+			for (int h = 0; h < PER; ++h) xs[h] = x[h];
+		}
+#pragma unroll
+		for (int h = 0; h < PER; ++h) y[h] = 0.0;
 		double src = xs[0];
 		if constexpr (PER == 2) src = src_h ? xs[1] : xs[0];
 #pragma unroll
@@ -803,6 +828,13 @@
 #pragma unroll
 			for (int v = 1; v < NW; ++v) tsum += pp[v][lane + 64 * h];
 			y[h] = tsum;
+		}
+		if (tr) {
+#pragma unroll
+			for (int h = 0; h < PER; ++h) em = fmax(em, y[h] > 0.0 ? ex[h] : -1e300);
+			const double emax = wave_max_f64(em);
+#pragma unroll
+			for (int h = 0; h < PER; ++h) y[h] = y[h] > 0.0 ? __builtin_amdgcn_ldexp(y[h], (int)(ex[h] - emax)) : 0.0;
 		}
 		double tot = y[0];
 		if constexpr (PER == 2) tot += y[1];
@@ -839,15 +871,33 @@
 #pragma unroll
 		for (int h = 0; h < PER; ++h) { if (w == 0) vec[(int64_t)t * S + lane + 64 * h] = y[h]; x[h] = y[h]; }
 	};
+	auto shared_ends = [&](bool before) {
+		if constexpr (SH) {
+			const Chunk c = chunks[t];
+			const uint8_t *o = obs + c.off;
+			int lo, top;
+			kc_range_shared(c, lo, top);
+			if (fwd) for (int p = c.lo; p < lo; ++p) x[0] = struct_step1(s1[0], x[0], wm) * walk_ev((int)o[p - 1] & 3, e0[0], e1[0]);
+			else if (before) x[0] = struct_step1(s1[0], x[0], wm);
+			else x[0] *= walk_ev((int)o[lo - 2] & 3, e0[0], e1[0]);
+		}
+	};
+	auto step = [&](int j, const double (&m)[RW][PER], const double (&ex)[PER]) {
+		const bool sh = is_shared(j);
+		if (sh && j % sub == 0) shared_ends(true);
+		product(j, sh && !fwd, m, ex);
+		if (j % sub == sub - 1) {
+			if (sh && !fwd) shared_ends(false);
+			tile_done();
+		}
+	};
 	if (n_mats > 0) load(0, ma, ea);
 	for (int j = 0; j < n_mats; j += 2) {
 		if (j + 1 < n_mats) load(j + 1, mb, eb);
-		product(j, ma, ea);
-		if (j % sub == sub - 1) tile_done();
+		step(j, ma, ea);
 		if (j + 1 >= n_mats) break;
 		if (j + 2 < n_mats) load(j + 2, ma, ea);
-		product(j + 1, mb, eb);
-		if ((j + 1) % sub == sub - 1) tile_done();
+		step(j + 1, mb, eb);
 	}
 }
 
@@ -1018,14 +1068,14 @@
 		                   (const KcTile *)p.d_kc, p.d_kuniq, p.d_Kcol, p.d_Kexp);
 	else
 		hipLaunchKernelGGL(k_kcol2_struct<2>, dim3(p.n_kuniq * p.kc_sub), dim3(128), 0, st_cols, p.d_kcc, p.d_obs, p.d_chunks, (const KcTile *)p.d_kc, p.d_kuniq,
-		                   p.d_Kcol, p.d_Kexp, p.kc_sub, p.kcol_prio);
+		                   p.d_Kcol, p.d_Kexp, p.d_KcolT, p.kc_sub, p.kcol_prio);
 	if (st_cols != st_chain) { (void)hipEventRecord(ev_cols, st_cols); (void)hipStreamWaitEvent(st_chain, ev_cols, 0); }
 	if (p.ns == 128)
 		hipLaunchKernelGGL(k_kchain_struct<2>, dim3(p.n_chain_f + p.n_chain_b), dim3(512), 0, st_chain, (const KcRun *)p.d_kruns, p.n_chain_f, p.d_kslot,
-		                   p.d_Kcol, p.d_Kexp, p.d_sp, p.d_e, p.d_obs, p.d_chunks, p.d_entry, p.d_bentry, p.kc_sub);
+		                   p.d_Kcol, p.d_KcolT, p.d_Kexp, p.d_sp, p.d_e, p.d_obs, p.d_chunks, p.d_entry, p.d_bentry, p.kc_sub);
 	else
 		hipLaunchKernelGGL(k_kchain_struct<1>, dim3(p.n_chain_f + p.n_chain_b), dim3(128), 0, st_chain, (const KcRun *)p.d_kruns, p.n_chain_f, p.d_kslot,
-		                   p.d_Kcol, p.d_Kexp, p.d_sp, p.d_e, p.d_obs, p.d_chunks, p.d_entry, p.d_bentry, p.kc_sub);
+		                   p.d_Kcol, p.d_KcolT, p.d_Kexp, p.d_sp, p.d_e, p.d_obs, p.d_chunks, p.d_entry, p.d_bentry, p.kc_sub);
 	PSMC_DBG("launch_kchain", p.n_kc, p.n_chain_f, p.n_chain_b);
 }
 int walk_blocks(const EstepLaunch &p) { return p.ns == 64 ? p.n_wl_f + p.n_wl_b : (p.n_wl_f + 3) / 4 + (p.n_wl_b + 3) / 4; }
diff --git a/psmc_amd/csrc/psmc_hip_ctx.h b/psmc_amd/csrc/psmc_hip_ctx.h
--- a/psmc_amd/csrc/psmc_hip_ctx.h
+++ b/psmc_amd/csrc/psmc_hip_ctx.h
@@ -90,6 +90,8 @@
 	std::vector<uint8_t> gap;
 	int gap_tiles = 1;
 	int n_kuniq = 0;
+	int kc_share = 1;
+	int n_kshared = 0, n_kc_shared = 0;
 	std::vector<int> flagged_f, flagged_b;
 	bool items_dirty = true;
 	int n_items_f = 0, n_items_b = 0;
diff --git a/psmc_amd/csrc/psmc_hip_internal.h b/psmc_amd/csrc/psmc_hip_internal.h
--- a/psmc_amd/csrc/psmc_hip_internal.h
+++ b/psmc_amd/csrc/psmc_hip_internal.h
@@ -37,6 +37,7 @@
 
 struct FastReport { int fwd_rounds, bwd_rounds, fwd_tiles, bwd_tiles, converged, merged, recounted; };
 
+constexpr int KC_SHARED = 1 << 30;
 struct EstepLaunch {
 	hipStream_t stream, stream2, stream3;
 	hipEvent_t evx[14];
@@ -81,6 +82,7 @@
 	const int *d_kc, *d_kruns; int n_kc, n_chain_f, n_chain_b;
 	const int *d_kslot, *d_kuniq; int n_kuniq;
 	double *d_Kcol, *d_Kexp;
+	double *d_KcolT;
 	int *d_ritems_f, *d_ritems_b;
 	int *h_ritems;
 	int *m_ritems, *m_cnt;
diff --git a/psmc_amd/hip.py b/psmc_amd/hip.py
--- a/psmc_amd/hip.py
+++ b/psmc_amd/hip.py
@@ -20,7 +20,7 @@
     "psmc_hip_load_segments_device", "psmc_hip_select", "psmc_hip_estep",
     "psmc_hip_estep_segments", "psmc_hip_estep_batch", "psmc_hip_estep_batch_cb", "psmc_hip_reserve_batch_tables", "psmc_hip_batch_info", "psmc_hip_estep_device", "psmc_hip_fast_diag", "psmc_hip_fast_repairs", "psmc_hip_fast_info", "psmc_hip_estep_factored",
     "psmc_hip_get_tables", "psmc_hip_decode", "psmc_hip_posterior", "psmc_hip_post_counts", "psmc_hip_scales",
-    "psmc_hip_group_selfcheck", "psmc_hip_fast_plan",
+    "psmc_hip_group_selfcheck", "psmc_hip_fast_plan", "psmc_hip_fast_plan_kc",
     "psmc_hip_group_create", "psmc_hip_group_destroy", "psmc_hip_group_last_error", "psmc_hip_group_set_option",
     "psmc_hip_group_load_segments", "psmc_hip_group_estep", "psmc_hip_group_estep_factored", "psmc_hip_group_info",
     "psmc_hip_group_route", "psmc_hip_estep_factored_device",
@@ -278,8 +278,11 @@
         o = np.zeros(8)
         self.lib.psmc_hip_fast_plan.argtypes = [C.c_void_p, _dp]
         self._chk(self.lib.psmc_hip_fast_plan(self.h, _p(o)), "fast_plan")
+        kc = (C.c_int * 4)()
+        self.lib.psmc_hip_fast_plan_kc.argtypes = [C.c_void_p, C.POINTER(C.c_int)]
+        self._chk(self.lib.psmc_hip_fast_plan_kc(self.h, kc), "fast_plan_kc")
         return dict(tiles=int(o[0]), tile_len=int(o[1]), warm_fwd_mean=o[2], warm_bwd_mean=o[3], warm_fwd_max=int(o[4]), warm_bwd_max=int(o[5]),
-                    glued_fwd=int(o[6]), glued_bwd=int(o[7]))
+                    glued_fwd=int(o[6]), glued_bwd=int(o[7]), kc_tiles=kc[0], kc_slots=kc[1], kc_shared=kc[2], kc_tiles_shared=kc[3])
 
     def tables(self, seg, want_b=True):
         L = int(self.lens[seg])
```

Result: no change. 2.525 billion bins/s (-0.6%).
